# facebookresearch/robust_cvd

Hardware: NVIDIA H100
Metric: flow_residual_constraints_per_sec_per_gn_iteration (higher is better)
Workload: dtype f64

## Files before the change

### include/rcvd_hooks.h

```cpp
#ifndef RCVD_HOOKS_H_
#define RCVD_HOOKS_H_
#include "rcvd.h"
#ifdef __cplusplus
extern "C" {
#endif

int64_t rcvd_launch_count(rcvd_problem* p);
int64_t rcvd_filter_launch_count(void);
int64_t rcvd_builder_launch_count(void);
int64_t rcvd_static_flag_launch_count(void);
int64_t rcvd_tracks_launch_count(void);
int64_t rcvd_builder_last_rounds(void);

int32_t rcvd_structure_info(rcvd_problem* p, int32_t out[8]);

int32_t rcvd_debug_factor_plan(const rcvd_config* cfg, int32_t np, const int32_t* pairs, int32_t nt, const int32_t* trip_centers,
                               int32_t order_slack, int32_t nranks, int32_t rank, int32_t num_sms,
                               int32_t* order, int32_t* level, int32_t* owner, int32_t* perm, int32_t out[13]);
int32_t rcvd_debug_update_passes(const rcvd_config* cfg, int32_t np, const int32_t* pairs, int32_t nt, const int32_t* trip_centers,
                                 int32_t order_slack, int32_t nranks, int32_t rank, int32_t num_sms,
                                 int32_t* passes, int32_t* sources, int32_t* join, int32_t* flags, int32_t counts[5]);

int32_t rcvd_debug_linear_solve(rcvd_problem* p, const double* S, const double* D2, const double* b, double* y);

int32_t rcvd_debug_solve_matrix(rcvd_problem* p, const double* H, const double* D2, const double* b, double* y);
int32_t rcvd_debug_factor_dense(rcvd_problem* p, int32_t* order, double* L, double* Linv);
int32_t rcvd_debug_linear_paths(rcvd_problem* p, int64_t out[13]);

int32_t rcvd_debug_linear_residual(rcvd_problem* p, double radius, double out[6]);

int32_t rcvd_debug_last_iteration(rcvd_problem* p, double* g, double* xc, double out[2]);

int32_t rcvd_debug_profile_linear(rcvd_problem* p, int32_t reps, double out_ms[8]);
int32_t rcvd_debug_level_profile(rcvd_problem* p, double* out, int32_t max_levels);
int32_t rcvd_debug_fp64_tensor_peak(int32_t device, int32_t shape, double* tflops);

int32_t rcvd_debug_set_fast_path(rcvd_problem* p, int32_t on);
int32_t rcvd_debug_set_overlap(rcvd_problem* p, int32_t on);
int32_t rcvd_debug_set_order_slack(rcvd_problem* p, int32_t slack);
int32_t rcvd_debug_set_eval_only(rcvd_problem* p, int32_t on);
int32_t rcvd_debug_set_distributed(rcvd_problem* p, int32_t on);
int32_t rcvd_distribution_info(rcvd_problem* p, int32_t out[4]);
int32_t rcvd_debug_set_update_kernel(rcvd_problem* p, int32_t tma, int32_t side_items_per_cta);

#ifdef __cplusplus
}
#endif
#endif
```

### robust_cvd_b200/csrc/rcvd_api.cu

```cuda
#include <algorithm>
#include <chrono>
#include <cmath>
#include <cstdarg>
#include <cstdio>
#include <cstring>
#include <dlfcn.h>
#include <limits>
#include <string>
#include <vector>

#include <cub/device/device_segmented_sort.cuh>
#include "rcvd_eval.cuh"
#include "rcvd_linalg.cuh"
#include "rcvd_update.cuh"
#include "rcvd_plan.h"
#include "rcvd_host.h"

using namespace rcvd;

static thread_local std::string g_err = "";
int set_err(int code, const char* fmt, ...) {
  char buf[512]; va_list ap; va_start(ap, fmt); vsnprintf(buf, sizeof(buf), fmt, ap); va_end(ap);
  g_err = buf; return code;
}

namespace nccl {
typedef struct { char internal[128]; } UniqueId;
typedef void* Comm;
static void* lib = nullptr;
static int (*GetUniqueId)(UniqueId*) = nullptr;
static int (*CommInitRank)(Comm*, int, UniqueId, int) = nullptr;
static int (*AllReduce)(const void*, void*, size_t, int, int, Comm, cudaStream_t) = nullptr;
static int (*CommDestroy)(Comm) = nullptr;
static const char* (*GetErrorString)(int) = nullptr;
static int (*GroupStart)() = nullptr;
static int (*GroupEnd)() = nullptr;
static int (*Broadcast)(const void*, void*, size_t, int, int, Comm, cudaStream_t) = nullptr;
static int (*Reduce)(const void*, void*, size_t, int, int, int, Comm, cudaStream_t) = nullptr;
static bool load() {
  if (lib) return true;
  const char* names[] = {"libnccl.so.2", "libnccl.so"};
  for (const char* n : names) { lib = dlopen(n, RTLD_NOW | RTLD_GLOBAL); if (lib) break; }
  if (!lib) return false;
  GetUniqueId = (int (*)(UniqueId*))dlsym(lib, "ncclGetUniqueId");
  CommInitRank = (int (*)(Comm*, int, UniqueId, int))dlsym(lib, "ncclCommInitRank");
  AllReduce = (int (*)(const void*, void*, size_t, int, int, Comm, cudaStream_t))dlsym(lib, "ncclAllReduce");
  CommDestroy = (int (*)(Comm))dlsym(lib, "ncclCommDestroy");
  GetErrorString = (const char* (*)(int))dlsym(lib, "ncclGetErrorString");
  GroupStart = (int (*)())dlsym(lib, "ncclGroupStart"); GroupEnd = (int (*)())dlsym(lib, "ncclGroupEnd");
  Broadcast = (int (*)(const void*, void*, size_t, int, int, Comm, cudaStream_t))dlsym(lib, "ncclBroadcast");
  Reduce = (int (*)(const void*, void*, size_t, int, int, int, Comm, cudaStream_t))dlsym(lib, "ncclReduce");
  return GetUniqueId && CommInitRank && AllReduce && CommDestroy && GroupStart && GroupEnd && Broadcast && Reduce;
}
constexpr int kFloat64 = 8, kUint8 = 1, kSum = 0, kMax = 2;
}

enum { SC_COST = 0, SC_CAND = 1, SC_GY = 2, SC_YHY = 3, SC_STEP2 = 4, SC_X2 = 5, SC_GMAX = 6, SC_GDOTD = 7, SC_DMAX = 8, SC_N = 16 };

__global__ void k_extract_diag(const double* __restrict__ H, double* __restrict__ diag, int N, int npad) {
  const int i = blockIdx.x * blockDim.x + threadIdx.x;
  if (i >= N * npad) return;
  const int f = i / npad, l = i % npad;
  diag[i] = H[(size_t)f * npad * npad + (size_t)l * npad + l];
}
__global__ void k_jacobi_scale(const double* __restrict__ diag, double* __restrict__ S, int n, int enable) {
  const int i = blockIdx.x * blockDim.x + threadIdx.x;
  if (i < n) S[i] = enable ? 1.0 / (1.0 + sqrt(diag[i])) : 1.0;
}
__global__ void k_lm_prepare(const double* __restrict__ diagH, const double* __restrict__ S, const double* __restrict__ g, double* __restrict__ lmdiag,
                             double* __restrict__ D2, double* __restrict__ gs, int n, int reuse, double radius, double dmin, double dmax) {
  const int i = blockIdx.x * blockDim.x + threadIdx.x;
  if (i >= n) return;
  const double s = S[i];
  double d = lmdiag[i];
  if (!reuse) { d = fmin(fmax(s * s * diagH[i], dmin), dmax); lmdiag[i] = d; }
  D2[i] = d / radius;
  gs[i] = s * g[i];
}
__global__ void k_mul(const double* __restrict__ a, const double* __restrict__ b, double* __restrict__ o, int n) {
  const int i = blockIdx.x * blockDim.x + threadIdx.x;
  if (i < n) o[i] = a[i] * b[i];
}
__device__ __forceinline__ double project_lb(const rcvd_config& c, const Layout& L, const uint8_t* in_range, int f, int l, double v) {
  if (c.depth_lower_bound && l >= L.offD && l < L.offS && ((l - L.offD) % L.k) == 0 && in_range[f]) return fmax(v, 0.0);
  return v;
}
__global__ void __launch_bounds__(256) k_state_norms(rcvd_config cfg, Layout L, const uint8_t* __restrict__ in_range, const uint8_t* __restrict__ active,
                                                      const double* __restrict__ x, const double* __restrict__ g, double* __restrict__ scal, int N) {
  const int i = blockIdx.x * blockDim.x + threadIdx.x;
  double x2 = 0.0, gm = 0.0;
  if (i < N * L.nf) {
    const int f = i / L.nf, l = i % L.nf;
    const size_t v = (size_t)f * L.npad + l;
    if (active[v]) {
      x2 = x[i] * x[i];
      gm = fabs(x[i] - project_lb(cfg, L, in_range, f, l, x[i] - g[v]));
    }
  }
  x2 = warp_sum(x2);
#pragma unroll
  for (int o = 16; o > 0; o >>= 1) gm = fmax(gm, __shfl_xor_sync(0xffffffffu, gm, o));
  if ((threadIdx.x & 31) == 0) {
    red_add(scal + SC_X2, x2);
    atomicMax((unsigned long long*)(scal + SC_GMAX), (unsigned long long)__double_as_longlong(gm));
  }
}
__global__ void __launch_bounds__(256) k_dot2(const double* __restrict__ a, const double* __restrict__ b, const double* __restrict__ c,
                                               const double* __restrict__ d, int n, double* __restrict__ scal, int s0, int s1) {
  const int i = blockIdx.x * blockDim.x + threadIdx.x;
  double p = 0.0, q = 0.0;
  if (i < n) { p = a[i] * b[i]; q = c[i] * d[i]; }
  p = warp_sum(p); q = warp_sum(q);
  if ((threadIdx.x & 31) == 0) { red_add(scal + s0, p); red_add(scal + s1, q); }
}
__global__ void k_finalize_mask(rcvd_config cfg, Layout L, uint8_t* __restrict__ mask, int N) {
  const int i = blockIdx.x * blockDim.x + threadIdx.x;
  if (i >= N * L.npad) return;
  const int l = i % L.npad;
  if (l >= L.nf || is_const_local(cfg, L, l)) mask[i] = 0;
}
__global__ void k_project_state(rcvd_config cfg, Layout L, const uint8_t* __restrict__ in_range, double* __restrict__ x, int N) {
  const int i = blockIdx.x * blockDim.x + threadIdx.x;
  if (i < N * L.nf) x[i] = project_lb(cfg, L, in_range, i / L.nf, i % L.nf, x[i]);
}
__global__ void k_h_to_dense(const double* __restrict__ H, const HBlock* __restrict__ hb, int nblocks, double* __restrict__ out, int N, int nf, int npad, const int* __restrict__ uperm) {
  const int b = blockIdx.y;
  const int e = blockIdx.x * blockDim.x + threadIdx.x;
  if (e >= nf * nf) return;
  const int i = e / nf, j = e % nf;
  const HBlock hbk = hb[b];
  if (hbk.r == hbk.c && j > i) return;
  const double v = H[(size_t)b * npad * npad + (size_t)i * npad + j];
  const size_t U = (size_t)N * nf;
  const int ur = uperm[hbk.r], uc = uperm[hbk.c];
  out[((size_t)ur * nf + i) * U + (size_t)uc * nf + j] = v;
  out[((size_t)uc * nf + j) * U + (size_t)ur * nf + i] = v;
}

enum { LP_POTRF_SMEM = 0, LP_POTRF_PANEL, LP_TRSM_LL4, LP_TRSM_LL2, LP_TRSM_GEMM, LP_UPD_TMA1, LP_UPD_TMA2, LP_SUB_LEVEL, LP_SUB_FUSED,
       LP_TRINV, LP_OTHER, LP_UPD_TMA1_MULTI, LP_TRSM_STREAMED, LP_N };

struct RecordSet {
  const int width, nframes;
  std::vector<int32_t> frames; std::vector<int64_t> offsets{0}; std::vector<float> records;
  RecordTiles dev = {}; int num_tiles = 0;
  RecordSet(int width_, int nframes_) : width(width_), nframes(nframes_) {}
  int groups() const { return (int)offsets.size() - 1; }
  int64_t count() const { return offsets.back(); }
};

struct rcvd_problem {
  rcvd_config cfg; Layout L; int N = 0; int device = 0;
  cudaStream_t stream = nullptr;
  std::vector<uint8_t> in_range; std::vector<double> median, adaptive;
  RecordSet pairs{6, 2}, trips{10, 1}, dpairs{6, 2};
  std::vector<int32_t> struct_pairs;
  int first_frame = 0, last_frame = -1;
  int32_t* d_blk_of = nullptr; uint8_t *d_in_range = nullptr, *d_active = nullptr;
  double *d_median = nullptr, *d_adaptive = nullptr; float* d_scale_locs = nullptr; int nscale = 0;
  double *d_x = nullptr, *d_xc = nullptr, *d_xsave = nullptr;
  double *d_g = nullptr, *d_S = nullptr, *d_diagH = nullptr, *d_lmdiag = nullptr, *d_D2 = nullptr, *d_gs = nullptr, *d_rhs = nullptr, *d_ytmp = nullptr,
         *d_y = nullptr, *d_Sy = nullptr, *d_Hy = nullptr, *d_partial = nullptr, *d_scal = nullptr;
  double* h_scal = nullptr;
  int part_reg = 0, part_trip = 0, part_dp = 0, npartial = 0;
  double *d_H = nullptr, *d_Lb = nullptr, *d_T = nullptr, *d_invL = nullptr, *d_invT = nullptr;
  HBlock *d_hblocks = nullptr, *d_lblocks = nullptr; int* d_fail = nullptr;
  int* d_potrf_progress = nullptr;
  FactorKernels fk = {};
  FactorPlan plan;
  int *d_lvl_frames = nullptr; TrsmTask* d_trsm_tasks = nullptr; int2* d_upd_pairs = nullptr; SolveTask* d_fwd_tasks = nullptr;
  SubTask* d_sub_tasks = nullptr; int* d_sub_counters = nullptr; int* d_sub_need = nullptr;
  cudaGraphExec_t solve_graph = nullptr;
  bool structure_ready = false, constraints_set = false, frames_set = false;
  int nranks = 1, rank = 0; nccl::Comm comm = nullptr;
  int64_t launches = 0, graph_launches = 0;
  std::vector<double> h_state; bool state_dirty = false; bool overlap = true; int order_slack = 4;
  cudaStream_t side_stream = nullptr; cudaEvent_t ev_fork = nullptr, ev_join = nullptr;
  std::vector<cudaEvent_t> ev_side;
  cudaStream_t inv_stream = nullptr; cudaEvent_t ev_inv_join = nullptr;
  double *d_g2 = nullptr, *d_delta = nullptr; int* h_fail = nullptr;
  cudaEvent_t ev[8] = {nullptr};
  std::vector<void*> allocs;
  std::vector<std::pair<int, cudaEvent_t>>* prof = nullptr;
  bool eval_only = false;
  bool records_sorted = false;
  int fast_path = 1;
  bool dist_enabled = true, graph_warm = false, force_full_H = false;
  int *d_lvl_own = nullptr, *d_load_lblocks = nullptr, *d_own_hblocks = nullptr, *d_uperm = nullptr;
  UpdItem* d_upd_items = nullptr; CUtensorMap tmapT; int num_sms = 0, upd_ipc = 0;
  std::vector<double> level_ms;
  bool factored = false;
  int64_t paths[LP_N] = {0}, graph_paths[LP_N] = {0};
  rcvd_problem() {}
};

template <class... Params, class... Args>
static int launch(rcvd_problem* p, void (*kernel)(Params...), dim3 grid, dim3 block, size_t smem, cudaStream_t s, bool pdl, Args... args) {
  cudaLaunchAttribute attr = {};
  attr.id = cudaLaunchAttributeProgrammaticStreamSerialization; attr.val.programmaticStreamSerializationAllowed = 1;
  cudaLaunchConfig_t lc = {};
  lc.gridDim = grid; lc.blockDim = block; lc.dynamicSmemBytes = smem; lc.stream = s; lc.attrs = &attr; lc.numAttrs = pdl ? 1 : 0;
  CK(cudaLaunchKernelEx(&lc, kernel, args...));
  p->launches += 1;
  return RCVD_OK;
}

template <class T> static int dalloc(rcvd_problem* p, T** ptr, size_t count) {
  *ptr = nullptr;
  if (count == 0) count = 1;
  cudaError_t e = cudaMallocAsync((void**)ptr, count * sizeof(T), p->stream);
  if (e != cudaSuccess) return set_err(RCVD_ERR_CUDA, "cudaMallocAsync(%zu bytes) failed: %s", count * sizeof(T), cudaGetErrorString(e));
  p->allocs.push_back(*ptr);
  return RCVD_OK;
}
template <class T> static int upload(rcvd_problem* p, T** ptr, const std::vector<T>& v) {
  int rc = dalloc(p, ptr, v.size()); if (rc) return rc;
  if (!v.empty()) CK(cudaMemcpyAsync(*ptr, v.data(), v.size() * sizeof(T), cudaMemcpyHostToDevice, p->stream));
  return RCVD_OK;
}
static void free_all(rcvd_problem* p) {
  if (p->solve_graph) { cudaGraphExecDestroy(p->solve_graph); p->solve_graph = nullptr; }
  if (p->side_stream) cudaStreamSynchronize(p->side_stream);
  if (p->inv_stream) cudaStreamSynchronize(p->inv_stream);
  for (void* q : p->allocs) cudaFreeAsync(q, p->stream);
  p->allocs.clear();
  if (p->stream) cudaStreamSynchronize(p->stream);
  if (p->h_scal) { cudaFreeHost(p->h_scal); p->h_scal = nullptr; }
  p->structure_ready = false; p->factored = false;
}

static DevProblem dev_problem(const rcvd_problem* p) {
  DevProblem d; d.cfg = p->cfg; d.L = p->L; d.N = p->N;
  d.pairs = p->pairs.dev; d.trips = p->trips.dev; d.dpairs = p->dpairs.dev;
  d.blk_of = p->d_blk_of; d.in_range = p->d_in_range; d.median = p->d_median;
  d.adaptive = p->adaptive.empty() ? nullptr : p->d_adaptive; d.scale_locs = p->d_scale_locs;
  d.rank = p->rank; d.nranks = p->nranks;
  return d;
}

template <EvalMode MODE>
static int enqueue_residuals(rcvd_problem* p, const double* x, double* g) {
  const DevProblem d = dev_problem(p);
  const RegCounts rcn = reg_counts(p->cfg, p->L, p->N, p->nscale);
  const int regblocks = p->part_trip - p->part_reg, ntiles = p->pairs.num_tiles;
  cudaStream_t st = p->stream; double* part = p->d_partial; int rc;
  if (ntiles > 0) {
    const bool tc = MODE == EvalMode::CostGradH && p->fast_path != 0;
    if (tc && p->fast_path == 1 && p->records_sorted) rc = launch(p, k_accumulate_runs, ntiles, kTile, kRunSmem, st, false, d, x, p->d_H, g, part);
    else if (tc && fast_path_ok(p->cfg, p->L)) rc = launch(p, k_accumulate_fast, ntiles, kTile, kFastSmem, st, false, d, x, p->d_H, g, part);
    else rc = launch(p, k_pairs<MODE>, ntiles, kTile, 0, st, false, d, x, p->d_H, g, part, p->d_active);
    if (rc) return rc;
  }
  if (regblocks > 0 && (rc = launch(p, k_regularisers<MODE>, regblocks, 128, 0, st, false, d, rcn, x, p->d_H, g, part + p->part_reg, p->d_active,
                                    p->first_frame, p->last_frame))) return rc;
  if (p->trips.num_tiles > 0 && (rc = launch(p, k_triplets<MODE>, p->trips.num_tiles, kTile, 0, st, false, d, x, p->d_H, g, part + p->part_trip, p->d_active))) return rc;
  if (p->dpairs.num_tiles > 0 && (rc = launch(p, k_depth_pairs<MODE>, p->dpairs.num_tiles, kTile, 0, st, false, d, x, p->d_H, g, part + p->part_dp, p->d_active))) return rc;
  return RCVD_OK;
}

#define UP(ptr, vec) if ((rc = upload(p, &(ptr), vec))) return rc
#define DA(ptr, n) if ((rc = dalloc(p, &(ptr), (n)))) return rc
static int upload_plan(rcvd_problem* p) {
  const FactorPlan& pl = p->plan; int rc;
  UP(p->d_blk_of, pl.blk_of); UP(p->d_hblocks, pl.hblocks); UP(p->d_lblocks, pl.lblocks); UP(p->d_lvl_frames, pl.lvl_frames); UP(p->d_lvl_own, pl.lvl_own);
  UP(p->d_load_lblocks, pl.load_lblocks); UP(p->d_own_hblocks, pl.own_hblocks); UP(p->d_uperm, pl.uperm);
  UP(p->d_trsm_tasks, pl.trsm_tasks); UP(p->d_upd_pairs, pl.upd_pairs);
  UP(p->d_sub_tasks, pl.sub_tasks); UP(p->d_sub_need, pl.sub_need); DA(p->d_sub_counters, (size_t)4 * p->N + 4);
  UP(p->d_fwd_tasks, pl.fwd_tasks); UP(p->d_upd_items, pl.upd_items);
  return RCVD_OK;
}

static int upload_record_set(rcvd_problem* p, RecordSet& s) {
  std::vector<int32_t> frames(s.frames.size()), tile_group, tile_count; std::vector<int64_t> tile_begin;
  for (size_t i = 0; i < frames.size(); ++i) frames[i] = p->plan.iperm[s.frames[i]];
  for (int i = 0; i < s.groups(); ++i)
    for (int64_t b = s.offsets[i]; b < s.offsets[i + 1]; b += kTile) { tile_group.push_back(i); tile_begin.push_back(b); tile_count.push_back((int32_t)std::min<int64_t>(kTile, s.offsets[i + 1] - b)); }
  s.num_tiles = (int)tile_group.size();
  float* rec; int32_t *fr, *tg, *tn; int64_t* tb; int rc;
  UP(rec, s.records); UP(fr, frames); UP(tg, tile_group); UP(tb, tile_begin); UP(tn, tile_count);
  s.dev = RecordTiles{rec, fr, tg, tb, tn};
  return RCVD_OK;
}

static int set_up_problem_data(rcvd_problem* p) {
  const int N = p->N; const Layout& L = p->L; const std::vector<int>& uperm = p->plan.uperm; int rc;
  for (RecordSet* s : {&p->pairs, &p->trips, &p->dpairs}) if ((rc = upload_record_set(p, *s))) return rc;
  p->records_sorted = false;
  if (run_path_ok(p->cfg, L) && p->pairs.count() > 0 && p->pairs.count() < (int64_t)0x7fffffff) {
    const long long n = p->pairs.count();
    unsigned *d_k0 = nullptr, *d_k1 = nullptr; int *d_i0 = nullptr, *d_i1 = nullptr; float* d_sorted = nullptr; int64_t* d_off = nullptr; void* d_tmp = nullptr;
    if ((rc = dalloc(p, &d_k0, (size_t)n)) || (rc = dalloc(p, &d_k1, (size_t)n)) || (rc = dalloc(p, &d_i0, (size_t)n)) || (rc = dalloc(p, &d_i1, (size_t)n)) || (rc = dalloc(p, &d_sorted, (size_t)n * 6)) ||
        (rc = upload(p, &d_off, p->pairs.offsets))) return rc;
    if ((rc = launch(p, k_record_keys, (unsigned)((n + 255) / 256), 256, 0, p->stream, false, p->cfg, p->pairs.dev.records, n, d_k0, d_i0))) return rc;
    size_t tmp_bytes = 0;
    CK(cub::DeviceSegmentedSort::SortPairs(nullptr, tmp_bytes, d_k0, d_k1, d_i0, d_i1, (int)n, p->pairs.groups(), d_off, d_off + 1, p->stream));
    CK(cudaMallocAsync(&d_tmp, std::max<size_t>(tmp_bytes, 16), p->stream));
    CK(cub::DeviceSegmentedSort::SortPairs(d_tmp, tmp_bytes, d_k0, d_k1, d_i0, d_i1, (int)n, p->pairs.groups(), d_off, d_off + 1, p->stream));
    if ((rc = launch(p, k_gather_records, (unsigned)((n * 6 + 255) / 256), 256, 0, p->stream, false, p->pairs.dev.records, d_i1, n, d_sorted))) return rc;
    CK(cudaFreeAsync(d_tmp, p->stream));
    CK(cudaGetLastError());
    p->pairs.dev.records = d_sorted; p->records_sorted = true;
  }
  {
    std::vector<uint8_t> ir(N); std::vector<double> md(N), ad;
    for (int i = 0; i < N; ++i) { ir[i] = p->in_range[uperm[i]]; md[i] = p->median[uperm[i]]; }
    UP(p->d_in_range, ir); UP(p->d_median, md);
    if (!p->adaptive.empty()) {
      const size_t G = p->adaptive.size() / N; ad.resize(p->adaptive.size());
      for (int i = 0; i < N; ++i) std::copy(p->adaptive.begin() + (size_t)uperm[i] * G, p->adaptive.begin() + (size_t)(uperm[i] + 1) * G, ad.begin() + (size_t)i * G);
      UP(p->d_adaptive, ad);
    }
  }
  {
    std::vector<float> locs; const int gx = p->cfg.scale_grid_x, gy = p->cfg.scale_grid_y;
    for (int y = 0; y < gy; ++y) for (int x = 0; x < gx; ++x) {
      const float fx = -1.f + 2.f * x / (gx - 1);
      const float fy = -1.f + 2.f * y / (gy - 1);
      locs.push_back(fx); locs.push_back(fy);
    }
    p->nscale = (int)(locs.size() / 2);
    UP(p->d_scale_locs, locs);
  }
  p->first_frame = 0; p->last_frame = -1;
  { bool any = false; for (int f = 0; f < N; ++f) if (p->in_range[f]) { if (!any) { p->first_frame = f; any = true; } p->last_frame = f; } }
  p->part_reg = p->pairs.num_tiles;
  p->part_trip = p->part_reg + (reg_counts(p->cfg, L, N, p->nscale).total + 127) / 128;
  p->part_dp = p->part_trip + p->trips.num_tiles;
  p->npartial = p->part_dp + p->dpairs.num_tiles;
  return RCVD_OK;
}
#undef UP

static int allocate_storage(rcvd_problem* p) {
  const int N = p->N; const Layout& L = p->L; const int npad = L.npad, nLoff = p->plan.nLoff; const size_t bs = (size_t)npad * npad; int rc;
  const size_t Upad = (size_t)N * npad, U = (size_t)N * L.nf;
  DA(p->d_x, U); DA(p->d_xc, U); DA(p->d_xsave, U);
  DA(p->d_g, 2 * Upad + 8); p->d_diagH = p->d_g + Upad + 8;
  DA(p->d_S, Upad); DA(p->d_lmdiag, Upad); DA(p->d_D2, Upad); DA(p->d_gs, Upad); DA(p->d_rhs, Upad);
  DA(p->d_g2, Upad + 8); DA(p->d_delta, Upad);
  DA(p->d_ytmp, Upad); DA(p->d_y, Upad); DA(p->d_Sy, Upad); DA(p->d_Hy, Upad); DA(p->d_scal, SC_N); DA(p->d_active, Upad); DA(p->d_fail, 1);
  DA(p->d_potrf_progress, (size_t)N);
  DA(p->d_partial, (size_t)p->npartial);
  if (p->eval_only) { DA(p->d_H, 1); DA(p->d_Lb, 1); DA(p->d_T, 1); DA(p->d_invL, 1); DA(p->d_invT, 1); }
  else {
    DA(p->d_H, p->plan.hblocks.size() * bs); DA(p->d_Lb, (size_t)(N + nLoff) * bs); DA(p->d_T, (size_t)std::max(nLoff, 1) * bs);
    DA(p->d_invL, (size_t)N * bs); DA(p->d_invT, (size_t)N * npad * 16);
  }
#undef DA
  {
    bool encoded = false;
    typedef CUresult (*EncodeFn)(CUtensorMap*, CUtensorMapDataType, cuuint32_t, void*, const cuuint64_t*, const cuuint64_t*, const cuuint32_t*, const cuuint32_t*,
                                 CUtensorMapInterleave, CUtensorMapSwizzle, CUtensorMapL2promotion, CUtensorMapFloatOOBfill);
    void* fn = nullptr; cudaDriverEntryPointQueryResult qres;
    if (cudaGetDriverEntryPoint("cuTensorMapEncodeTiled", &fn, cudaEnableDefault, &qres) == cudaSuccess && fn && qres == cudaDriverEntryPointSuccess) {
      const cuuint64_t gdim[2] = {(cuuint64_t)npad, (cuuint64_t)std::max(nLoff, 1) * npad};
      const cuuint64_t gstr[1] = {(cuuint64_t)npad * sizeof(double)};
      const cuuint32_t box[2] = {16u, (cuuint32_t)p->plan.upd_rb};
      const cuuint32_t estr[2] = {1u, 1u};
      const CUresult r = ((EncodeFn)fn)(&p->tmapT, CU_TENSOR_MAP_DATA_TYPE_FLOAT64, 2, p->d_T, gdim, gstr, box, estr, CU_TENSOR_MAP_INTERLEAVE_NONE,
                                        CU_TENSOR_MAP_SWIZZLE_128B, CU_TENSOR_MAP_L2_PROMOTION_L2_128B, CU_TENSOR_MAP_FLOAT_OOB_FILL_NONE);
      encoded = (r == CUDA_SUCCESS);
    }
    cudaGetLastError();
    if (!encoded) return set_err(RCVD_ERR_CUDA, "cuTensorMapEncodeTiled unavailable or failed: the TMA update kernel cannot run");
    CK(cudaFuncSetAttribute(k_update_tma<1>, cudaFuncAttributeMaxDynamicSharedMemorySize, (int)upd_smem_bytes(p->plan.upd_rb, 1)));
    CK(cudaFuncSetAttribute(k_update_tma<2>, cudaFuncAttributeMaxDynamicSharedMemorySize, (int)upd_smem_bytes(p->plan.upd_rb, 2)));
  }
  CK(cudaMallocHost((void**)&p->h_scal, (SC_N + 2) * sizeof(double)));
  p->h_fail = (int*)(p->h_scal + SC_N);
  CK(cudaMemsetAsync(p->d_x, 0, U * sizeof(double), p->stream));
  CK(cudaMemsetAsync(p->d_lmdiag, 0, Upad * sizeof(double), p->stream));
  CK(cudaMemsetAsync(p->d_S, 0, Upad * sizeof(double), p->stream));
  CK(cudaMemsetAsync(p->d_active, 0, Upad, p->stream));
  if ((rc = enqueue_residuals<EvalMode::MarkActive>(p, p->d_x, nullptr))) return rc;
  if ((rc = launch(p, k_finalize_mask, (int)((Upad + 255) / 256), 256, 0, p->stream, false, p->cfg, L, p->d_active, N))) return rc;
  if (p->nranks > 1) {
    const int r = nccl::AllReduce(p->d_active, p->d_active, Upad, nccl::kUint8, nccl::kMax, p->comm, p->stream);
    if (r != 0) return set_err(RCVD_ERR_NCCL, "ncclAllReduce(active mask) failed");
  }
  FactorKernels& fk = p->fk = factor_kernels(npad);
  if (fk.trinv_bytes > kMaxDynSmem) return set_err(RCVD_ERR_INVALID, "frame block too large for the panel-inverse kernel (npad=%d)", npad);
  CK(cudaFuncSetAttribute(k_trinv, cudaFuncAttributeMaxDynamicSharedMemorySize, (int)fk.trinv_bytes));
  CK(cudaFuncSetAttribute(k_accumulate_fast, cudaFuncAttributeMaxDynamicSharedMemorySize, kFastSmem));
  CK(cudaFuncSetAttribute(k_accumulate_runs, cudaFuncAttributeMaxDynamicSharedMemorySize, kRunSmem));
  if (fk.trsm_ll) {
    CK(cudaFuncSetAttribute(k_trsm_ll<2>, cudaFuncAttributeMaxDynamicSharedMemorySize, (int)fk.trsm_ll2_bytes));
    CK(cudaFuncSetAttribute(k_trsm_ll<2, true>, cudaFuncAttributeMaxDynamicSharedMemorySize, (int)fk.trsm_ll2_bytes));
    CK(cudaOccupancyMaxActiveBlocksPerMultiprocessor(&fk.trsm2_ctas_per_sm, k_trsm_ll<2, true>, 128, fk.trsm_ll2_bytes));
  }
  if (fk.trsm_ll4) {
    CK(cudaFuncSetAttribute(k_trsm_ll<4>, cudaFuncAttributeMaxDynamicSharedMemorySize, (int)fk.trsm_ll4_bytes));
    CK(cudaFuncSetAttribute(k_trsm_ll<4, true>, cudaFuncAttributeMaxDynamicSharedMemorySize, (int)fk.trsm_ll4_bytes));
  }
  if (fk.potrf_smem) CK(cudaFuncSetAttribute(k_potrf_smem, cudaFuncAttributeMaxDynamicSharedMemorySize, (int)fk.potrf_bytes));
  return RCVD_OK;
}

static int build_structure(rcvd_problem* p) {
  if (p->nranks > 1 && !p->dpairs.frames.empty()) return set_err(RCVD_ERR_INVALID, "depth-normalisation pairs are not sharded: they need a single-GPU problem (nranks = 1)");
  free_all(p);
  CK(cudaSetDevice(p->device));
  std::vector<int32_t> graph = p->struct_pairs.empty() ? p->pairs.frames : p->struct_pairs;
  graph.insert(graph.end(), p->dpairs.frames.begin(), p->dpairs.frames.end());
  if (const char* e = make_factor_plan(p->plan, p->cfg, graph, p->trips.frames, p->order_slack, p->nranks, p->rank, p->dist_enabled, p->num_sms))
    return set_err(RCVD_ERR_INVALID, "%s", e);
  while (p->ev_side.size() < 2 * p->plan.levels.size()) { cudaEvent_t e; CK(cudaEventCreateWithFlags(&e, cudaEventDisableTiming)); p->ev_side.push_back(e); }
  int rc;
  if ((rc = upload_plan(p)) || (rc = set_up_problem_data(p)) || (rc = allocate_storage(p))) return rc;
  CK(cudaStreamSynchronize(p->stream));
  p->structure_ready = true;
  return RCVD_OK;
}

static int allreduce(rcvd_problem* p, double* buf, size_t count) {
  if (p->nranks <= 1) return RCVD_OK;
  const int r = nccl::AllReduce(buf, buf, count, nccl::kFloat64, nccl::kSum, p->comm, p->stream);
  if (r != 0) return set_err(RCVD_ERR_NCCL, "ncclAllReduce failed: %s", nccl::GetErrorString ? nccl::GetErrorString(r) : "?");
  return RCVD_OK;
}
struct Seg { size_t first, count; };
static int grouped(rcvd_problem* p, double* base, size_t unit, const std::vector<Seg>& segs, bool bcast) {
  int r = nccl::GroupStart();
  for (size_t i = 0; i < segs.size() && r == 0; ++i) {
    if (segs[i].count == 0) continue;
    const int root = (int)(i % (size_t)p->nranks);
    double* ptr = base + segs[i].first * unit;
    r = bcast ? nccl::Broadcast(ptr, ptr, segs[i].count * unit, nccl::kFloat64, root, p->comm, p->stream)
              : nccl::Reduce(ptr, ptr, segs[i].count * unit, nccl::kFloat64, nccl::kSum, root, p->comm, p->stream);
  }
  const int r2 = nccl::GroupEnd();
  if (r == 0) r = r2;
  if (r != 0) return set_err(RCVD_ERR_NCCL, "grouped NCCL %s failed: %s", bcast ? "broadcast" : "reduce", nccl::GetErrorString ? nccl::GetErrorString(r) : "?");
  return RCVD_OK;
}

struct FactorSolve {
  enum { P_LOAD = 0, P_POTRF, P_TRINV, P_TRSM, P_GEMM, P_SOLVE };
  rcvd_problem* p; const FactorPlan& pl; const FactorKernels& fk; const int N, npad, strips; cudaStream_t st, side, inv;
  int prof_level = 0;
  bool side_used = false, inv_used = false;
  int side_joined = -1;

  explicit FactorSolve(rcvd_problem* p_)
      : p(p_), pl(p_->plan), fk(p_->fk), N(p_->N), npad(p_->L.npad), strips((npad + kTrsmStrip - 1) / kTrsmStrip), st(p_->stream), side(p_->side_stream),
        inv(p_->inv_stream) {}

  void mark(int cls) {
    if (!p->prof) return;
    cudaEvent_t e; cudaEventCreate(&e); cudaEventRecord(e, st); p->prof->push_back({cls < 0 ? cls : (cls | (prof_level << 8)), e});
  }
  template <class... Params, class... Args>
  int launch(int path, void (*kernel)(Params...), dim3 grid, dim3 block, size_t smem, cudaStream_t s, bool pdl, Args... args) {
    if (int rc = ::launch(p, kernel, grid, block, smem, s, pdl, args...)) return rc;
    p->paths[path]++;
    return RCVD_OK;
  }
  int wait(cudaStream_t waiter, cudaStream_t from, cudaEvent_t e) {
    CK(cudaEventRecord(e, from)); CK(cudaStreamWaitEvent(waiter, e, 0));
    return RCVD_OK;
  }
  int join_all(int level) {
    if (side_used) { if (int rc = wait(st, side, p->ev_join)) return rc; side_joined = 2 * level - 1; }
    if (inv_used) { if (int rc = wait(st, inv, p->ev_inv_join)) return rc; inv_used = false; }
    return RCVD_OK;
  }

  bool trsm_deep(const Level& v) const { return strips * v.ntrsm <= p->num_sms && fk.trsm_ll4; }
  bool streamed(const Level& v) const {
    return fk.trsm_ll && v.nown > 0 && v.ntrsm > 0 && fk.potrf_smem && strips * v.ntrsm <= (trsm_deep(v) ? 1 : fk.trsm2_ctas_per_sm) * p->num_sms;
  }

  int factor_diagonal(const int* frames, int nfr, bool pdl) {
    if (fk.potrf_smem)
      return launch(LP_POTRF_SMEM, k_potrf_smem, dim3(nfr), dim3(kPotrfSmemThreads), fk.potrf_bytes, st, pdl, p->d_Lb, p->d_invT, frames, npad,
                    p->d_fail, p->d_potrf_progress);
    for (int jb = 0; jb < npad / 16; ++jb) {
      if (int rc = launch(LP_POTRF_PANEL, k_potrf_panel, dim3(nfr), dim3(kPotrfThreads), 0, st, false, p->d_Lb, p->d_invT, frames, npad, jb, p->d_fail)) return rc;
      const int m = npad - (jb + 1) * 16, n64 = (m + 63) / 64;
      if (m > 0) { if (int rc = launch(LP_OTHER, k_potrf_trail, dim3(n64 * (n64 + 1) / 2, nfr), dim3(128), 0, st, false, p->d_Lb, frames, npad, jb)) return rc; }
    }
    return RCVD_OK;
  }

  int trsm(const Level& lv, const int* frames, int nfr, bool chain) {
    const bool inv_stream = fk.trsm_ll && p->overlap;
    if (inv_stream) { if (int rc = wait(inv, st, p->ev_fork)) return rc; inv_used = true; }
    if (int rc = launch(LP_TRINV, k_trinv, dim3(npad / 16, nfr), dim3(256), fk.trinv_bytes, inv_stream ? inv : st, false,
                        p->d_Lb, p->d_invT, p->d_invL, frames, npad)) return rc;
    mark(P_TRINV);
    if (lv.ntrsm == 0) return RCVD_OK;
    int rc;
    if (fk.trsm_ll) {
      const bool deep = trsm_deep(lv);
      decltype(&k_trsm_ll<2>) kernel = deep ? (chain ? k_trsm_ll<4, true> : k_trsm_ll<4>) : (chain ? k_trsm_ll<2, true> : k_trsm_ll<2>);
      if (chain) p->paths[LP_TRSM_STREAMED]++;
      rc = launch(deep ? LP_TRSM_LL4 : LP_TRSM_LL2, kernel, dim3(strips, lv.ntrsm), dim3(128), deep ? fk.trsm_ll4_bytes : fk.trsm_ll2_bytes, st, chain,
                  p->d_T, p->d_Lb, p->d_invT, p->d_trsm_tasks + lv.trsm_off, npad, chain ? p->d_potrf_progress : nullptr);
    } else {
      const int tiles = (npad + 63) / 64;
      rc = launch(LP_TRSM_GEMM, k_gemm_nt, dim3(tiles, tiles, lv.ntrsm), dim3(128), 0, st, false, p->d_T, p->d_Lb, p->d_invL,
                  p->d_trsm_tasks + lv.trsm_off, npad);
    }
    if (rc) return rc;
    mark(P_TRSM);
    return RCVD_OK;
  }

  int update(cudaStream_t s, int off, int n) {
    if (n <= p->num_sms)
      return launch(LP_UPD_TMA2, k_update_tma<2>, dim3(n), dim3(UpdShape<2>::threads), upd_smem_bytes(pl.upd_rb, 2), s, false,
                    p->tmapT, p->d_Lb, p->d_upd_items + off, n, p->d_upd_pairs, npad, pl.upd_neff, pl.upd_rb, 0);
    int grid = std::min(n, 2 * p->num_sms);
    if (p->upd_ipc > 0) grid = std::max(grid, (n + p->upd_ipc - 1) / p->upd_ipc);
    if (grid < n) p->paths[LP_UPD_TMA1_MULTI]++;
    return launch(LP_UPD_TMA1, k_update_tma<1>, dim3(grid), dim3(UpdShape<1>::threads), upd_smem_bytes(pl.upd_rb, 1), s, false,
                  p->tmapT, p->d_Lb, p->d_upd_items + off, n, p->d_upd_pairs, npad, pl.upd_neff, pl.upd_rb, 0);
  }

  int updates(int li) {
    const Level& lv = pl.levels[li];
    const bool u2 = lv.nit2[0] + lv.nit2[1] > 0;
    const bool fork_late = li + 1 < (int)pl.levels.size() && streamed(pl.levels[li + 1]);
    if (p->overlap && u2 && !fork_late) { if (int rc = wait(side, st, p->ev_fork)) return rc; }
    if (p->overlap) {
      int s = -1;
      for (int q = side_joined + 1; q < 2 * li; ++q) { const Level& v = pl.levels[q / 2]; if (v.nit2[q % 2] > 0 && v.join[q % 2] <= li) s = q; }
      if (s >= 0) { CK(cudaStreamWaitEvent(st, p->ev_side[s], 0)); side_joined = s; }
    }
    if (lv.nit > 0) { if (int rc = update(st, lv.it_off, lv.nit)) return rc; mark(P_GEMM); }
    if (p->overlap && u2 && fork_late) { if (int rc = wait(side, st, p->ev_fork)) return rc; }
    for (int h = 0; h < 2; ++h) if (lv.nit2[h] > 0) {
      if (int rc = update(p->overlap ? side : st, lv.it2_off[h], lv.nit2[h])) return rc;
      mark(P_GEMM);
      if (p->overlap) { CK(cudaEventRecord(p->ev_side[2 * li + h], side)); side_used = true; }
    }
    return RCVD_OK;
  }

  int broadcast_level(int li) {
    std::vector<Seg> segs;
    for (int q = 0; q < p->nranks; ++q) segs.push_back({(size_t)pl.tseg[(li * p->nranks + q) * 2], (size_t)pl.tseg[(li * p->nranks + q) * 2 + 1]});
    return grouped(p, p->d_T, (size_t)npad * npad, segs, true);
  }
  int phase_boundary() {
    if (int rc = join_all(pl.LB)) return rc;
    const size_t bsz = (size_t)npad * npad;
    std::vector<Seg> invs, tr;
    for (int q = 0; q < p->nranks; ++q) invs.push_back({(size_t)pl.fa_off[q], (size_t)pl.fa_cnt[q]});
    for (int q = 0; q < p->nranks; ++q) tr.push_back({(size_t)pl.fb_off[q], (size_t)pl.fb_cnt[q]});
    for (int q = 0; q < p->nranks; ++q) tr.push_back({(size_t)N + (size_t)pl.bseg[2 * q], (size_t)pl.bseg[2 * q + 1]});
    if (int rc = grouped(p, p->d_invL, bsz, invs, true)) return rc;
    return grouped(p, p->d_Lb, bsz, tr, true);
  }

  int substitution() {
    CK(cudaMemcpyAsync(p->d_rhs, p->d_gs, (size_t)N * npad * sizeof(double), cudaMemcpyDeviceToDevice, st));
    const int LS = pl.sub_first_level;
    int rc;
    for (int l = 0; l < LS; ++l) {
      const Level& lv = pl.levels[l];
      if ((rc = launch(LP_SUB_LEVEL, k_fwd_diag, dim3((npad + 7) / 8, lv.nframes), dim3(256), 0, st, false, p->d_invL, p->d_rhs, p->d_ytmp,
                       p->d_lvl_frames + lv.frame_off, npad))) return rc;
      if (lv.nfwd > 0 && (rc = launch(LP_SUB_LEVEL, k_fwd_update, dim3((npad + 7) / 8, lv.nfwd), dim3(256), 0, st, false, p->d_T, p->d_ytmp, p->d_rhs,
                                      p->d_fwd_tasks + lv.fwd_off, npad))) return rc;
    }
    if (LS < (int)pl.levels.size() && !pl.sub_tasks.empty()) {
      CK(cudaMemsetAsync(p->d_sub_counters, 0, ((size_t)4 * N + 4) * sizeof(int), st));
      SubCounters cn; cn.ticket = p->d_sub_counters; cn.fin = p->d_sub_counters + 4; cn.fdone = cn.fin + N; cn.bin = cn.fdone + N; cn.bdone = cn.bin + N;
      cn.fin_need = p->d_sub_need; cn.bin_need = p->d_sub_need + N;
      const int ntasks = (int)pl.sub_tasks.size();
      if ((rc = launch(LP_SUB_FUSED, k_substitution, dim3(std::min(ntasks, p->num_sms)), dim3(kSubThreads), fk.substitution_bytes, st, false,
                       p->d_invL, p->d_T, p->d_rhs, p->d_ytmp, p->d_y, p->d_sub_tasks, ntasks, cn, npad))) return rc;
    }
    for (int l = LS - 1; l >= 0; --l) {
      const Level& lv = pl.levels[l];
      if (lv.nfwd > 0 && (rc = launch(LP_SUB_LEVEL, k_bwd_update, dim3((npad + 31) / 32, lv.nfwd), dim3(256), 0, st, false, p->d_T, p->d_y, p->d_ytmp,
                                      p->d_fwd_tasks + lv.fwd_off, npad))) return rc;
      if ((rc = launch(LP_SUB_LEVEL, k_bwd_diag, dim3((npad + 31) / 32, lv.nframes), dim3(256), 0, st, false, p->d_invL, p->d_ytmp, p->d_y,
                       p->d_lvl_frames + lv.frame_off, npad))) return rc;
    }
    mark(P_SOLVE);
    return RCVD_OK;
  }
};

static int enqueue_factor_solve(rcvd_problem* p) {
  FactorSolve f(p);
  const FactorPlan& pl = p->plan; const int npad = p->L.npad, nlv = (int)pl.levels.size();
  f.mark(-1);
  CK(cudaMemsetAsync(p->d_potrf_progress, 0, (size_t)p->N * sizeof(int), p->stream));
  const int nfill = (int)pl.load_lblocks.size() - pl.nload;
  if (int rc = f.launch(LP_OTHER, k_load_factor, dim3((npad * npad + 255) / 256, pl.nload + load_factor_pad_rows(npad, pl.upd_neff, nfill)), dim3(256), 0,
                        p->stream, false, p->d_H, p->d_Lb, p->d_lblocks, p->d_S, p->d_D2, npad, p->L.nf, pl.upd_neff, p->d_load_lblocks, pl.nload, nfill)) return rc;
  f.mark(FactorSolve::P_LOAD);
  for (int li = 0; li < nlv; ++li) {
    const Level& lv = pl.levels[li]; f.prof_level = li;
    if (pl.dist && li == pl.LB) { if (int rc = f.phase_boundary()) return rc; }
    if (lv.nown > 0) {
      const int* frames = p->d_lvl_own + lv.own_off;
      const bool chain = f.streamed(lv);
      if (int rc = f.factor_diagonal(frames, lv.nown, chain && li > 0)) return rc;
      f.mark(FactorSolve::P_POTRF);
      if (int rc = f.trsm(lv, frames, lv.nown, chain)) return rc;
    }
    if (pl.dist && li < pl.LB) { if (int rc = f.broadcast_level(li)) return rc; }
    if (int rc = f.updates(li)) return rc;
  }
  if (pl.dist && pl.LB >= nlv) { if (int rc = f.phase_boundary()) return rc; }
  if (int rc = f.join_all(nlv)) return rc;
  if (int rc = f.substitution()) return rc;
  CK(cudaGetLastError());
  return RCVD_OK;
}

static int factor_solve(rcvd_problem* p) {
  if (p->nranks > 1 && !p->graph_warm) {
    p->graph_warm = true; p->factored = true;
    return enqueue_factor_solve(p);
  }
  if (!p->solve_graph) {
    cudaGraph_t graph;
    const int64_t l0 = p->launches;
    int64_t paths0[LP_N]; std::copy(p->paths, p->paths + LP_N, paths0);
    CK(cudaStreamBeginCapture(p->stream, cudaStreamCaptureModeThreadLocal));
    int rc = enqueue_factor_solve(p);
    cudaError_t e = cudaStreamEndCapture(p->stream, &graph);
    for (int i = 0; i < LP_N; ++i) { p->graph_paths[i] = p->paths[i] - paths0[i]; p->paths[i] = paths0[i]; }
    if (rc) return rc;
    if (e != cudaSuccess) return set_err(RCVD_ERR_CUDA, "graph capture failed: %s", cudaGetErrorString(e));
    CK(cudaGraphInstantiate(&p->solve_graph, graph, 0));
    cudaGraphDestroy(graph);
    p->graph_launches = p->launches - l0;
    p->launches = l0;
  }
  CK(cudaGraphLaunch(p->solve_graph, p->stream));
  p->launches += p->graph_launches;
  for (int i = 0; i < LP_N; ++i) p->paths[i] += p->graph_paths[i];
  p->factored = true;
  return RCVD_OK;
}


static int enqueue_evaluate(rcvd_problem* p, const double* x, bool wantG, bool wantH, double* gout, int slot) {
  if (wantH && p->eval_only) return set_err(RCVD_ERR_INVALID, "this handle was set to evaluation-only (rcvd_debug_set_eval_only): no normal matrix");
  const Layout& L = p->L; const int N = p->N, npad = L.npad; cudaStream_t st = p->stream;
  const size_t bs = (size_t)npad * npad, Upad = (size_t)N * npad;
  if (wantH) CK(cudaMemsetAsync(p->d_H, 0, p->plan.hblocks.size() * bs * sizeof(double), st));
  if (wantG) CK(cudaMemsetAsync(gout, 0, (Upad + 8) * sizeof(double), st));
  int rc = wantH ? enqueue_residuals<EvalMode::CostGradH>(p, x, gout)
           : wantG ? enqueue_residuals<EvalMode::CostGrad>(p, x, gout) : enqueue_residuals<EvalMode::Cost>(p, x, gout);
  if (rc) return rc;
  if ((rc = launch(p, k_reduce_partials, 1, 1024, 0, st, false, p->d_partial, p->npartial, p->d_scal, slot))) return rc;
  if (p->nranks > 1) {
    if (wantG) {
      CK(cudaMemcpyAsync(gout + Upad, p->d_scal + slot, sizeof(double), cudaMemcpyDeviceToDevice, st));
      size_t cnt = Upad + 8;
      if (wantH && gout == p->d_g) { if ((rc = launch(p, k_extract_diag, (int)((Upad + 255) / 256), 256, 0, st, false, p->d_H, p->d_diagH, N, npad))) return rc; cnt = 2 * Upad + 8; }
      if ((rc = allreduce(p, gout, cnt))) return rc;
      CK(cudaMemcpyAsync(p->d_scal + slot, gout + Upad, sizeof(double), cudaMemcpyDeviceToDevice, st));
    } else if ((rc = allreduce(p, p->d_scal + slot, 1))) return rc;
    if (wantH) {
      if (p->plan.dist && !p->force_full_H) {
        std::vector<Seg> segs;
        for (int q = 0; q < p->nranks; ++q) segs.push_back({(size_t)p->plan.fa_off[q], (size_t)(p->plan.fa_cnt[q] + p->plan.fb_cnt[q])});
        for (int q = 0; q < p->nranks; ++q) segs.push_back({(size_t)p->plan.hseg[2 * q], (size_t)p->plan.hseg[2 * q + 1]});
        if ((rc = grouped(p, p->d_H, bs, segs, false))) return rc;
      } else if ((rc = allreduce(p, p->d_H, p->plan.hblocks.size() * bs))) return rc;
    }
  }
  return RCVD_OK;
}

static int upload_frames(rcvd_problem* p, double* dst, const double* src_user, int stride_dst, int stride_src, int count) {
  std::vector<double> tmp((size_t)p->N * stride_dst, 0.0);
  for (int i = 0; i < p->N; ++i) memcpy(tmp.data() + (size_t)i * stride_dst, src_user + (size_t)p->plan.uperm[i] * stride_src, (size_t)count * sizeof(double));
  CK(cudaMemcpyAsync(dst, tmp.data(), tmp.size() * sizeof(double), cudaMemcpyHostToDevice, p->stream));
  CK(cudaStreamSynchronize(p->stream));
  return RCVD_OK;
}
static int download_frames(rcvd_problem* p, double* dst_user, const double* src, int stride_dst, int stride_src, int count) {
  std::vector<double> tmp((size_t)p->N * stride_src);
  CK(cudaMemcpyAsync(tmp.data(), src, tmp.size() * sizeof(double), cudaMemcpyDeviceToHost, p->stream));
  CK(cudaStreamSynchronize(p->stream));
  for (int i = 0; i < p->N; ++i) memcpy(dst_user + (size_t)p->plan.uperm[i] * stride_dst, tmp.data() + (size_t)i * stride_src, (size_t)count * sizeof(double));
  return RCVD_OK;
}
static int save_state(rcvd_problem* p) {
  DevGuard g(p->device); cudaStreamSynchronize(p->stream);
  if (p->h_state.size() != (size_t)p->N * p->L.nf) p->h_state.assign((size_t)p->N * p->L.nf, 0.0);
  return download_frames(p, p->h_state.data(), p->d_x, p->L.nf, p->L.nf, p->L.nf);
}

static int ensure_ready(rcvd_problem* p) {
  if (!p->structure_ready) {
    if (p->in_range.empty()) p->in_range.assign(p->N, 1);
    if (p->median.empty()) p->median.assign(p->N, 1.0);
    int rc = build_structure(p); if (rc) return rc;
    p->state_dirty = true;
  }
  if (p->state_dirty) {
    if (p->h_state.size() != (size_t)p->N * p->L.nf) p->h_state.assign((size_t)p->N * p->L.nf, 0.0);
    { int rc = upload_frames(p, p->d_x, p->h_state.data(), p->L.nf, p->L.nf, p->L.nf); if (rc) return rc; }
    p->state_dirty = false;
  }
  return RCVD_OK;
}

static int read_scalars(rcvd_problem* p) {
  CK(cudaMemcpyAsync(p->h_scal, p->d_scal, SC_N * sizeof(double), cudaMemcpyDeviceToHost, p->stream));
  CK(cudaMemcpyAsync(p->h_fail, p->d_fail, sizeof(int), cudaMemcpyDeviceToHost, p->stream));
  CK(cudaStreamSynchronize(p->stream));
  return RCVD_OK;
}

namespace ls {
struct Sample { double x, value, gradient; bool valueValid, gradValid; };
static double evalPoly(const std::vector<double>& p, double x) { double v = 0; for (double c : p) v = v * x + c; return v; }
static bool solveDense(std::vector<std::vector<double>> A, std::vector<double> b, std::vector<double>& x) {
  const int n = (int)b.size(); std::vector<int> perm(n); for (int i = 0; i < n; ++i) perm[i] = i;
  for (int k = 0; k < n; ++k) {
    int pr = k, pc = k; double best = 0;
    for (int i = k; i < n; ++i) for (int j = k; j < n; ++j) if (std::fabs(A[i][j]) > best) { best = std::fabs(A[i][j]); pr = i; pc = j; }
    if (best == 0) return false;
    std::swap(A[k], A[pr]); std::swap(b[k], b[pr]);
    for (int i = 0; i < n; ++i) std::swap(A[i][k], A[i][pc]);
    std::swap(perm[k], perm[pc]);
    for (int i = k + 1; i < n; ++i) { const double f = A[i][k] / A[k][k]; for (int j = k; j < n; ++j) A[i][j] -= f * A[k][j]; b[i] -= f * b[k]; }
  }
  std::vector<double> y(n);
  for (int i = n - 1; i >= 0; --i) { double s = b[i]; for (int j = i + 1; j < n; ++j) s -= A[i][j] * y[j]; y[i] = s / A[i][i]; }
  x.assign(n, 0.0); for (int i = 0; i < n; ++i) x[perm[i]] = y[i];
  return true;
}
static std::vector<double> realRoots(std::vector<double> p) {
  while (!p.empty() && p[0] == 0.0) p.erase(p.begin());
  std::vector<double> out; const int d = (int)p.size() - 1; if (d < 1) return out;
  if (d == 1) { out.push_back(-p[1] / p[0]); return out; }
  if (d == 2) { const double a = p[0], b = p[1], c = p[2], D = b * b - 4 * a * c; if (D >= 0) { const double sq = std::sqrt(D); out.push_back((-b + sq) / (2 * a)); out.push_back((-b - sq) / (2 * a)); } else { out.push_back(-b / (2 * a)); out.push_back(-b / (2 * a)); } return out; }
  std::vector<std::pair<double, double>> z(d);
  for (int i = 0; i < d; ++i) { const double ang = 2 * M_PI * i / d + 0.4; z[i] = {0.9 * std::cos(ang), 0.9 * std::sin(ang)}; }
  auto cmul = [](std::pair<double, double> a, std::pair<double, double> b) { return std::make_pair(a.first * b.first - a.second * b.second, a.first * b.second + a.second * b.first); };
  auto cdiv = [](std::pair<double, double> a, std::pair<double, double> b) { const double dd = b.first * b.first + b.second * b.second; return std::make_pair((a.first * b.first + a.second * b.second) / dd, (a.second * b.first - a.first * b.second) / dd); };
  for (int it = 0; it < 500; ++it) {
    double mx = 0;
    for (int i = 0; i < d; ++i) {
      std::pair<double, double> v = {p[0], 0.0};
      for (int j = 1; j <= d; ++j) { v = cmul(v, z[i]); v.first += p[j]; }
      std::pair<double, double> den = {p[0], 0.0};
      for (int j = 0; j < d; ++j) if (j != i) den = cmul(den, {z[i].first - z[j].first, z[i].second - z[j].second});
      auto dl = cdiv(v, den); z[i].first -= dl.first; z[i].second -= dl.second;
      mx = std::max(mx, std::fabs(dl.first) + std::fabs(dl.second));
    }
    if (mx < 1e-14) break;
  }
  for (auto& r : z) out.push_back(r.first);
  return out;
// ... 280 lines not shown
  return RCVD_OK;
}
RCVD_API int32_t rcvd_problem_set_constraints(rcvd_problem* p, int32_t np, const int32_t* pf, const int64_t* off, const float* rec) {
  return set_records(p, &rcvd_problem::pairs, "constraint", np, pf, off, rec);
}
RCVD_API int32_t rcvd_problem_set_triplets(rcvd_problem* p, int32_t nt, const int32_t* centers, const int64_t* off, const float* rec) {
  return set_records(p, &rcvd_problem::trips, "triplet", nt, centers, off, rec);
}
RCVD_API int32_t rcvd_problem_set_depth_pairs(rcvd_problem* p, int32_t np, const int32_t* pf, const int64_t* off, const float* rec) {
  if (p && p->nranks > 1 && np > 0) return set_err(RCVD_ERR_INVALID, "depth-normalisation pairs are not sharded: they need a single-GPU problem (nranks = 1)");
  return set_records(p, &rcvd_problem::dpairs, "depth-pair", np, pf, off, rec);
}
RCVD_API int32_t rcvd_problem_set_structure(rcvd_problem* p, int32_t np, const int32_t* pf) {
  if (!p || np < 0 || (np > 0 && !pf)) return set_err(RCVD_ERR_INVALID, "bad structure arrays");
  p->struct_pairs.assign(pf, pf + 2 * (size_t)np);
  p->structure_ready = false;
  return RCVD_OK;
}
RCVD_API int32_t rcvd_nccl_unique_id(uint8_t out[128]) {
  if (!nccl::load()) return set_err(RCVD_ERR_NCCL, "libnccl.so.2 not found");
  nccl::UniqueId id; const int r = nccl::GetUniqueId(&id);
  if (r != 0) return set_err(RCVD_ERR_NCCL, "ncclGetUniqueId failed (%d)", r);
  memcpy(out, id.internal, 128); return RCVD_OK;
}
RCVD_API int32_t rcvd_problem_init_comm(rcvd_problem* p, int32_t nranks, int32_t rank, const uint8_t uid[128]) {
  if (!p || nranks < 1 || rank < 0 || rank >= nranks) return set_err(RCVD_ERR_INVALID, "bad rank/nranks");
  if (nranks == 1) { p->nranks = 1; p->rank = 0; return RCVD_OK; }
  if (!nccl::load()) return set_err(RCVD_ERR_NCCL, "libnccl.so.2 not found");
  SET_DEVICE(p->device);
  nccl::UniqueId id; memcpy(id.internal, uid, 128);
  const int r = nccl::CommInitRank(&p->comm, nranks, id, rank);
  if (r != 0) return set_err(RCVD_ERR_NCCL, "ncclCommInitRank failed: %s", nccl::GetErrorString ? nccl::GetErrorString(r) : "?");
  p->nranks = nranks; p->rank = rank; p->structure_ready = false;
  return RCVD_OK;
}
RCVD_API int32_t rcvd_problem_set_state(rcvd_problem* p, const double* x) {
  if (!p || !x) return set_err(RCVD_ERR_INVALID, "null argument");
  p->h_state.assign(x, x + (size_t)p->N * p->L.nf); p->state_dirty = true;
  return RCVD_OK;
}
RCVD_API int32_t rcvd_problem_get_state(rcvd_problem* p, double* x) {
  if (!p || !x) return set_err(RCVD_ERR_INVALID, "null argument");
  const size_t U = (size_t)p->N * p->L.nf;
  if (!p->structure_ready || p->state_dirty) { if (p->h_state.size() != U) p->h_state.assign(U, 0.0); memcpy(x, p->h_state.data(), U * sizeof(double)); return RCVD_OK; }
  SET_DEVICE(p->device);
  return download_frames(p, x, p->d_x, p->L.nf, p->L.nf, p->L.nf);
}
RCVD_API int32_t rcvd_evaluate(rcvd_problem* p, double* cost, double* gradient) {
  if (!p || !cost) return set_err(RCVD_ERR_INVALID, "null argument");
  SET_DEVICE(p->device);
  int rc = ensure_ready(p); if (rc) return rc;
  CK(cudaMemsetAsync(p->d_scal, 0, SC_N * sizeof(double), p->stream));
  rc = enqueue_evaluate(p, p->d_x, gradient != nullptr, false, p->d_g, SC_COST); if (rc) return rc;
  rc = read_scalars(p); if (rc) return rc;
  *cost = p->h_scal[SC_COST];
  if (gradient) {
    if ((rc = download_frames(p, gradient, p->d_g, p->L.nf, p->L.npad, p->L.nf))) return rc;
  }
  return RCVD_OK;
}
RCVD_API int32_t rcvd_normal_matrix_dense(rcvd_problem* p, double* Hout) {
  if (!p || !Hout) return set_err(RCVD_ERR_INVALID, "null argument");
  SET_DEVICE(p->device);
  int rc = ensure_ready(p); if (rc) return rc;
  p->force_full_H = true;
  rc = enqueue_evaluate(p, p->d_x, true, true, p->d_g, SC_COST);
  p->force_full_H = false;
  if (rc) return rc;
  const size_t U = (size_t)p->N * p->L.nf;
  double* d_out = nullptr;
  CK(cudaMalloc((void**)&d_out, U * U * sizeof(double)));
  CK(cudaMemsetAsync(d_out, 0, U * U * sizeof(double), p->stream));
  rc = launch(p, k_h_to_dense, dim3(nblk((size_t)p->L.nf * p->L.nf), (int)p->plan.hblocks.size()), 256, 0, p->stream, false, p->d_H, p->d_hblocks, (int)p->plan.hblocks.size(), d_out, p->N, p->L.nf, p->L.npad, p->d_uperm);
  cudaError_t e = rc ? cudaSuccess : cudaMemcpyAsync(Hout, d_out, U * U * sizeof(double), cudaMemcpyDeviceToHost, p->stream);
  cudaStreamSynchronize(p->stream); cudaFree(d_out);
  if (rc) return rc;
  if (e != cudaSuccess) return set_err(RCVD_ERR_CUDA, "copy failed: %s", cudaGetErrorString(e));
  return RCVD_OK;
}
static int solve_loaded(rcvd_problem* p, const double* S, const double* D2, const double* b, double* y) {
  const int N = p->N, nf = p->L.nf, npad = p->L.npad; const size_t Upad = (size_t)N * npad;
  std::vector<double> hs(Upad, 1.0), hd(Upad, 1.0), hb(Upad, 0.0);
  for (int f = 0; f < N; ++f) for (int l = 0; l < nf; ++l) { const size_t u = (size_t)p->plan.uperm[f] * nf + l; hs[(size_t)f * npad + l] = S ? S[u] : 1.0; hd[(size_t)f * npad + l] = D2[u]; hb[(size_t)f * npad + l] = b[u]; }
  CK(cudaMemcpyAsync(p->d_S, hs.data(), Upad * 8, cudaMemcpyHostToDevice, p->stream));
  CK(cudaMemcpyAsync(p->d_D2, hd.data(), Upad * 8, cudaMemcpyHostToDevice, p->stream));
  CK(cudaMemcpyAsync(p->d_gs, hb.data(), Upad * 8, cudaMemcpyHostToDevice, p->stream));
  CK(cudaMemsetAsync(p->d_fail, 0, sizeof(int), p->stream));
  int rc = factor_solve(p); if (rc) return rc;
  std::vector<double> hy(Upad);
  CK(cudaMemcpyAsync(hy.data(), p->d_y, Upad * 8, cudaMemcpyDeviceToHost, p->stream));
  rc = read_scalars(p); if (rc) return rc;
  for (int f = 0; f < N; ++f) for (int l = 0; l < nf; ++l) y[(size_t)p->plan.uperm[f] * nf + l] = hy[(size_t)f * npad + l];
  if (*p->h_fail) return set_err(RCVD_ERR_NUMERIC, "factorisation hit a non-positive pivot");
  return RCVD_OK;
}
RCVD_API int32_t rcvd_debug_linear_solve(rcvd_problem* p, const double* S, const double* D2, const double* b, double* y) {
  if (!p) return set_err(RCVD_ERR_INVALID, "null argument");
  SET_DEVICE(p->device);
  int rc = ensure_ready(p); if (rc) return rc;
  rc = enqueue_evaluate(p, p->d_x, true, true, p->d_g, SC_COST); if (rc) return rc;
  return solve_loaded(p, S, D2, b, y);
}
RCVD_API int32_t rcvd_debug_solve_matrix(rcvd_problem* p, const double* H, const double* D2, const double* b, double* y) {
  if (!p || !H || !D2 || !b || !y) return set_err(RCVD_ERR_INVALID, "null argument");
  if (p->nranks > 1) return set_err(RCVD_ERR_INVALID, "rcvd_debug_solve_matrix works on single-GPU handles only");
  if (p->eval_only) return set_err(RCVD_ERR_INVALID, "this handle was set to evaluation-only (rcvd_debug_set_eval_only): no factor storage");
  SET_DEVICE(p->device);
  int rc = ensure_ready(p); if (rc) return rc;
  const int N = p->N, nf = p->L.nf, npad = p->L.npad; const size_t U = (size_t)N * nf, bs = (size_t)npad * npad;
  std::vector<uint8_t> coupled((size_t)N * N, 0);
  for (const HBlock& hb : p->plan.hblocks) { const int a = p->plan.uperm[hb.r], c = p->plan.uperm[hb.c]; coupled[(size_t)a * N + c] = coupled[(size_t)c * N + a] = 1; }
  for (int a = 0; a < N; ++a) for (int c = 0; c < N; ++c) {
    if (coupled[(size_t)a * N + c]) continue;
    for (int i = 0; i < nf; ++i) for (int j = 0; j < nf; ++j)
      if (H[((size_t)a * nf + i) * U + (size_t)c * nf + j] != 0.0)
        return set_err(RCVD_ERR_INVALID, "H couples frames %d and %d, which the problem's frame graph does not couple", a, c);
  }
  std::vector<double> hH(p->plan.hblocks.size() * bs, 0.0);
  for (int h = 0; h < (int)p->plan.hblocks.size(); ++h) {
    const int a = p->plan.uperm[p->plan.hblocks[h].r], c = p->plan.uperm[p->plan.hblocks[h].c];
    for (int i = 0; i < nf; ++i) for (int j = 0; j < nf; ++j) hH[h * bs + (size_t)i * npad + j] = H[((size_t)a * nf + i) * U + (size_t)c * nf + j];
  }
  CK(cudaMemcpyAsync(p->d_H, hH.data(), hH.size() * sizeof(double), cudaMemcpyHostToDevice, p->stream));
  return solve_loaded(p, nullptr, D2, b, y);
}
RCVD_API int32_t rcvd_debug_factor_dense(rcvd_problem* p, int32_t* order, double* L, double* Linv) {
  if (!p || !order || !L) return set_err(RCVD_ERR_INVALID, "null argument");
  if (!p->structure_ready || !p->factored) return set_err(RCVD_ERR_INVALID, "no factorisation has run on this handle");
  if (p->plan.dist) return set_err(RCVD_ERR_INVALID, "the distributed factorisation keeps its blocks on their owners");
  SET_DEVICE(p->device);
  CK(cudaStreamSynchronize(p->side_stream)); CK(cudaStreamSynchronize(p->inv_stream)); CK(cudaStreamSynchronize(p->stream));
  const int N = p->N, nf = p->L.nf, npad = p->L.npad, nT = p->plan.nLoff; const size_t U = (size_t)N * nf, bs = (size_t)npad * npad;
  std::vector<double> hL((size_t)N * bs), hT((size_t)nT * bs);
  CK(cudaMemcpy(hL.data(), p->d_Lb, hL.size() * sizeof(double), cudaMemcpyDeviceToHost));
  if (nT > 0) CK(cudaMemcpy(hT.data(), p->d_T, hT.size() * sizeof(double), cudaMemcpyDeviceToHost));
  std::vector<size_t> off(N);
  for (int q = 0; q < N; ++q) { off[p->plan.elim_order[q]] = (size_t)q * nf; order[q] = p->plan.uperm[p->plan.elim_order[q]]; }
  std::fill(L, L + U * U, 0.0);
  for (int f = 0; f < N; ++f)
    for (int i = 0; i < nf; ++i) for (int j = 0; j <= i; ++j) L[(off[f] + i) * U + off[f] + j] = hL[f * bs + (size_t)i * npad + j];
  for (int t = 0; t < nT; ++t) {
    const HBlock& b = p->plan.lblocks[N + t];
    for (int i = 0; i < nf; ++i) for (int j = 0; j < nf; ++j) L[(off[b.r] + i) * U + off[b.c] + j] = hT[t * bs + (size_t)i * npad + j];
  }
  if (Linv) {
    CK(cudaMemcpy(hL.data(), p->d_invL, hL.size() * sizeof(double), cudaMemcpyDeviceToHost));
    for (int f = 0; f < N; ++f) {
      double* out = Linv + off[f] * nf;
      for (int i = 0; i < nf; ++i) for (int j = 0; j < nf; ++j) out[(size_t)i * nf + j] = j <= i ? hL[f * bs + (size_t)i * npad + j] : 0.0;
    }
  }
  return RCVD_OK;
}
RCVD_API int32_t rcvd_debug_linear_paths(rcvd_problem* p, int64_t out[13]) {
  if (!p || !out) return set_err(RCVD_ERR_INVALID, "null argument");
  static_assert(LP_N == 13, "include/rcvd_hooks.h documents thirteen counters");
  std::copy(p->paths, p->paths + LP_N, out);
  return RCVD_OK;
}
RCVD_API int32_t rcvd_time_accumulate(rcvd_problem* p, int32_t iters, double* ms) {
  if (!p || iters <= 0) return set_err(RCVD_ERR_INVALID, "bad argument");
  SET_DEVICE(p->device);
  int rc = ensure_ready(p); if (rc) return rc;
  if ((rc = enqueue_evaluate(p, p->d_x, true, true, p->d_g, SC_COST))) return rc;
  CK(cudaEventRecord(p->ev[0], p->stream));
  for (int i = 0; i < iters; ++i) if ((rc = enqueue_evaluate(p, p->d_x, true, true, p->d_g, SC_COST))) return rc;
  CK(cudaEventRecord(p->ev[1], p->stream));
  CK(cudaStreamSynchronize(p->stream));
  *ms = ev_ms(p->ev[0], p->ev[1]) / iters;
  return RCVD_OK;
}
RCVD_API int32_t rcvd_time_iteration(rcvd_problem* p, int32_t iters, double radius, double* ms_iter, double* ms_acc, double* ms_lin, double* ms_cost) {
  if (!p || iters <= 0) return set_err(RCVD_ERR_INVALID, "bad argument");
  SET_DEVICE(p->device);
  int rc = ensure_ready(p); if (rc) return rc;
  const size_t Upad = (size_t)p->N * p->L.npad; cudaStream_t st = p->stream;
  rcvd_solve_options o; rcvd_default_solve_options(&o);
  double ta = 0, tl = 0, tc = 0, tt = 0;
  for (int it = -1; it < iters; ++it) {
    CK(cudaMemsetAsync(p->d_scal, 0, SC_N * sizeof(double), st));
    CK(cudaMemsetAsync(p->d_fail, 0, sizeof(int), st));
    CK(cudaEventRecord(p->ev[0], st));
    if ((rc = enqueue_assemble(p))) return rc;
    if ((rc = launch(p, k_jacobi_scale, nblk(Upad), 256, 0, st, false, p->d_diagH, p->d_S, (int)Upad, o.jacobi_scaling))) return rc;
    CK(cudaEventRecord(p->ev[1], st));
    if ((rc = enqueue_damped_step(p, o, radius, false))) return rc;
    CK(cudaEventRecord(p->ev[2], st));
    if ((rc = enqueue_candidate_cost(p, 1.0, false))) return rc;
    CK(cudaEventRecord(p->ev[3], st));
    if ((rc = read_scalars(p))) return rc;
    if (it >= 0) { ta += ev_ms(p->ev[0], p->ev[1]); tl += ev_ms(p->ev[1], p->ev[2]); tc += ev_ms(p->ev[2], p->ev[3]); tt += ev_ms(p->ev[0], p->ev[3]); }
  }
  *ms_iter = tt / iters; if (ms_acc) *ms_acc = ta / iters; if (ms_lin) *ms_lin = tl / iters; if (ms_cost) *ms_cost = tc / iters;
  return RCVD_OK;
}
RCVD_API int32_t rcvd_debug_last_iteration(rcvd_problem* p, double* g, double* xc, double out[2]) {
  if (!p || !g || !xc || !out) return set_err(RCVD_ERR_INVALID, "null argument");
  if (!p->structure_ready) return set_err(RCVD_ERR_INVALID, "no iteration has run on this handle");
  SET_DEVICE(p->device);
  int rc = read_scalars(p); if (rc) return rc;
  out[0] = p->h_scal[SC_COST]; out[1] = p->h_scal[SC_CAND];
  if ((rc = download_frames(p, g, p->d_g, p->L.nf, p->L.npad, p->L.nf))) return rc;
  return download_frames(p, xc, p->d_xc, p->L.nf, p->L.nf, p->L.nf);
}
RCVD_API int32_t rcvd_debug_profile_linear(rcvd_problem* p, int32_t reps, double out_ms[8]) {
  const bool keep_overlap = reps < 0; if (reps < 0) reps = -reps;
  if (!p || !out_ms || reps == 0) return set_err(RCVD_ERR_INVALID, "bad argument");
  SET_DEVICE(p->device);
  int rc = ensure_ready(p); if (rc) return rc;
  const bool ov = p->overlap; if (!keep_overlap) p->overlap = false;
  for (int i = 0; i < 8; ++i) out_ms[i] = 0.0;
  std::vector<std::pair<int, cudaEvent_t>> evs;
  p->level_ms.assign(p->plan.levels.size() * 6, 0.0);
  for (int r = -1; r < reps; ++r) {
    CK(cudaMemsetAsync(p->d_fail, 0, sizeof(int), p->stream));
    evs.clear(); p->prof = &evs;
    rc = enqueue_factor_solve(p);
    p->prof = nullptr; p->factored = true;
    cudaStreamSynchronize(p->stream); cudaStreamSynchronize(p->side_stream); cudaStreamSynchronize(p->inv_stream);
    double ngemm = 0;
    for (size_t i = 1; i < evs.size(); ++i) {
      float ms = 0; cudaEventElapsedTime(&ms, evs[i - 1].second, evs[i].second);
      const int cls = evs[i].first < 0 ? -1 : (evs[i].first & 0xff), lvl = evs[i].first < 0 ? 0 : (evs[i].first >> 8);
      if (r >= 0 && cls >= 0 && cls < 6) out_ms[cls] += ms;
      if (cls == 4) ngemm += 1;
      if (r == reps - 1 && cls >= 0 && cls < 6 && p->level_ms.size() >= (size_t)(lvl + 1) * 6) p->level_ms[(size_t)lvl * 6 + cls] += ms;
    }
    for (auto& e : evs) cudaEventDestroy(e.second);
    out_ms[6] = ngemm;
    if (rc) break;
  }
  p->overlap = ov;
  for (int i = 0; i < 6; ++i) out_ms[i] /= reps;
  out_ms[7] = p->plan.upd_flops;
  return rc;
}
template <int SHAPE>
__global__ void k_dmma_peak(double* out, int iters) {
  double c[8][4];
#pragma unroll
  for (int i = 0; i < 8; ++i) { c[i][0] = 0; c[i][1] = 0; c[i][2] = 0; c[i][3] = 0; }
  const double a = threadIdx.x * 1e-3, b = 1.0 + threadIdx.x * 1e-6;
  for (int it = 0; it < iters; ++it) {
#pragma unroll
    for (int i = 0; i < 8; ++i) {
      if (SHAPE == 0) dmma_8x8x4(c[i][0], c[i][1], a, b);
      if (SHAPE == 1) dmma_16x8x4(c[i][0], c[i][1], c[i][2], c[i][3], a, a, b);
      if (SHAPE == 2)
        asm volatile("mma.sync.aligned.m16n8k8.row.col.f64.f64.f64.f64 {%0,%1,%2,%3}, {%4,%4,%4,%4}, {%5,%5}, {%0,%1,%2,%3};"
                     : "+d"(c[i][0]), "+d"(c[i][1]), "+d"(c[i][2]), "+d"(c[i][3]) : "d"(a), "d"(b));
      if (SHAPE == 3)
        asm volatile("mma.sync.aligned.m16n8k16.row.col.f64.f64.f64.f64 {%0,%1,%2,%3}, {%4,%4,%4,%4,%4,%4,%4,%4}, {%5,%5,%5,%5}, {%0,%1,%2,%3};"
                     : "+d"(c[i][0]), "+d"(c[i][1]), "+d"(c[i][2]), "+d"(c[i][3]) : "d"(a), "d"(b));
    }
  }
  double s = 0;
#pragma unroll
  for (int i = 0; i < 8; ++i) s += c[i][0] + c[i][1] + c[i][2] + c[i][3];
  out[(size_t)blockIdx.x * blockDim.x + threadIdx.x] = s;
}
RCVD_API int32_t rcvd_debug_fp64_tensor_peak(int32_t device, int32_t shape, double* tflops) {
  if (!tflops || shape < 0 || shape > 3) return set_err(RCVD_ERR_INVALID, "bad argument");
  if (int rc = check_device(device)) return rc;
  SET_DEVICE(device);
  cudaDeviceProp prop; CK(cudaGetDeviceProperties(&prop, device));
  const int threads = 512, blocks = prop.multiProcessorCount * 4, iters = 20000 >> shape;
  const double flops_per_mma = 512.0 * (1 << shape);
  double* out = nullptr; CK(cudaMalloc((void**)&out, (size_t)blocks * threads * sizeof(double)));
  cudaEvent_t e0, e1; cudaEventCreate(&e0); cudaEventCreate(&e1);
  double best = 0;
  for (int rep = 0; rep < 4; ++rep) {
    cudaEventRecord(e0);
    switch (shape) {
      case 0: k_dmma_peak<0><<<blocks, threads>>>(out, iters); break;
      case 1: k_dmma_peak<1><<<blocks, threads>>>(out, iters); break;
      case 2: k_dmma_peak<2><<<blocks, threads>>>(out, iters); break;
      default: k_dmma_peak<3><<<blocks, threads>>>(out, iters); break;
    }
    cudaEventRecord(e1); cudaEventSynchronize(e1);
    float ms = 0; cudaEventElapsedTime(&ms, e0, e1);
    const double tf = flops_per_mma * 8 * iters * (double)blocks * (threads / 32) / (ms * 1e-3) / 1e12;
    if (rep > 0 && tf > best) best = tf;
  }
  cudaEventDestroy(e0); cudaEventDestroy(e1); cudaFree(out);
  CK(cudaGetLastError());
  *tflops = best; return RCVD_OK;
}
__global__ void __launch_bounds__(256) k_lin_residual(const double* __restrict__ S, const double* __restrict__ HSy, const double* __restrict__ D2,
                                                       const double* __restrict__ y, const double* __restrict__ gs, const double* __restrict__ g,
                                                       int n, double* __restrict__ out) {
  const int i = blockIdx.x * blockDim.x + threadIdx.x;
  double r2 = 0.0, b2 = 0.0, g2 = 0.0, y2 = 0.0;
  if (i < n) { const double r = S[i] * HSy[i] + D2[i] * y[i] - gs[i]; r2 = r * r; b2 = gs[i] * gs[i]; g2 = g[i] * g[i]; y2 = y[i] * y[i]; }
  r2 = warp_sum(r2); b2 = warp_sum(b2); g2 = warp_sum(g2); y2 = warp_sum(y2);
  if ((threadIdx.x & 31) == 0) { red_add(out + 0, r2); red_add(out + 1, b2); red_add(out + 2, g2); red_add(out + 3, y2); }
}
RCVD_API int32_t rcvd_debug_linear_residual(rcvd_problem* p, double radius, double out[6]) {
  if (!p || !out || !(radius > 0.0)) return set_err(RCVD_ERR_INVALID, "bad argument");
  SET_DEVICE(p->device);
  int rc = ensure_ready(p); if (rc) return rc;
  const size_t Upad = (size_t)p->N * p->L.npad; cudaStream_t st = p->stream;
  rcvd_solve_options o; rcvd_default_solve_options(&o);
  CK(cudaMemsetAsync(p->d_scal, 0, SC_N * sizeof(double), st));
  CK(cudaMemsetAsync(p->d_fail, 0, sizeof(int), st));
  if ((rc = enqueue_assemble(p))) return rc;
  if ((rc = launch(p, k_jacobi_scale, nblk(Upad), 256, 0, st, false, p->d_diagH, p->d_S, (int)Upad, o.jacobi_scaling))) return rc;
  if ((rc = enqueue_damped_step(p, o, radius, false))) return rc;
  if (p->plan.dist && (rc = allreduce(p, p->d_Hy, Upad))) return rc;
  double* d_out = p->d_scal + 9;
  if ((rc = launch(p, k_lin_residual, nblk(Upad), 256, 0, st, false, p->d_S, p->d_Hy, p->d_D2, p->d_y, p->d_gs, p->d_g, (int)Upad, d_out))) return rc;
  if ((rc = read_scalars(p))) return rc;
  const double r2 = p->h_scal[9], b2 = p->h_scal[10];
  out[0] = b2 > 0.0 ? std::sqrt(r2 / b2) : std::sqrt(r2); out[1] = std::sqrt(b2); out[2] = p->h_scal[SC_COST];
  out[3] = std::sqrt(p->h_scal[11]); out[4] = std::sqrt(p->h_scal[12]); out[5] = (double)*p->h_fail;
  return RCVD_OK;
}
RCVD_API int32_t rcvd_debug_level_profile(rcvd_problem* p, double* out, int32_t max_levels) {
  if (!p || !out) return -1;
  const int n = std::min<int>(max_levels, (int)(p->level_ms.size() / 6));
  for (int i = 0; i < n * 6; ++i) out[i] = p->level_ms[i];
  return n;
}
RCVD_API int64_t rcvd_launch_count(rcvd_problem* p) { return p ? p->launches : 0; }
RCVD_API int32_t rcvd_debug_set_order_slack(rcvd_problem* p, int32_t slack) { if (!p) return RCVD_ERR_INVALID; p->order_slack = slack; p->structure_ready = false; return RCVD_OK; }
RCVD_API int32_t rcvd_debug_set_overlap(rcvd_problem* p, int32_t on) { if (!p) return RCVD_ERR_INVALID; p->overlap = on != 0; if (p->solve_graph) { cudaGraphExecDestroy(p->solve_graph); p->solve_graph = nullptr; } return RCVD_OK; }
RCVD_API int32_t rcvd_debug_set_update_kernel(rcvd_problem* p, int32_t tma, int32_t side_items_per_cta) {
  if (!p) return RCVD_ERR_INVALID;
  if (!tma) return set_err(RCVD_ERR_INVALID, "the cp.async update path was removed: k_update_tma is the only update kernel");
  p->upd_ipc = side_items_per_cta;
  if (p->solve_graph) { cudaGraphExecDestroy(p->solve_graph); p->solve_graph = nullptr; }
  return RCVD_OK;
}
RCVD_API int32_t rcvd_debug_set_eval_only(rcvd_problem* p, int32_t on) { if (!p) return RCVD_ERR_INVALID; p->eval_only = on != 0; p->structure_ready = false; return RCVD_OK; }
RCVD_API int32_t rcvd_debug_set_distributed(rcvd_problem* p, int32_t on) { if (!p) return RCVD_ERR_INVALID; p->dist_enabled = on != 0; if (p->structure_ready) { int rc_ = save_state(p); if (rc_) return rc_; p->state_dirty = true; } p->structure_ready = false; return RCVD_OK; }
RCVD_API int32_t rcvd_distribution_info(rcvd_problem* p, int32_t out[4]) {
  if (!p || !out) return set_err(RCVD_ERR_INVALID, "null argument");
  SET_DEVICE(p->device);
  int rc = ensure_ready(p); if (rc) return rc;
  out[0] = p->plan.dist ? 1 : 0; out[1] = p->plan.LB; out[2] = (int)p->plan.levels.size(); out[3] = p->plan.dist ? p->plan.fa_cnt[p->rank] + p->plan.fb_cnt[p->rank] : p->N;
  return RCVD_OK;
}
RCVD_API int32_t rcvd_debug_set_fast_path(rcvd_problem* p, int32_t on) {
  if (!p) return RCVD_ERR_INVALID;
  if (on < 0 || on > 2) return set_err(RCVD_ERR_INVALID, "fast path switch must be 0, 1 or 2 (got %d)", on);
  p->fast_path = on; return RCVD_OK;
}
RCVD_API int32_t rcvd_solve(rcvd_problem* p, const rcvd_solve_options* opt, rcvd_solve_summary* summary) {
  if (!p || !summary) return set_err(RCVD_ERR_INVALID, "null argument");
  SET_DEVICE(p->device);
  rcvd_solve_options o; if (opt) o = *opt; else rcvd_default_solve_options(&o);
  return lm_solve(p, o, *summary);
}
static int32_t debug_plan(FactorPlan& pl, const rcvd_config* cfg, int32_t np, const int32_t* pairs, int32_t nt, const int32_t* trip_centers,
                          int32_t order_slack, int32_t nranks, int32_t rank, int32_t num_sms) {
  if (!cfg || np < 0 || nt < 0 || (np > 0 && !pairs) || (nt > 0 && !trip_centers)) return set_err(RCVD_ERR_INVALID, "null or negative argument");
  if (nranks < 1 || rank < 0 || rank >= nranks || num_sms < 1) return set_err(RCVD_ERR_INVALID, "bad rank/nranks/num_sms");
  if (const char* e = make_factor_plan(pl, *cfg, std::vector<int32_t>(pairs, pairs + 2 * (size_t)np), std::vector<int32_t>(trip_centers, trip_centers + nt),
                                       order_slack, nranks, rank, true, num_sms))
    return set_err(RCVD_ERR_INVALID, "%s", e);
  return RCVD_OK;
}
RCVD_API int32_t rcvd_debug_factor_plan(const rcvd_config* cfg, int32_t np, const int32_t* pairs, int32_t nt, const int32_t* trip_centers,
                                        int32_t order_slack, int32_t nranks, int32_t rank, int32_t num_sms,
                                        int32_t* order, int32_t* level, int32_t* owner, int32_t* perm, int32_t out[13]) {
  if (!order || !level || !owner || !perm || !out) return set_err(RCVD_ERR_INVALID, "null or negative argument");
  FactorPlan pl;
  if (int32_t rc = debug_plan(pl, cfg, np, pairs, nt, trip_centers, order_slack, nranks, rank, num_sms)) return rc;
  const int N = cfg->num_frames;
  for (int i = 0; i < N; ++i) {
    const int f = pl.uperm[i];
    order[i] = pl.uperm[pl.elim_order[i]]; level[f] = pl.level[i]; owner[f] = pl.owner[i]; perm[i] = f;
  }
  const int32_t v[13] = {(int32_t)pl.levels.size(), pl.nLoff, (int32_t)pl.hblocks.size(), pl.upd_targets, (int32_t)pl.upd_items.size(), (int32_t)pl.sub_tasks.size(),
                         pl.dist ? 1 : 0, pl.LB, pl.sub_first_level, (int32_t)pl.own_lblocks.size(), (int32_t)pl.own_hblocks.size(),
                         pl.dist ? pl.fa_cnt[rank] + pl.fb_cnt[rank] : N, (int32_t)pl.upd_tasks.size()};
  std::copy(v, v + 13, out);
  return RCVD_OK;
}
RCVD_API int32_t rcvd_debug_update_passes(const rcvd_config* cfg, int32_t np, const int32_t* pairs, int32_t nt, const int32_t* trip_centers,
                                          int32_t order_slack, int32_t nranks, int32_t rank, int32_t num_sms,
                                          int32_t* passes, int32_t* sources, int32_t* join, int32_t* flags, int32_t counts[5]) {
  if (!counts) return set_err(RCVD_ERR_INVALID, "null argument");
  FactorPlan pl;
  if (int32_t rc = debug_plan(pl, cfg, np, pairs, nt, trip_centers, order_slack, nranks, rank, num_sms)) return rc;
  const int32_t need[3] = {(int32_t)pl.upd_tasks.size(), (int32_t)pl.upd_pairs.size(), 2 * (int32_t)pl.levels.size()};
  if (passes) {
    if (!sources || !join || !flags || counts[0] < need[0] || counts[1] < need[1] || counts[2] < need[2]) return set_err(RCVD_ERR_INVALID, "null or short output array");
    const int N = cfg->num_frames;
    for (size_t l = 0; l < pl.levels.size(); ++l) {
      const Level& lv = pl.levels[l];
      join[2 * l] = lv.join[0]; join[2 * l + 1] = lv.join[1];
      for (int q = lv.upd_off; q < lv.upd2_off[1] + lv.nupd2[1]; ++q) {
        const UpdPass& t = pl.upd_tasks[q];
        const HBlock& b = pl.lblocks[t.dst];
        int32_t* o = passes + 5 * (size_t)q;
        o[0] = pl.uperm[b.r]; o[1] = pl.uperm[b.c]; o[2] = (int32_t)l; o[3] = q >= lv.upd2_off[1] ? 2 : q >= lv.upd2_off[0] ? 1 : 0; o[4] = t.count;
        flags[q] = t.flags;
        for (int i = 0; i < t.count; ++i) sources[t.first + i] = pl.uperm[pl.lblocks[N + pl.upd_pairs[t.first + i].x].c];
      }
    }
  }
  std::copy(need, need + 3, counts); counts[3] = pl.TB; counts[4] = pl.upd_window;
  return RCVD_OK;
}
RCVD_API int32_t rcvd_structure_info(rcvd_problem* p, int32_t out[8]) {
  if (!p) return set_err(RCVD_ERR_INVALID, "null argument");
  SET_DEVICE(p->device);
  int rc = ensure_ready(p); if (rc) return rc;
  out[0] = p->N; out[1] = p->plan.nLoff; out[2] = (int)p->plan.levels.size(); out[3] = (int)p->plan.hblocks.size(); out[4] = p->L.npad; out[5] = p->L.nf; out[6] = p->pairs.num_tiles;
  out[7] = p->plan.upd_targets;
  return RCVD_OK;
}
```

### robust_cvd_b200/csrc/rcvd_linalg.cuh

```cuda
#pragma once
#include "rcvd_device.cuh"
#include "rcvd_ptx.cuh"

namespace rcvd {

constexpr int kPotrfThreads = 256;

__global__ void __launch_bounds__(kPotrfThreads) k_potrf_panel(double* __restrict__ Lb, double* __restrict__ invT,
                                                                const int* __restrict__ frames, int npad, int jb, int* __restrict__ fail) {
  __shared__ double D[16][17];
  __shared__ double Di[16][17];
  const int frame = frames[blockIdx.x];
  double* A = Lb + (size_t)frame * npad * npad;
  double* iT = invT + (size_t)frame * npad * 16;
  const int tid = threadIdx.x;
  const int j0 = jb * 16;
  {
    const int r = tid >> 4, cc = tid & 15;
    D[r][cc] = (cc <= r) ? A[(size_t)(j0 + r) * npad + j0 + cc] : 0.0;
  }
  __syncthreads();
  if (tid < 32) {
    const int i = tid;
    for (int j = 0; j < 16; ++j) {
// ... 284 lines not shown
  for (int i = 0; i < j; ++i) out[(size_t)(i * 16 + r) * npad + j * 16 + c] = 0.0;
  Z[(size_t)j * 256 + tid] = iT[(size_t)j * 256 + tid];
  out[(size_t)(j * 16 + r) * npad + j * 16 + c] = Z[(size_t)j * 256 + tid];
  __syncthreads();
  for (int i = j + 1; i < nt; ++i) {
    const int kw = (i - j) * 16;
    for (int e = tid; e < 16 * kw; e += 256) { const int rr = e / kw, kk = e % kw; Lrow_s[rr * ldp + kk] = A[(size_t)(i * 16 + rr) * npad + j * 16 + kk]; }
    __syncthreads();
    double s0 = 0.0, s1 = 0.0, s2 = 0.0, s3 = 0.0;
    const double* lr = Lrow_s + r * ldp;
    const double* zp = Z + (size_t)j * 256 + c;
    for (int kk = 0; kk < kw; kk += 4) {
      s0 += lr[kk] * zp[(size_t)kk * 16]; s1 += lr[kk + 1] * zp[(size_t)(kk + 1) * 16];
      s2 += lr[kk + 2] * zp[(size_t)(kk + 2) * 16]; s3 += lr[kk + 3] * zp[(size_t)(kk + 3) * 16];
    }
    W[r][c] = (s0 + s1) + (s2 + s3);
    __syncthreads();
    double zv = 0.0;
    const double* ti = iT + (size_t)i * 256;
#pragma unroll
    for (int q = 0; q < 16; ++q) zv -= ti[r * 16 + q] * W[q][c];
    Z[(size_t)i * 256 + tid] = zv;
    out[(size_t)(i * 16 + r) * npad + j * 16 + c] = zv;
    __syncthreads();
  }
}

struct TrsmTask { int dst; int src; int kframe; };

constexpr int kGemmLd = 20;

template <int NI, int NJ>
__device__ __forceinline__ void gemm_stage(const double* __restrict__ as, const double* __restrict__ bsm, double (&acc)[4][4][2], int wm, int wn, int g, int t) {
#pragma unroll
  for (int k4 = 0; k4 < 4; ++k4) {
    double af[NI > 0 ? NI : 1], bf[NJ > 0 ? NJ : 1];
#pragma unroll
    for (int i = 0; i < NI; ++i) af[i] = as[(wm + i * 8 + g) * kGemmLd + k4 * 4 + t];
#pragma unroll
    for (int j = 0; j < NJ; ++j) bf[j] = bsm[(wn + j * 8 + g) * kGemmLd + k4 * 4 + t];
#pragma unroll
    for (int i = 0; i < NI; ++i)
#pragma unroll
      for (int j = 0; j < NJ; ++j) dmma_8x8x4(acc[i][j][0], acc[i][j][1], af[i], bf[j]);
  }
}

__global__ void __launch_bounds__(128, 4) k_gemm_nt(double* __restrict__ T, const double* __restrict__ Lb, const double* __restrict__ invL,
                                                  const TrsmTask* __restrict__ tasks, int npad) {
  __shared__ __align__(16) double As[2][64 * kGemmLd];
  __shared__ __align__(16) double Bs[2][64 * kGemmLd];
  const TrsmTask task = tasks[blockIdx.z];
  const int m0 = blockIdx.y * 64, n0 = blockIdx.x * 64;
  const size_t bs = (size_t)npad * npad;
  const int tid = threadIdx.x, warp = tid >> 5, lane = tid & 31;
  const int wm = (warp >> 1) * 32, wn = (warp & 1) * 32;
  const int g = lane >> 2, t = lane & 3;
  const int kchunks = min(npad, n0 + 64) / 16;
  const int ni = min(4, max(0, (npad - (m0 + wm)) / 8)), nj = min(4, max(0, (npad - (n0 + wn)) / 8));
  double acc[4][4][2];
#pragma unroll
  for (int i = 0; i < 4; ++i)
#pragma unroll
    for (int j = 0; j < 4; ++j) { acc[i][j][0] = 0.0; acc[i][j][1] = 0.0; }

  auto load_stage = [&](int st, int kk) {
    const double* Ag = Lb + (size_t)task.src * bs + kk * 16;
    const double* Bg = invL + (size_t)task.kframe * bs + kk * 16;
#pragma unroll
    for (int q = 0; q < 4; ++q) {
      const int cidx = tid + q * 128;
      const int row = cidx >> 3, kc = (cidx & 7) * 2;
      const bool va = (m0 + row) < npad, vb = (n0 + row) < npad;
      cp_async16(&As[st][row * kGemmLd + kc], Ag + (size_t)(va ? m0 + row : 0) * npad + kc, va);
      cp_async16(&Bs[st][row * kGemmLd + kc], Bg + (size_t)(vb ? n0 + row : 0) * npad + kc, vb);
    }
    cp_async_commit();
  };

  load_stage(0, 0);
  for (int kk = 0; kk < kchunks; ++kk) {
    const int st = kk & 1;
    if (kk + 1 < kchunks) { load_stage(st ^ 1, kk + 1); cp_async_wait<1>(); } else { cp_async_wait<0>(); }
    __syncthreads();
    const double* as = As[st]; const double* bsm = Bs[st];
    if (ni == 4 && nj == 4) gemm_stage<4, 4>(as, bsm, acc, wm, wn, g, t);
    else if (ni == 4 && nj == 2) gemm_stage<4, 2>(as, bsm, acc, wm, wn, g, t);
    else if (ni == 2 && nj == 4) gemm_stage<2, 4>(as, bsm, acc, wm, wn, g, t);
    else if (ni == 2 && nj == 2) gemm_stage<2, 2>(as, bsm, acc, wm, wn, g, t);
    __syncthreads();
  }
  double* C = T + (size_t)task.dst * bs;
#pragma unroll
  for (int i = 0; i < 4; ++i) {
    const int row = m0 + wm + i * 8 + g;
    if (row >= npad) continue;
#pragma unroll
    for (int j = 0; j < 4; ++j) {
      const int col = n0 + wn + j * 8 + 2 * t;
      if (col >= npad) continue;
      *reinterpret_cast<double2*>(C + (size_t)row * npad + col) = make_double2(acc[i][j][0], acc[i][j][1]);
    }
  }
}

__global__ void __launch_bounds__(128, 4) k_potrf_trail(double* __restrict__ Lb, const int* __restrict__ frames, int npad, int jb) {
  __shared__ __align__(16) double Ps[2][64 * kGemmLd];
  const int frame = frames[blockIdx.y];
  double* A = Lb + (size_t)frame * npad * npad;
  const int j0 = jb * 16, j1 = j0 + 16;
  const int2 tij = tri_index(blockIdx.x);
  const int m0 = j1 + tij.x * 64, n0 = j1 + tij.y * 64;
  const int tid = threadIdx.x, warp = tid >> 5, lane = tid & 31, g = lane >> 2, t = lane & 3;
  const int wm = (warp >> 1) * 32, wn = (warp & 1) * 32;
  for (int e = tid; e < 64 * 8; e += 128) {
    const int row = e >> 3, kc = (e & 7) * 2;
    const bool va = (m0 + row) < npad, vb = (n0 + row) < npad;
    cp_async16(&Ps[0][row * kGemmLd + kc], A + (size_t)(va ? m0 + row : 0) * npad + j0 + kc, va);
    cp_async16(&Ps[1][row * kGemmLd + kc], A + (size_t)(vb ? n0 + row : 0) * npad + j0 + kc, vb);
  }
  cp_async_commit(); cp_async_wait<0>();
  __syncthreads();
  const int ni = min(4, max(0, (npad - (m0 + wm)) / 8)), nj = min(4, max(0, (npad - (n0 + wn)) / 8));
  double acc[4][4][2];
#pragma unroll
  for (int i = 0; i < 4; ++i)
#pragma unroll
    for (int j = 0; j < 4; ++j) { acc[i][j][0] = 0.0; acc[i][j][1] = 0.0; }
  if (ni == 4 && nj == 4) gemm_stage<4, 4>(Ps[0], Ps[1], acc, wm, wn, g, t);
  else if (ni == 4 && nj == 2) gemm_stage<4, 2>(Ps[0], Ps[1], acc, wm, wn, g, t);
  else if (ni == 2 && nj == 4) gemm_stage<2, 4>(Ps[0], Ps[1], acc, wm, wn, g, t);
  else if (ni == 2 && nj == 2) gemm_stage<2, 2>(Ps[0], Ps[1], acc, wm, wn, g, t);
#pragma unroll
  for (int i = 0; i < 4; ++i) {
    const int row = m0 + wm + i * 8 + g;
    if (i >= ni) continue;
#pragma unroll
    for (int j = 0; j < 4; ++j) {
      const int col = n0 + wn + j * 8 + 2 * t;
      if (j >= nj || col > row) continue;
      double* ptr = A + (size_t)row * npad + col;
      if (col + 1 <= row) { double2 o = *reinterpret_cast<double2*>(ptr); o.x -= acc[i][j][0]; o.y -= acc[i][j][1]; *reinterpret_cast<double2*>(ptr) = o; }
      else ptr[0] -= acc[i][j][0];
    }
  }
}

constexpr int kTrsmRW = 8;
constexpr int kTrsmStrip = 4 * kTrsmRW;
__host__ __device__ inline size_t trsm_ll_smem_bytes(int npad, int ahead) { return ((size_t)kTrsmStrip * (npad + 4) + ahead * 16 * (size_t)(npad + 4) + ahead * 16 * 20) * sizeof(double); }

template <int kTrsmAhead, bool kStreamed = false>
__global__ void __launch_bounds__(128) k_trsm_ll(double* __restrict__ T, const double* __restrict__ Lb, const double* __restrict__ invT,
                                                  const TrsmTask* __restrict__ tasks, int npad, const int* progress) {
  static_assert(!kStreamed || kTrsmAhead <= 4, "cp_async_wait_upto3 leaves at most three groups in flight");
  extern __shared__ __align__(16) double smx[];
  __shared__ int s_ready;
  const int ld = npad + 4;
  double* Xs = smx;
  double* Ls = smx + (size_t)kTrsmStrip * ld;
  double* Ds = Ls + (size_t)kTrsmAhead * 16 * ld;
  const TrsmTask task = tasks[blockIdx.y];
  const int m0 = blockIdx.x * kTrsmStrip;
  const size_t bs = (size_t)npad * npad;
  const double* A = Lb + (size_t)task.src * bs;
  const double* Lk = Lb + (size_t)task.kframe * bs;
  const double* iT = invT + (size_t)task.kframe * npad * 16;
  double* X = T + (size_t)task.dst * bs;
  const int tid = threadIdx.x, warp = tid >> 5, lane = tid & 31, g = lane >> 2, t = lane & 3;
  const int nt = npad / 16;
  const int rows = min(kTrsmStrip, npad - m0);
  for (int r = tid >> 3; r < kTrsmStrip; r += 16) {
    const bool v = r < rows;
    const double* src = A + (size_t)(v ? m0 + r : 0) * npad;
    for (int c = (tid & 7) * 2; c < npad; c += 16) cp_async16(&Xs[(size_t)r * ld + c], src + c, v);
  }
  auto stage = [&](int jt) {
    if (jt < nt) {
      double* ls = Ls + (size_t)(jt % kTrsmAhead) * 16 * ld; double* dsm = Ds + (jt % kTrsmAhead) * 320;
      const int kw = jt * 16;
      { const int r = tid >> 3; const double* src = Lk + (size_t)(jt * 16 + r) * npad; for (int c = (tid & 7) * 2; c < kw; c += 16) cp_async16(&ls[(size_t)r * ld + c], src + c, true); }
      { const int r = tid >> 3, c = (tid & 7) * 2; cp_async16(&dsm[r * 20 + c], iT + (size_t)jt * 256 + r * 16 + c, true); }
    }
    cp_async_commit();
  };
  if constexpr (kStreamed) {
    cp_async_commit();
  } else {
#pragma unroll
    for (int q = 0; q < kTrsmAhead; ++q) stage(q);
  }
  constexpr int NI = kTrsmRW / 8;
  const int wr = warp * kTrsmRW;
  int staged = 0, ready = 0;
  for (int jt = 0; jt < nt; ++jt) {
    if constexpr (kStreamed) {
      if (ready < min(nt, jt + kTrsmAhead)) {
        if (tid == 0) {
          int v = ld_acquire_gpu(progress + task.kframe);
          while (v <= jt) { __nanosleep(32); v = ld_acquire_gpu(progress + task.kframe); }
          s_ready = v;
        }
        __syncthreads();
        ready = s_ready;
      }
      for (; staged < min(ready, jt + kTrsmAhead); ++staged) stage(staged);
      cp_async_wait_upto3(staged - 1 - jt);
    } else {
      cp_async_wait<kTrsmAhead - 1>();
    }
    __syncthreads();
    const double* ls = Ls + (size_t)(jt % kTrsmAhead) * 16 * ld; const double* dsm = Ds + (jt % kTrsmAhead) * 320;
    double acc[NI][2][2];
#pragma unroll
    for (int i = 0; i < NI; ++i) { acc[i][0][0] = acc[i][0][1] = acc[i][1][0] = acc[i][1][1] = 0.0; }
    {
      double af[2][4][NI], bf[2][4][2];
      auto frag = [&](int kt, int buf) {
#pragma unroll
        for (int q = 0; q < 4; ++q) {
#pragma unroll
          for (int i = 0; i < NI; ++i) af[buf][q][i] = Xs[(size_t)(wr + i * 8 + g) * ld + kt * 16 + q * 4 + t];
#pragma unroll
          for (int j = 0; j < 2; ++j) bf[buf][q][j] = ls[(size_t)(j * 8 + g) * ld + kt * 16 + q * 4 + t];
        }
      };
      if (jt > 0) frag(0, 0);
      for (int kt = 0; kt < jt; kt += 2) {
        if (kt + 1 < jt) frag(kt + 1, 1);
#pragma unroll
        for (int q = 0; q < 4; ++q)
#pragma unroll
          for (int i = 0; i < NI; ++i)
#pragma unroll
            for (int j = 0; j < 2; ++j) dmma_8x8x4(acc[i][j][0], acc[i][j][1], af[0][q][i], bf[0][q][j]);
        if (kt + 1 < jt) {
          if (kt + 2 < jt) frag(kt + 2, 0);
#pragma unroll
          for (int q = 0; q < 4; ++q)
#pragma unroll
            for (int i = 0; i < NI; ++i)
#pragma unroll
              for (int j = 0; j < 2; ++j) dmma_8x8x4(acc[i][j][0], acc[i][j][1], af[1][q][i], bf[1][q][j]);
        }
      }
    }
#pragma unroll
    for (int i = 0; i < NI; ++i)
#pragma unroll
      for (int j = 0; j < 2; ++j) {
        double2* ptr = reinterpret_cast<double2*>(&Xs[(size_t)(wr + i * 8 + g) * ld + jt * 16 + j * 8 + 2 * t]);
        double2 v = *ptr; v.x -= acc[i][j][0]; v.y -= acc[i][j][1]; *ptr = v;
      }
    __syncwarp();
    double out[NI][2][2];
#pragma unroll
    for (int i = 0; i < NI; ++i) { out[i][0][0] = out[i][0][1] = out[i][1][0] = out[i][1][1] = 0.0; }
#pragma unroll
    for (int k4 = 0; k4 < 4; ++k4) {
      double af[NI], bf[2];
#pragma unroll
      for (int i = 0; i < NI; ++i) af[i] = Xs[(size_t)(wr + i * 8 + g) * ld + jt * 16 + k4 * 4 + t];
#pragma unroll
      for (int j = 0; j < 2; ++j) bf[j] = dsm[(j * 8 + g) * 20 + k4 * 4 + t];
#pragma unroll
      for (int i = 0; i < NI; ++i)
#pragma unroll
        for (int j = 0; j < 2; ++j) dmma_8x8x4(out[i][j][0], out[i][j][1], af[i], bf[j]);
    }
    __syncwarp();
#pragma unroll
    for (int i = 0; i < NI; ++i)
#pragma unroll
      for (int j = 0; j < 2; ++j) {
        const int r = wr + i * 8 + g, cidx = jt * 16 + j * 8 + 2 * t;
        const double2 v = make_double2(out[i][j][0], out[i][j][1]);
        *reinterpret_cast<double2*>(&Xs[(size_t)r * ld + cidx]) = v;
        if (r < rows) *reinterpret_cast<double2*>(&X[(size_t)(m0 + r) * npad + cidx]) = v;
      }
    __syncthreads();
    if constexpr (!kStreamed) stage(jt + kTrsmAhead);
  }
  if constexpr (kStreamed) griddep_wait();
}


__global__ void __launch_bounds__(256) k_fwd_diag(const double* __restrict__ invL, const double* __restrict__ rhs, double* __restrict__ y,
                                                   const int* __restrict__ frames, int npad) {
  const int frame = frames[blockIdx.y];
  const int row = blockIdx.x * 8 + (threadIdx.x >> 5);
  const int lane = threadIdx.x & 31;
  if (row >= npad) return;
  const double* M = invL + (size_t)frame * npad * npad + (size_t)row * npad;
  const double* b = rhs + (size_t)frame * npad;
  double s = 0.0;
  for (int q = lane; q <= row; q += 32) s += M[q] * b[q];
  s = warp_sum(s);
  if (lane == 0) y[(size_t)frame * npad + row] = s;
}
struct SolveTask { int blk; int r; int k; };
__global__ void __launch_bounds__(256) k_fwd_update(const double* __restrict__ T, const double* __restrict__ y, double* __restrict__ rhs,
                                                     const SolveTask* __restrict__ tasks, int npad) {
  const SolveTask tk = tasks[blockIdx.y];
  const int row = blockIdx.x * 8 + (threadIdx.x >> 5);
  const int lane = threadIdx.x & 31;
  if (row >= npad) return;
  const double* M = T + (size_t)tk.blk * npad * npad + (size_t)row * npad;
  const double* v = y + (size_t)tk.k * npad;
  double s = 0.0;
  for (int q = lane; q < npad; q += 32) s += M[q] * v[q];
  s = warp_sum(s);
  if (lane == 0) red_add(rhs + (size_t)tk.r * npad + row, -s);
}
__global__ void __launch_bounds__(256) k_bwd_update(const double* __restrict__ T, const double* __restrict__ x, double* __restrict__ y,
                                                     const SolveTask* __restrict__ tasks, int npad) {
  __shared__ double red[8][33];
  const SolveTask tk = tasks[blockIdx.y];
  const int cl = threadIdx.x & 31, rg = threadIdx.x >> 5;
  const int j = blockIdx.x * 32 + cl;
  double acc = 0.0;
  if (j < npad) {
    const double* M = T + (size_t)tk.blk * npad * npad + j;
    const double* xr = x + (size_t)tk.r * npad;
    for (int i = rg; i < npad; i += 8) acc += M[(size_t)i * npad] * xr[i];
  }
  red[rg][cl] = acc;
  __syncthreads();
  if (rg == 0 && j < npad) {
    double s = 0.0;
#pragma unroll
    for (int q = 0; q < 8; ++q) s += red[q][cl];
    if (s != 0.0) red_add(y + (size_t)tk.k * npad + j, -s);
  }
}
__global__ void __launch_bounds__(256) k_bwd_diag(const double* __restrict__ invL, const double* __restrict__ y, double* __restrict__ x,
                                                   const int* __restrict__ frames, int npad) {
  __shared__ double red[8][33];
  const int frame = frames[blockIdx.y];
  const int cl = threadIdx.x & 31, rg = threadIdx.x >> 5;
  const int j = blockIdx.x * 32 + cl;
  double acc = 0.0;
  if (j < npad) {
    const double* M = invL + (size_t)frame * npad * npad + j;
    const double* v = y + (size_t)frame * npad;
    const int i0 = j - (j % 8) + rg;
    for (int i = (i0 < j ? i0 + 8 : i0); i < npad; i += 8) acc += M[(size_t)i * npad] * v[i];
  }
  red[rg][cl] = acc;
  __syncthreads();
  if (rg == 0 && j < npad) {
    double s = 0.0;
#pragma unroll
    for (int q = 0; q < 8; ++q) s += red[q][cl];
    x[(size_t)frame * npad + j] = s;
  }
}

constexpr int kSubChunk = 64;
constexpr int kSubThreads = 256;
struct SubTask { int type; int blk; int r; int k; int chunk; };
struct SubCounters { int* ticket; int* fin; int* fdone; int* bin; int* bdone; const int* fin_need; const int* bin_need; };

__device__ __forceinline__ void sub_wait(const int* c, int need) { while (ld_acquire_gpu(c) < need) __nanosleep(20); }

__device__ __forceinline__ double2 ldcg2(const double* p) { return __ldcg(reinterpret_cast<const double2*>(p)); }

__global__ void __launch_bounds__(kSubThreads) k_substitution(const double* __restrict__ invL, const double* __restrict__ T, double* rhs, double* y, double* x,
                                                              const SubTask* __restrict__ tasks, int ntasks, SubCounters cn, int npad) {
  extern __shared__ __align__(16) double red[];
  __shared__ int s_task;
  const int tid = threadIdx.x, warp = tid >> 5, lane = tid & 31;
  const int nchunks = (npad + kSubChunk - 1) / kSubChunk;
  const size_t bs = (size_t)npad * npad;
  for (;;) {
    if (tid == 0) s_task = atomicAdd(cn.ticket, 1);
    __syncthreads();
    const int ti = s_task;
    if (ti >= ntasks) break;
    const SubTask tk = tasks[ti];
    const int c0 = tk.chunk * kSubChunk, c1 = min(npad, c0 + kSubChunk);
    const double* vin = tk.type == 0 ? rhs + (size_t)tk.k * npad : (tk.type == 2 ? x + (size_t)tk.r * npad : y + (size_t)tk.k * npad);
    const double* M = (tk.type == 0 || tk.type == 3) ? invL + (size_t)tk.k * bs : T + (size_t)tk.blk * bs;
    auto dep_wait = [&]() {
      if (tid == 0) {
        if (tk.type == 0) sub_wait(cn.fin + tk.k, cn.fin_need[tk.k]);
        else if (tk.type == 1) sub_wait(cn.fdone + tk.k, nchunks);
        else if (tk.type == 2) sub_wait(cn.bdone + tk.r, nchunks);
        else { sub_wait(cn.fdone + tk.k, nchunks); sub_wait(cn.bin + tk.k, cn.bin_need[tk.k]); }
      }
      __syncthreads();
    };
    if (tk.type <= 1) {
      constexpr int RW = kSubChunk / (kSubThreads / 32);
      const int r0 = c0 + warp * RW;
      double acc[RW];
#pragma unroll
      for (int i = 0; i < RW; ++i) acc[i] = 0.0;
      for (int qb = 0; qb < npad; qb += 256) {
        double2 m[4][RW];
#pragma unroll
        for (int qi = 0; qi < 4; ++qi) {
          const int q = qb + qi * 64 + 2 * lane;
#pragma unroll
          for (int i = 0; i < RW; ++i) {
            const int row = r0 + i;
            const int len = tk.type == 0 ? row + 1 : npad;
            m[qi][i] = (row < c1 && q < len) ? *reinterpret_cast<const double2*>(M + (size_t)row * npad + q) : make_double2(0.0, 0.0);
            if (q + 1 >= len) m[qi][i].y = 0.0;
          }
        }
        if (qb == 0) dep_wait();
        double2 v[4];
#pragma unroll
        for (int qi = 0; qi < 4; ++qi) { const int q = qb + qi * 64 + 2 * lane; v[qi] = q < npad ? ldcg2(vin + q) : make_double2(0.0, 0.0); }
#pragma unroll
        for (int qi = 0; qi < 4; ++qi)
#pragma unroll
          for (int i = 0; i < RW; ++i) acc[i] += m[qi][i].x * v[qi].x + m[qi][i].y * v[qi].y;
      }
#pragma unroll
      for (int i = 0; i < RW; ++i) {
        const double sum = warp_sum(acc[i]);
        const int row = r0 + i;
        if (lane == 0 && row < c1) { if (tk.type == 0) y[(size_t)tk.k * npad + row] = sum; else red_add(rhs + (size_t)tk.r * npad + row, -sum); }
      }
    } else {
      const int cl = tid & 31, rg = tid >> 5, j = c0 + 2 * cl;
      double ax = 0.0, ay = 0.0;
      const int ifirst = tk.type == 3 ? j + ((rg - j) & 7) : rg;
      for (int ib = ifirst; ib < npad || ib == ifirst; ib += 256) {
        double2 m[32];
#pragma unroll
        for (int u = 0; u < 32; ++u) { const int i = ib + 8 * u; m[u] = (i < npad && j < c1) ? *reinterpret_cast<const double2*>(M + (size_t)i * npad + j) : make_double2(0.0, 0.0); }
        if (ib == ifirst) dep_wait();
// ... 99 lines not shown
```

### robust_cvd_b200/csrc/rcvd_plan.h

```cpp
#pragma once
#include <algorithm>
#include <map>
#include <set>
#include <vector>

#include "rcvd_linalg.cuh"
#include "rcvd_update.cuh"

namespace rcvd {

struct UpdPass { int dst; int first; int count; int flags; };

struct Level { int frame_off, nframes; int trsm_off, ntrsm; int upd_off, nupd; int upd2_off[2], nupd2[2]; int fwd_off, nfwd; int it_off, nit, it2_off[2], nit2[2]; int own_off, nown; int join[2]; };

constexpr int kUpdWindow = 2, kUpdWindowMaxNf = 256;

struct FactorPlan {
  std::vector<int> elim_order;
  std::vector<int> level, owner;
  std::vector<Level> levels;
  bool dist = false; int LB = 0;
  std::vector<int> uperm, iperm;
  std::vector<int> fa_off, fa_cnt, fb_off, fb_cnt, tseg, bseg, hseg;
  int nLoff = 0;
// ... 55 lines not shown
      }
    }
    for (int f = 0; f < N; ++f) std::sort(cs[f].begin(), cs[f].end(), [&](int a, int b) { return pos[a] < pos[b]; });
  }
  std::vector<int> lvl(N, 0); int nl = 0;
  for (int k : order) { for (int a : cs[k]) lvl[a] = std::max(lvl[a], lvl[k] + 1); nl = std::max(nl, lvl[k] + 1); }
  std::vector<std::vector<int>> lf(nl);
  for (int k : order) lf[lvl[k]].push_back(k);

  const int R = nranks;
  bool dist = R > 1 && dist_enabled && cfg.intr_opt != RCVD_INTR_SHARED && !(cfg.position_reg > 0.0) && trip_centers.empty();
  int TB = nl; while (TB > 0 && (int)lf[TB - 1].size() < 3) --TB;
  int LB = 0;
  if (dist) { LB = TB; if (LB == 0) dist = false; }
  P.dist = dist; P.LB = LB; P.TB = TB;
  std::vector<int> own(N, 0);
  if (dist) {
    std::vector<double> tot_in(N, 0.0);
    for (int l = 0; l < LB; ++l) for (int k : lf[l]) { const auto& m = cs[k]; for (size_t a = 0; a < m.size(); ++a) for (size_t b = 0; b <= a; ++b) tot_in[m[b]] += (a == b) ? 0.5 : 1.0; }
    std::vector<double> load(R, 0.0);
    for (int l = 0; l < nl; ++l) {
      std::vector<int> fr = lf[l];
      auto w = [&](int k) { return tot_in[k] + (l < LB ? 0.6 * cs[k].size() + 0.3 : 0.0); };
      std::stable_sort(fr.begin(), fr.end(), [&](int a, int b) { return w(a) > w(b); });
      for (int k : fr) { int q = 0; for (int t = 1; t < R; ++t) if (load[t] < load[q]) q = t; own[k] = q; load[q] += w(k); }
    }
  }
  std::vector<int>& uperm = P.uperm; std::vector<int>& iperm = P.iperm;
  iperm.assign(N, -1);
  P.fa_off.assign(R, 0); P.fa_cnt.assign(R, 0); P.fb_off.assign(R, 0); P.fb_cnt.assign(R, 0);
  for (int q = 0; q < R; ++q) for (int ph = 0; ph < 2; ++ph) {
    (ph ? P.fb_off : P.fa_off)[q] = (int)uperm.size();
    for (int f = 0; f < N; ++f) if (own[f] == q && ((lvl[f] >= LB) == (ph == 1))) uperm.push_back(f);
    (ph ? P.fb_cnt : P.fa_cnt)[q] = (int)uperm.size() - (ph ? P.fb_off : P.fa_off)[q];
  }
  for (int i = 0; i < N; ++i) iperm[uperm[i]] = i;
  bool identity_perm = true; for (int i = 0; i < N; ++i) if (uperm[i] != i) identity_perm = false;
  if (!identity_perm) {
    auto I = [&](int f) { return iperm[f]; };
    std::vector<int> order2(N), pos2(N), lvl2(N), own2(N); std::vector<std::vector<int>> cs2(N); std::vector<std::set<int>> orig2(N);
    for (int i = 0; i < N; ++i) order2[i] = I(order[i]);
    for (int f = 0; f < N; ++f) { pos2[I(f)] = pos[f]; lvl2[I(f)] = lvl[f]; own2[I(f)] = own[f]; for (int a : cs[f]) cs2[I(f)].push_back(I(a)); for (int a : orig[f]) orig2[I(f)].insert(I(a)); }
    for (auto& v : lf) for (int& k : v) k = I(k);
    order.swap(order2); pos.swap(pos2); lvl.swap(lvl2); own.swap(own2); cs.swap(cs2); orig.swap(orig2);
  }
  std::map<std::pair<int, int>, int> lid; int nLoff = 0;
  std::vector<int> lcol;
  auto number_col = [&](int k) { for (int r : cs[k]) { lid[{r, k}] = N + nLoff++; lcol.push_back(k); } };
  P.tseg.assign((size_t)std::max(LB, 0) * R * 2, 0); P.bseg.assign((size_t)R * 2, 0);
  for (int l = 0; l < LB; ++l) for (int q = 0; q < R; ++q) {
    const int first = nLoff;
    for (int k : lf[l]) if (own[k] == q) number_col(k);
    P.tseg[((size_t)l * R + q) * 2] = first; P.tseg[((size_t)l * R + q) * 2 + 1] = nLoff - first;
  }
  for (int q = 0; q < R; ++q) {
    const int first = nLoff;
    for (int l = LB; l < nl; ++l) for (int k : lf[l]) if (own[k] == q) number_col(k);
    P.bseg[(size_t)q * 2] = first; P.bseg[(size_t)q * 2 + 1] = nLoff - first;
  }
  P.nLoff = nLoff;
  std::vector<HBlock>& hblocks = P.hblocks;
  P.blk_of.assign((size_t)N * N, -1);
  for (int f = 0; f < N; ++f) hblocks.push_back({f, f, f});
  P.hseg.assign((size_t)R * 2, 0);
  for (int q = 0; q < R; ++q) {
    P.hseg[(size_t)q * 2] = (int)hblocks.size();
    for (int a = 0; a < N; ++a) for (int b : orig[a]) if (a < b) {
      const int r = pos[a] > pos[b] ? a : b, c = pos[a] > pos[b] ? b : a;
      if (own[c] != q) continue;
      const int hid = (int)hblocks.size();
      hblocks.push_back({lid[{r, c}], r, c});
      P.blk_of[(size_t)r * N + c] = hid * 2 + 1;
      P.blk_of[(size_t)c * N + r] = hid * 2 + 0;
    }
    P.hseg[(size_t)q * 2 + 1] = (int)hblocks.size() - P.hseg[(size_t)q * 2];
  }
  const int nHblocks = (int)hblocks.size();
  P.lblocks.resize(N + nLoff);
  for (int f = 0; f < N; ++f) P.lblocks[f] = {f, f, f};
  for (auto& kv : lid) P.lblocks[kv.second] = {-1, kv.first.first, kv.first.second};
  for (int h = N; h < nHblocks; ++h) P.lblocks[hblocks[h].lblk].lblk = h;
  P.elim_order = order; P.level = lvl; P.owner = own;
  for (int b = 0; b < N + nLoff; ++b) { const int c = b < N ? b : lcol[b - N]; if (!dist || own[c] == rank) P.own_lblocks.push_back(b); }
  for (int h = 0; h < nHblocks; ++h) if (!dist || own[hblocks[h].c] == rank) P.own_hblocks.push_back(h);
  for (int b : P.own_lblocks) if (P.lblocks[b].lblk >= 0) P.load_lblocks.push_back(b);
  P.nload = (int)P.load_lblocks.size();
  for (int b : P.own_lblocks) if (P.lblocks[b].lblk < 0) P.load_lblocks.push_back(b);
  const int upd_neff = std::min(npad, (L.nf + 7) / 8 * 8);
  const int upd_nt = (upd_neff + kUpdMaxTile - 1) / kUpdMaxTile;
  const int upd_tile = std::min(kUpdMaxTile, upd_neff);
  P.upd_rb = upd_tile; P.upd_neff = upd_neff;
  auto col_of = [&](int target) { return target < N ? target : lcol[target - N]; };
  std::map<int, std::vector<std::pair<int, int2>>> prod;
  std::map<int, int> first_level;
  for (int l = 0; l < nl; ++l) {
    const bool shared_level = !dist || l >= LB;
    std::set<int> targets;
    for (int k : lf[l]) for (size_t a = 0; a < cs[k].size(); ++a) for (size_t b = 0; b <= a; ++b) {
      const int r = cs[k][a], c = cs[k][b];
      const int target = (r == c) ? r : lid[{r, c}];
      first_level.emplace(target, l);
      if (!shared_level && own[c] != rank) continue;
      prod[target].push_back({l, make_int2(lid[{r, k}] - N, lid[{c, k}] - N)});
      targets.insert(target);
    }
    P.upd_targets += (int)targets.size();
  }
  const int W = P.upd_window = L.nf <= kUpdWindowMaxNf ? kUpdWindow : 1;
  auto window = [&](int l) { return l < TB ? l / W : nl + l; };
  std::vector<std::vector<std::pair<int, std::vector<int2>>>> late(nl), deferred(nl);
  for (auto& kv : prod) {
    const int Lc = lvl[col_of(kv.first)];
    const auto& v = kv.second;
    for (size_t i = 0, j; i < v.size(); i = j) {
      const bool is_late = v[i].first == Lc - 1;
      for (j = i + 1; j < v.size() && (v[j].first == Lc - 1) == is_late && (is_late || window(v[j].first) == window(v[i].first)); ++j) {}
      auto& pass = (is_late ? late : deferred)[v[j - 1].first];
      pass.push_back({kv.first, {}});
      for (size_t q = i; q < j; ++q) pass.back().second.push_back(v[q].second);
    }
  }
  std::vector<uint8_t> updated(N + nLoff, 0);
  for (int l = 0; l < nl; ++l) {
    Level lv; lv.frame_off = (int)P.lvl_frames.size(); lv.nframes = (int)lf[l].size(); lv.own_off = (int)P.lvl_own.size();
    lv.trsm_off = (int)P.trsm_tasks.size(); lv.upd_off = (int)P.upd_tasks.size(); lv.fwd_off = (int)P.fwd_tasks.size();
    const bool shared_level = !dist || l >= LB;
    for (int k : lf[l]) {
      P.lvl_frames.push_back(k);
      const bool mine = shared_level || own[k] == rank;
      if (mine) P.lvl_own.push_back(k);
      for (int r : cs[k]) {
        const int id = lid[{r, k}];
        if (mine) P.trsm_tasks.push_back({id - N, id, k});
        P.fwd_tasks.push_back({id - N, r, k});
      }
    }
    lv.nown = (int)P.lvl_own.size() - lv.own_off;
    lv.join[0] = lv.join[1] = nl;
    const bool split = W > 1 && l < TB;
    for (int pass = 0; pass < 3; ++pass) {
      if (pass > 0) lv.upd2_off[pass - 1] = (int)P.upd_tasks.size();
      for (auto& tp : (pass ? deferred : late)[l]) {
        const int Lc = lvl[col_of(tp.first)];
        if (pass > 0 && (!split || Lc == l + 2) != (pass == 1)) continue;
        if (pass > 0) lv.join[pass - 1] = std::min(lv.join[pass - 1], Lc - 1);
        const bool first_fill = P.lblocks[tp.first].lblk < 0 && !updated[tp.first] && prod[tp.first][0].first == first_level[tp.first];
        updated[tp.first] = 1;
        P.upd_tasks.push_back({tp.first, (int)P.upd_pairs.size(), (int)tp.second.size(), (tp.first < N ? 1 : 0) | (first_fill ? 2 : 0)});
        { const double n = (double)L.nf; P.upd_flops += (double)tp.second.size() * (tp.first < N ? n * n * (n + 1.0) : 2.0 * n * n * n); }
        P.upd_pairs.insert(P.upd_pairs.end(), tp.second.begin(), tp.second.end());
      }
    }
    lv.ntrsm = (int)P.trsm_tasks.size() - lv.trsm_off; lv.nupd = lv.upd2_off[0] - lv.upd_off; lv.nfwd = (int)P.fwd_tasks.size() - lv.fwd_off;
    lv.nupd2[0] = lv.upd2_off[1] - lv.upd2_off[0]; lv.nupd2[1] = (int)P.upd_tasks.size() - lv.upd2_off[1];
    std::vector<UpdItem>& items = P.upd_items;
    for (int pass = 0; pass < 3; ++pass) {
      const int t0 = pass ? lv.upd2_off[pass - 1] : lv.upd_off, tn = pass ? lv.nupd2[pass - 1] : lv.nupd;
      const size_t i0 = items.size();
      for (int q = t0; q < t0 + tn; ++q) {
        const UpdPass& tk = P.upd_tasks[q];
        for (int ti = 0; ti < upd_nt; ++ti) for (int tj = 0; tj < ((tk.flags & 1) ? ti + 1 : upd_nt); ++tj) {
          UpdItem it; it.dst = tk.dst; it.first = tk.first; it.count = tk.count; it.m0 = (short)(ti * upd_tile); it.n0 = (short)(tj * upd_tile);
          it.mrows = (short)std::min(upd_tile, upd_neff - ti * upd_tile); it.ncols = (short)std::min(upd_tile, upd_neff - tj * upd_tile);
          it.flags = (((tk.flags & 1) && ti == tj) ? kUpdSymDiag : 0) | ((tk.flags & 2) ? kUpdFirstFill : 0);
          items.push_back(it);
        }
      }
      auto cost = [](const UpdItem& a) { return (long)a.count * (a.mrows / 8) * (a.ncols / 8) * ((a.flags & kUpdSymDiag) ? 3 : 4); };
      std::stable_sort(items.begin() + i0, items.end(), [&](const UpdItem& a, const UpdItem& b) { return cost(a) > cost(b); });
      if (pass) { lv.it2_off[pass - 1] = (int)i0; lv.nit2[pass - 1] = (int)(items.size() - i0); } else { lv.it_off = (int)i0; lv.nit = (int)(items.size() - i0); }
    }
    P.levels.push_back(lv);
  }
  P.sub_need.assign(2 * (size_t)N, 0);
  {
    const int nch = (npad + kSubChunk - 1) / kSubChunk;
    const int limit = 4 * num_sms;
    int LS = (int)P.levels.size();
    while (LS > 0 && (P.levels[LS - 1].nframes + P.levels[LS - 1].nfwd) * nch <= limit) --LS;
    P.sub_first_level = LS;
    for (size_t l = LS; l < P.levels.size(); ++l) {
      const Level& lv = P.levels[l];
      for (int i = 0; i < lv.nframes; ++i) for (int c = 0; c < nch; ++c) P.sub_tasks.push_back({0, -1, -1, P.lvl_frames[lv.frame_off + i], c});
      for (int q = 0; q < lv.nfwd; ++q) { const SolveTask& t = P.fwd_tasks[lv.fwd_off + q]; for (int c = 0; c < nch; ++c) P.sub_tasks.push_back({1, t.blk, t.r, t.k, c}); P.sub_need[t.r] += nch; P.sub_need[N + t.k] += nch; }
    }
    for (int l = (int)P.levels.size() - 1; l >= LS; --l) {
      const Level& lv = P.levels[l];
      for (int q = 0; q < lv.nfwd; ++q) { const SolveTask& t = P.fwd_tasks[lv.fwd_off + q]; for (int c = 0; c < nch; ++c) P.sub_tasks.push_back({2, t.blk, t.r, t.k, c}); }
      for (int i = 0; i < lv.nframes; ++i) for (int c = 0; c < nch; ++c) P.sub_tasks.push_back({3, -1, -1, P.lvl_frames[lv.frame_off + i], c});
    }
  }
  return nullptr;
}

}
```

### robust_cvd_b200/csrc/rcvd_ptx.cuh

```cuda
#pragma once
#include <cuda.h>
#include <cuda_runtime.h>
#include <stdint.h>

namespace rcvd {

__device__ __forceinline__ uint32_t smem_u32(const void* p) { return (uint32_t)__cvta_generic_to_shared(p); }

__device__ __forceinline__ void dmma_8x8x4(double& c0, double& c1, double a, double b) {
  asm volatile("mma.sync.aligned.m8n8k4.row.col.f64.f64.f64.f64 {%0,%1}, {%2}, {%3}, {%0,%1};"
               : "+d"(c0), "+d"(c1) : "d"(a), "d"(b));
}
__device__ __forceinline__ void dmma_16x8x4(double& c0, double& c1, double& c2, double& c3, double a0, double a1, double b) {
  asm volatile("mma.sync.aligned.m16n8k4.row.col.f64.f64.f64.f64 {%0,%1,%2,%3}, {%4,%5}, {%6}, {%0,%1,%2,%3};"
               : "+d"(c0), "+d"(c1), "+d"(c2), "+d"(c3) : "d"(a0), "d"(a1), "d"(b));
}

__device__ __forceinline__ void cp_async16(void* smem, const void* gmem) {
  asm volatile("cp.async.cg.shared.global [%0], [%1], 16;" ::"r"(smem_u32(smem)), "l"(gmem) : "memory");
}
__device__ __forceinline__ void cp_async16(void* smem, const void* gmem, bool valid) {
  const int sz = valid ? 16 : 0;
  asm volatile("cp.async.cg.shared.global [%0], [%1], 16, %2;" ::"r"(smem_u32(smem)), "l"(gmem), "r"(sz) : "memory");
}
__device__ __forceinline__ void cp_async4_ca(void* smem, const void* gmem) {
  asm volatile("cp.async.ca.shared.global [%0], [%1], 4;" ::"r"(smem_u32(smem)), "l"(gmem) : "memory");
}
__device__ __forceinline__ void cp_async_commit() { asm volatile("cp.async.commit_group;" ::: "memory"); }
template <int N> __device__ __forceinline__ void cp_async_wait() { asm volatile("cp.async.wait_group %0;" ::"n"(N) : "memory"); }
__device__ __forceinline__ void cp_async_wait_upto3(int n) {
  if (n >= 3) cp_async_wait<3>(); else if (n == 2) cp_async_wait<2>(); else if (n == 1) cp_async_wait<1>(); else cp_async_wait<0>();
}

__device__ __forceinline__ void mbar_init(uint64_t* bar, int count) { asm volatile("mbarrier.init.shared::cta.b64 [%0], %1;" ::"r"(smem_u32(bar)), "r"(count) : "memory"); }
__device__ __forceinline__ void mbar_expect_tx(uint64_t* bar, uint32_t bytes) {
  asm volatile("mbarrier.arrive.expect_tx.shared::cta.b64 _, [%0], %1;" ::"r"(smem_u32(bar)), "r"(bytes) : "memory");
}
__device__ __forceinline__ void mbar_arrive(uint64_t* bar) { asm volatile("mbarrier.arrive.shared::cta.b64 _, [%0];" ::"r"(smem_u32(bar)) : "memory"); }
__device__ __forceinline__ void mbar_wait(uint64_t* bar, uint32_t parity) {
  asm volatile(
      "{\n"
      ".reg .pred P1;\n"
      "LAB_WAIT:\n"
      "mbarrier.try_wait.parity.shared::cta.b64 P1, [%0], %1;\n"
      "@P1 bra DONE;\n"
      "bra LAB_WAIT;\n"
      "DONE:\n"
      "}" ::"r"(smem_u32(bar)), "r"(parity) : "memory");
}
__device__ __forceinline__ void tma_load_2d(void* dst, const CUtensorMap* map, uint64_t* bar, int c0, int c1) {
  asm volatile("cp.async.bulk.tensor.2d.shared::cluster.global.mbarrier::complete_tx::bytes [%0], [%1, {%3, %4}], [%2];"
               ::"r"(smem_u32(dst)), "l"(reinterpret_cast<uint64_t>(map)), "r"(smem_u32(bar)), "r"(c0), "r"(c1) : "memory");
}
__device__ __forceinline__ void prefetch_l2_bulk(const void* gmem, int bytes) { asm volatile("cp.async.bulk.prefetch.L2.global [%0], %1;" ::"l"(gmem), "r"(bytes) : "memory"); }

__device__ __forceinline__ int ld_acquire_gpu(const int* p) { int v; asm volatile("ld.acquire.gpu.global.s32 %0, [%1];" : "=r"(v) : "l"(p) : "memory"); return v; }
__device__ __forceinline__ void st_release_gpu(int* p, int v) { asm volatile("st.release.gpu.global.s32 [%0], %1;" ::"l"(p), "r"(v) : "memory"); }
__device__ __forceinline__ void red_release_add(int* p, int v) { asm volatile("red.release.gpu.global.add.s32 [%0], %1;" ::"l"(p), "r"(v) : "memory"); }
__device__ __forceinline__ void griddep_wait() { asm volatile("griddepcontrol.wait;" ::: "memory"); }
__device__ __forceinline__ void griddep_launch_dependents() { asm volatile("griddepcontrol.launch_dependents;" ::: "memory"); }
template <int ID, int N> __device__ __forceinline__ void named_bar_sync() { asm volatile("bar.sync %0, %1;" ::"n"(ID), "n"(N) : "memory"); }
template <int ID, int N> __device__ __forceinline__ void named_bar_arrive() { asm volatile("bar.arrive %0, %1;" ::"n"(ID), "n"(N) : "memory"); }

template <class Index> __device__ __forceinline__ int2 tri_index(Index t) {
  int i = (int)((sqrtf(8.f * t + 1.f) - 1.f) * 0.5f);
  while ((i + 1) * (i + 2) / 2 <= (int)t) ++i;
  while (i * (i + 1) / 2 > (int)t) --i;
  return make_int2(i, (int)t - i * (i + 1) / 2);
}

}
```

### robust_cvd_b200/csrc/rcvd_update.cuh

```cuda
#pragma once
#include "rcvd_linalg.cuh"
#include "rcvd_ptx.cuh"

namespace rcvd {

struct UpdItem {
  int dst;
  int first, count;
  short m0, n0;
  short mrows, ncols;
  int flags;
};
constexpr int kUpdSymDiag = 1;
constexpr int kUpdFirstFill = 2;

constexpr int kUpdMaxTile = 80;
constexpr int kUpdPartial = 4 * 25 * 32 * 2;
template <int TEAMS> struct UpdShape { static constexpr int stages = TEAMS == 2 ? 8 : 5, threads = TEAMS * 128 + 32, ctas = TEAMS == 2 ? 1 : 2; };
__host__ __device__ inline size_t upd_smem_bytes(int rb, int teams) {
  const int stages = teams == 2 ? 8 : 5;
  return (size_t)stages * 2 * rb * 16 * sizeof(double) + (teams == 2 ? (size_t)kUpdPartial * sizeof(double) : 0) + 2 * stages * sizeof(uint64_t) + 1024;
}

template <int NI, int NJ>
__device__ __forceinline__ void upd_mma(const double (&af)[NI], const double (&bf)[NJ], double (&acc)[5][5][2]) {
#pragma unroll
  for (int i = 0; i + 1 < NI; i += 2)
#pragma unroll
    for (int j = 0; j < NJ; ++j) dmma_16x8x4(acc[i][j][0], acc[i][j][1], acc[i + 1][j][0], acc[i + 1][j][1], af[i], af[i + 1], bf[j]);
  if (NI & 1) {
#pragma unroll
    for (int j = 0; j < NJ; ++j) dmma_8x8x4(acc[NI - 1][j][0], acc[NI - 1][j][1], af[NI - 1], bf[j]);
  }
}

template <int NI, int NJ>
__device__ __forceinline__ void upd_stage(const unsigned char* __restrict__ As, const unsigned char* __restrict__ Bs, const int (&kc)[4], int k4n, double (&acc)[5][5][2]) {
  if (k4n == 4) {
#pragma unroll
    for (int k4 = 0; k4 < 4; ++k4) {
      double af[NI], bf[NJ];
#pragma unroll
      for (int i = 0; i < NI; ++i) af[i] = *reinterpret_cast<const double*>(As + kc[k4] + i * 1024);
#pragma unroll
      for (int j = 0; j < NJ; ++j) bf[j] = *reinterpret_cast<const double*>(Bs + kc[k4] + j * 1024);
      upd_mma<NI, NJ>(af, bf, acc);
    }
  } else {
#pragma unroll
    for (int k4 = 0; k4 < 4; ++k4) {
      if (k4 < k4n) {
        double af[NI], bf[NJ];
#pragma unroll
        for (int i = 0; i < NI; ++i) af[i] = *reinterpret_cast<const double*>(As + kc[k4] + i * 1024);
#pragma unroll
        for (int j = 0; j < NJ; ++j) bf[j] = *reinterpret_cast<const double*>(Bs + kc[k4] + j * 1024);
        upd_mma<NI, NJ>(af, bf, acc);
      }
    }
  }
}

template <int NI, int NJ>
__device__ __forceinline__ void upd_epilogue(double* __restrict__ C, int npad, const double (&acc)[5][5][2], int t, const double* __restrict__ part, bool fresh) {
  const bool hi = (t & 2) != 0;
#pragma unroll
  for (int i = 0; i < NI; ++i) {
    double2 v[NJ];
#pragma unroll
    for (int j = 0; j < NJ; ++j) v[j] = fresh ? make_double2(0.0, 0.0) : *reinterpret_cast<const double2*>(C + (size_t)i * 8 * npad + j * 8);
#pragma unroll
    for (int j = 0; j < NJ; ++j) {
      double a0 = acc[i][j][0], a1 = acc[i][j][1];
      if (part) { const double2 q = *reinterpret_cast<const double2*>(part + (size_t)(i * 5 + j) * 64); a0 += q.x; a1 += q.y; }
      const double give = hi ? a0 : a1;
      const double got = __shfl_xor_sync(0xffffffffu, give, 2);
      const double lo = hi ? got : a0, up = hi ? a1 : got;
      v[j].x -= lo; v[j].y -= up;
      *reinterpret_cast<double2*>(C + (size_t)i * 8 * npad + j * 8) = v[j];
    }
  }
}
template <int NI, int NJ>
__device__ __forceinline__ void upd_store_partial(double* __restrict__ part, const double (&acc)[5][5][2]) {
#pragma unroll
  for (int i = 0; i < NI; ++i)
#pragma unroll
    for (int j = 0; j < NJ; ++j) *reinterpret_cast<double2*>(part + (size_t)(i * 5 + j) * 64) = make_double2(acc[i][j][0], acc[i][j][1]);
}

#define RCVD_UPD_CASES(M) \
  M(1, 1) M(1, 2) M(1, 3) M(1, 4) M(1, 5) M(2, 1) M(2, 2) M(2, 3) M(2, 4) M(2, 5) M(3, 1) M(3, 2) M(3, 3) M(3, 4) M(3, 5) \
  M(4, 1) M(4, 2) M(4, 3) M(4, 4) M(4, 5) M(5, 1) M(5, 2) M(5, 3) M(5, 4) M(5, 5)

template <int TEAMS>
__global__ void __launch_bounds__(UpdShape<TEAMS>::threads, UpdShape<TEAMS>::ctas) k_update_tma(const __grid_constant__ CUtensorMap tmap, double* __restrict__ dst,
                                                               const UpdItem* __restrict__ items, int nitems, const int2* __restrict__ pairs,
                                                               int npad, int neff, int rb, int dbg) {
  extern __shared__ __align__(1024) unsigned char ring[];
  griddep_launch_dependents();
  if (smem_u32(ring) & 1023u) __trap();
  constexpr int kUpdStages = UpdShape<TEAMS>::stages;
  const int tile_bytes = rb * 128, stage_bytes = 2 * tile_bytes;
  double* partial = reinterpret_cast<double*>(ring + (size_t)kUpdStages * stage_bytes);
  uint64_t* full = reinterpret_cast<uint64_t*>(partial + (TEAMS == 2 ? kUpdPartial : 0));
  uint64_t* empty = full + kUpdStages;
  const int tid = threadIdx.x, warp = tid >> 5, lane = tid & 31;
  if (tid == 0) {
    for (int s = 0; s < kUpdStages; ++s) { mbar_init(&full[s], 1); mbar_init(&empty[s], 4); }
    asm volatile("fence.mbarrier_init.release.cluster;" ::: "memory");
    asm volatile("fence.proxy.async.shared::cta;" ::: "memory");
  }
  __syncthreads();
  const int nk = (neff + 15) >> 4;
  const size_t bs = (size_t)npad * npad;
  if (warp == 4 * TEAMS) {
    if (lane != 0 || (dbg & 1)) return;
    int stage = 0; uint32_t phase = 0;
    for (int w = blockIdx.x; w < nitems; w += gridDim.x) {
      const UpdItem it = items[w];
      for (int p = 0; p < it.count; ++p) {
        const int2 pr = pairs[it.first + p];
        const int rowA = pr.x * npad + it.m0, rowB = pr.y * npad + it.n0;
        for (int kk = 0; kk < nk; ++kk) {
          mbar_wait(&empty[stage], phase ^ 1);
          unsigned char* sa = ring + (size_t)stage * stage_bytes;
          mbar_expect_tx(&full[stage], (uint32_t)stage_bytes);
          tma_load_2d(sa, &tmap, &full[stage], kk * 16, rowA);
          tma_load_2d(sa + tile_bytes, &tmap, &full[stage], kk * 16, rowB);
          if (++stage == kUpdStages) { stage = 0; phase ^= 1; }
        }
      }
      if (TEAMS == 1 && !(it.flags & kUpdFirstFill)) {
        const int hm = ((it.mrows >> 3) + 1) >> 1 << 3, hn = ((it.ncols >> 3) + 1) >> 1 << 3;
        const double* row = dst + (size_t)it.dst * bs + (size_t)it.m0 * npad + it.n0;
        for (int r = 0; r < it.mrows; ++r, row += npad) {
          const int bytes = ((it.flags & kUpdSymDiag) && r < hm ? hn : it.ncols) * 8;
          prefetch_l2_bulk(row, bytes);
        }
      }
    }
    return;
  }
  const int team = warp >> 2, tw = warp & 3;
  const int g = lane >> 2, t = lane & 3;
  const int pg = ((g & 3) << 1) | (g >> 2);
  int kc[4];
#pragma unroll
  for (int k4 = 0; k4 < 4; ++k4) kc[k4] = (((2 * k4 + (t >> 1)) ^ pg) << 4) + ((t & 1) << 3);
  const int wr = tw >> 1, wc = tw & 1;
  double* mypart = partial + (size_t)tw * (25 * 64) + lane * 2;
  if (TEAMS == 2 && team == 0) named_bar_arrive<2, 256>();
  int stage = 0; uint32_t phase = 0; unsigned sidx = 0;
  for (int w = blockIdx.x; w < nitems; w += gridDim.x) {
    const UpdItem it = items[w];
    const int hm = ((it.mrows >> 3) + 1) >> 1 << 3, hn = ((it.ncols >> 3) + 1) >> 1 << 3;
    const int wm = wr * hm, wn = wc * hn;
    int ni = wr ? (it.mrows - hm) >> 3 : hm >> 3, nj = wc ? (it.ncols - hn) >> 3 : hn >> 3;
    if ((it.flags & kUpdSymDiag) && wr == 0 && wc == 1) ni = 0;
    if (ni == 0 || nj == 0) { ni = 0; nj = 0; }
    double acc[5][5][2];
#pragma unroll
    for (int i = 0; i < 5; ++i)
#pragma unroll
      for (int j = 0; j < 5; ++j) { acc[i][j][0] = 0.0; acc[i][j][1] = 0.0; }
    const int code = ni * 8 + nj;
    const int steps = it.count * nk;
    int kk = 0;
    for (int s = 0; s < steps; ++s, ++sidx) {
      if (TEAMS == 1 || (int)(sidx & 1u) == team) {
        if (!(dbg & 1)) mbar_wait(&full[stage], phase);
        const int k4n = min(4, (neff - kk * 16 + 3) >> 2);
        const unsigned char* sa = ring + (size_t)stage * stage_bytes + (size_t)(wm + pg) * 128;
        const unsigned char* sb = ring + (size_t)stage * stage_bytes + tile_bytes + (size_t)(wn + pg) * 128;
        switch (code) {
#define RCVD_UPD_STAGE(NI_, NJ_) case NI_ * 8 + NJ_: upd_stage<NI_, NJ_>(sa, sb, kc, k4n, acc); break;
          RCVD_UPD_CASES(RCVD_UPD_STAGE)
#undef RCVD_UPD_STAGE
          default: break;
        }
        __syncwarp();
        if (lane == 0 && !(dbg & 1)) mbar_arrive(&empty[stage]);
      }
      if (++stage == kUpdStages) { stage = 0; phase ^= 1; }
      if (++kk == nk) kk = 0;
    }
    if (TEAMS == 2 && team == 1) {
      named_bar_sync<2, 256>();
      switch (code) {
#define RCVD_UPD_PART(NI_, NJ_) case NI_ * 8 + NJ_: upd_store_partial<NI_, NJ_>(mypart, acc); break;
        RCVD_UPD_CASES(RCVD_UPD_PART)
#undef RCVD_UPD_PART
        default: break;
      }
      named_bar_arrive<1, 256>();
      continue;
    }
    if (TEAMS == 2) named_bar_sync<1, 256>();
    if (dbg & 2) { if (acc[0][0][0] == 1.2345e300) dst[0] = acc[4][4][1] + acc[2][3][0]; if (TEAMS == 2) named_bar_arrive<2, 256>(); continue; }
    double* C = dst + (size_t)it.dst * bs + (size_t)(it.m0 + wm + pg) * npad + it.n0 + wn + ((t & 1) << 2) + (t & 2);
    const bool fresh = (it.flags & kUpdFirstFill) != 0;
    switch (code) {
#define RCVD_UPD_EPI(NI_, NJ_) case NI_ * 8 + NJ_: upd_epilogue<NI_, NJ_>(C, npad, acc, t, TEAMS == 2 ? mypart : nullptr, fresh); break;
      RCVD_UPD_CASES(RCVD_UPD_EPI)
#undef RCVD_UPD_EPI
      default: break;
    }
    if (TEAMS == 2) named_bar_arrive<2, 256>();
  }
}

}
```

### robust_cvd_b200/solver.py

```python
import ctypes as C
import os
import numpy as np

from . import abi

_HERE = os.path.dirname(os.path.abspath(__file__))
_LIB = None


def lib():
    global _LIB
    if _LIB is None:
        path = os.path.join(_HERE, "librcvd_b200.so")
        if not os.path.exists(path):
            raise RuntimeError(f"{path} is missing: run `python -c 'import __graft_entry__ as g; g.build()'` "
                               "(the CUDA extension is mandatory, there is no CPU fallback)")
        L = C.CDLL(path)
        L.rcvd_last_error.restype = C.c_char_p
        L.rcvd_launch_count.restype = C.c_int64
        L.rcvd_problem_create.argtypes = [C.POINTER(abi.Config), C.c_int32, C.POINTER(C.c_void_p)]
        L.rcvd_problem_destroy.argtypes = [C.c_void_p]
        for name in ("rcvd_frame_stride", "rcvd_depth_param_offset", "rcvd_spatial_param_offset"):
            getattr(L, name).argtypes = [C.POINTER(abi.Config)]
        _LIB = L
    return _LIB


def _p(a, t):
    return a.ctypes.data_as(C.POINTER(t)) if a is not None else None


def _check(rc):
    if rc != 0:
        raise RuntimeError(f"rcvd error {rc}: {lib().rcvd_last_error().decode()}")


def frame_stride(cfg):
    return lib().rcvd_frame_stride(C.byref(cfg))


def depth_param_offset(cfg):
    return lib().rcvd_depth_param_offset(C.byref(cfg))


def spatial_param_offset(cfg):
    return lib().rcvd_spatial_param_offset(C.byref(cfg))


FACTOR_PLAN_COUNTS = ("levels", "offdiag_factor_blocks", "h_blocks", "update_targets", "update_items", "substitution_tasks",
                      "distributed", "first_replicated_level", "first_substitution_level", "rank_l_blocks", "rank_h_blocks", "rank_frames",
                      "update_passes")


def factor_plan(cfg, pairs, trip_centers=(), order_slack=4, nranks=1, rank=0, num_sms=132):
    n = cfg.num_frames
    pf = np.ascontiguousarray(np.asarray(pairs, np.int32).reshape(-1, 2))
    tc = np.ascontiguousarray(np.asarray(trip_centers, np.int32).reshape(-1))
    arrays = {k: np.zeros(n, np.int32) for k in ("order", "level", "owner", "perm")}
    out = (C.c_int32 * len(FACTOR_PLAN_COUNTS))()
    _check(lib().rcvd_debug_factor_plan(C.byref(cfg), C.c_int32(pf.shape[0]), _p(pf, C.c_int32), C.c_int32(tc.size), _p(tc, C.c_int32),
                                        C.c_int32(order_slack), C.c_int32(nranks), C.c_int32(rank), C.c_int32(num_sms),
                                        *(_p(a, C.c_int32) for a in arrays.values()), out))
    return {**arrays, **dict(zip(FACTOR_PLAN_COUNTS, list(out)))}


def update_passes(cfg, pairs, trip_centers=(), order_slack=4, nranks=1, rank=0, num_sms=132):
    pf = np.ascontiguousarray(np.asarray(pairs, np.int32).reshape(-1, 2))
    tc = np.ascontiguousarray(np.asarray(trip_centers, np.int32).reshape(-1))
    args = (C.byref(cfg), C.c_int32(pf.shape[0]), _p(pf, C.c_int32), C.c_int32(tc.size), _p(tc, C.c_int32),
            C.c_int32(order_slack), C.c_int32(nranks), C.c_int32(rank), C.c_int32(num_sms))
    counts = (C.c_int32 * 5)()
    _check(lib().rcvd_debug_update_passes(*args, None, None, None, None, counts))
    passes, sources, join = np.zeros((counts[0], 5), np.int32), np.zeros(counts[1], np.int32), np.zeros(counts[2], np.int32)
    flags = np.zeros(counts[0], np.int32)
    _check(lib().rcvd_debug_update_passes(*args, _p(passes, C.c_int32), _p(sources, C.c_int32), _p(join, C.c_int32), _p(flags, C.c_int32), counts))
    return {"passes": passes, "sources": sources, "join": join.reshape(-1, 2), "flags": flags, "tail": counts[3], "window": counts[4]}


class Problem:
    def __init__(self, cfg, device=0):
        self.cfg = cfg
        self.L = lib()
        self.h = C.c_void_p()
        _check(self.L.rcvd_problem_create(C.byref(cfg), C.c_int32(device), C.byref(self.h)))
        self.N = cfg.num_frames
        self.stride = frame_stride(cfg)
        self.U = self.N * self.stride
        self.num_constraints = 0

    def close(self):
        if getattr(self, "h", None):
            self.L.rcvd_problem_destroy(self.h)
            self.h = None

    def __del__(self):
        try:
            self.close()
        except Exception:
            pass

    def set_frames(self, in_range=None, median_depth=None, adaptive_weights=None):
        ir = None if in_range is None else np.ascontiguousarray(in_range, np.uint8)
        md = None if median_depth is None else np.ascontiguousarray(median_depth, np.float64)
        aw = None if adaptive_weights is None else np.ascontiguousarray(adaptive_weights, np.float64)
        _check(self.L.rcvd_problem_set_frames(self.h, _p(ir, C.c_uint8), _p(md, C.c_double), _p(aw, C.c_double)))

    def _set_records(self, setter, frames, frames_per_group, offsets, records, width):
        fr = np.ascontiguousarray(frames, np.int32).reshape(-1, frames_per_group)
        off = np.ascontiguousarray(offsets, np.int64)
        rec = np.ascontiguousarray(records, np.float32).reshape(-1, width)
        assert off.shape[0] == fr.shape[0] + 1 and off[-1] == rec.shape[0]
        _check(setter(self.h, C.c_int32(fr.shape[0]), _p(fr, C.c_int32), _p(off, C.c_int64), _p(rec, C.c_float)))
        return int(rec.shape[0])

    def set_constraints(self, pair_frames, offsets, records):
        self.num_constraints = self._set_records(self.L.rcvd_problem_set_constraints, pair_frames, 2, offsets, records, 6)

    def set_triplets(self, centers, offsets, records):
        self._set_records(self.L.rcvd_problem_set_triplets, centers, 1, offsets, records, 10)

    def set_depth_pairs(self, pair_frames, offsets, records):
        self._set_records(self.L.rcvd_problem_set_depth_pairs, pair_frames, 2, offsets, records, 6)

    def set_structure(self, pair_frames):
        pf = np.ascontiguousarray(pair_frames, np.int32).reshape(-1, 2)
        _check(self.L.rcvd_problem_set_structure(self.h, C.c_int32(pf.shape[0]), _p(pf, C.c_int32)))

    def init_comm(self, nranks, rank, unique_id):
        uid = np.ascontiguousarray(unique_id, np.uint8)
        assert uid.size == 128
        _check(self.L.rcvd_problem_init_comm(self.h, C.c_int32(nranks), C.c_int32(rank), _p(uid, C.c_uint8)))

    def set_state(self, x):
        x = np.ascontiguousarray(x, np.float64).reshape(-1)
        assert x.size == self.U
        _check(self.L.rcvd_problem_set_state(self.h, _p(x, C.c_double)))

    def get_state(self):
        x = np.empty(self.U, np.float64)
        _check(self.L.rcvd_problem_get_state(self.h, _p(x, C.c_double)))
        return x.reshape(self.N, self.stride)

    def evaluate(self, gradient=False):
        cost = C.c_double()
        g = np.zeros(self.U, np.float64) if gradient else None
        _check(self.L.rcvd_evaluate(self.h, C.byref(cost), _p(g, C.c_double)))
        return (cost.value, g) if gradient else cost.value

    def normal_matrix_dense(self):
        H = np.zeros((self.U, self.U), np.float64)
        _check(self.L.rcvd_normal_matrix_dense(self.h, _p(H, C.c_double)))
        return H

    def debug_linear_solve(self, S, D2, b):
        S = np.ascontiguousarray(S, np.float64); D2 = np.ascontiguousarray(D2, np.float64)
        b = np.ascontiguousarray(b, np.float64); y = np.zeros_like(b)
        _check(self.L.rcvd_debug_linear_solve(self.h, _p(S, C.c_double), _p(D2, C.c_double), _p(b, C.c_double), _p(y, C.c_double)))
        return y

    def solve_matrix(self, H, D2, b):
        H = np.ascontiguousarray(H, np.float64); D2 = np.ascontiguousarray(D2, np.float64); b = np.ascontiguousarray(b, np.float64)
        assert H.shape == (self.U, self.U) and D2.size == self.U and b.size == self.U
        y = np.zeros(self.U, np.float64)
        _check(self.L.rcvd_debug_solve_matrix(self.h, _p(H, C.c_double), _p(D2, C.c_double), _p(b, C.c_double), _p(y, C.c_double)))
        return y

    def factor_dense(self, inverses=False):
        order = np.zeros(self.N, np.int32); Lf = np.zeros((self.U, self.U), np.float64)
        Li = np.zeros((self.N, self.stride, self.stride), np.float64) if inverses else None
        _check(self.L.rcvd_debug_factor_dense(self.h, _p(order, C.c_int32), _p(Lf, C.c_double), _p(Li, C.c_double)))
        return order, Lf, Li

    LINEAR_PATHS = ("potrf_smem", "potrf_panel", "trsm_ll4", "trsm_ll2", "trsm_gemm", "update_tma1", "update_tma2", "substitution_levels", "substitution_fused", "trinv", "other", "update_tma1_multi_item", "trsm_ll_streamed")

    def linear_paths(self):
        out = (C.c_int64 * len(self.LINEAR_PATHS))()
        _check(self.L.rcvd_debug_linear_paths(self.h, out))
        return dict(zip(self.LINEAR_PATHS, list(out)))

    def solve(self, options=None):
        opt = options or abi.default_solve_options()
        s = abi.SolveSummary()
        _check(self.L.rcvd_solve(self.h, C.byref(opt), C.byref(s)))
        return s

    def time_accumulate(self, iters=10):
        ms = C.c_double()
        _check(self.L.rcvd_time_accumulate(self.h, C.c_int32(iters), C.byref(ms)))
        return ms.value

    def time_iteration(self, iters=5, radius=1e4):
        a, b, c, d = C.c_double(), C.c_double(), C.c_double(), C.c_double()
        _check(self.L.rcvd_time_iteration(self.h, C.c_int32(iters), C.c_double(radius), C.byref(a), C.byref(b), C.byref(c), C.byref(d)))
        return {"iter_ms": a.value, "accumulate_ms": b.value, "linear_ms": c.value, "cost_ms": d.value}

    def last_iteration(self):
        g, xc, out = np.empty(self.U, np.float64), np.empty(self.U, np.float64), (C.c_double * 2)()
        _check(self.L.rcvd_debug_last_iteration(self.h, _p(g, C.c_double), _p(xc, C.c_double), out))
        return {"gradient": g.reshape(self.N, self.stride), "candidate_state": xc.reshape(self.N, self.stride), "cost": out[0], "candidate_cost": out[1]}

    def structure_info(self):
        out = (C.c_int32 * 8)()
        _check(self.L.rcvd_structure_info(self.h, out))
        keys = ["frames", "offdiag_factor_blocks", "levels", "h_blocks", "npad", "stride", "tiles", "update_tasks"]
        return dict(zip(keys, list(out)))

    def linear_residual(self, radius=1e4):
        out = (C.c_double * 6)()
        _check(self.L.rcvd_debug_linear_residual(self.h, C.c_double(radius), out))
        keys = ["rel_residual", "rhs_norm", "cost", "grad_norm", "step_norm", "pivot_fail"]
        return dict(zip(keys, list(out)))

    def profile_linear(self, reps=3):
        out = (C.c_double * 8)()
        _check(self.L.rcvd_debug_profile_linear(self.h, C.c_int32(reps), out))
        keys = ["load_ms", "potrf_ms", "trinv_ms", "trsm_ms", "gemm_ms", "solve_ms", "gemm_launches", "gemm_flops"]
        return dict(zip(keys, list(out)))

    def set_fast_path(self, on=True):
        _check(self.L.rcvd_debug_set_fast_path(self.h, C.c_int32(int(on))))

    def set_update_kernel(self, tma=True, side_items_per_cta=0):
        _check(self.L.rcvd_debug_set_update_kernel(self.h, C.c_int32(1 if tma else 0), C.c_int32(side_items_per_cta)))

    def set_eval_only(self, on=True):
        _check(self.L.rcvd_debug_set_eval_only(self.h, C.c_int32(1 if on else 0)))

    def set_distributed(self, on=True):
        _check(self.L.rcvd_debug_set_distributed(self.h, C.c_int32(1 if on else 0)))

    def distribution_info(self):
        out = (C.c_int32 * 4)()
        _check(self.L.rcvd_distribution_info(self.h, out))
        return dict(zip(["distributed", "first_replicated_level", "levels", "frames_owned"], list(out)))

    def set_order_slack(self, slack):
        _check(self.L.rcvd_debug_set_order_slack(self.h, C.c_int32(slack)))

    def set_overlap(self, on=True):
        _check(self.L.rcvd_debug_set_overlap(self.h, C.c_int32(1 if on else 0)))

    def launch_count(self):
        return int(self.L.rcvd_launch_count(self.h))


def nccl_unique_id():
    out = np.zeros(128, np.uint8)
    _check(lib().rcvd_nccl_unique_id(_p(out, C.c_uint8)))
    return out


def depth_apply(cfg, depth_params, src, device=0):
    src = np.ascontiguousarray(src, np.float32); h, w = src.shape
    dp = np.ascontiguousarray(depth_params, np.float64); dst = np.empty_like(src)
    _check(lib().rcvd_depth_apply(C.byref(cfg), C.c_int32(device), _p(dp, C.c_double), _p(src, C.c_float), _p(dst, C.c_float), C.c_int32(h), C.c_int32(w)))
    return dst


def depth_param_map(cfg, depth_params, h, w, device=0):
    k = 2 if cfg.value_xform == abi.VALUE_SCALESHIFT else 1
    dp = np.ascontiguousarray(depth_params, np.float64); out = np.empty((h, w, k), np.float64)
    _check(lib().rcvd_depth_param_map(C.byref(cfg), C.c_int32(device), _p(dp, C.c_double), _p(out, C.c_double), C.c_int32(h), C.c_int32(w)))
    return out[:, :, 0] if k == 1 else out


def spatial_warp(cfg, spatial_params, h, w, device=0):
    sp = np.ascontiguousarray(spatial_params, np.float64); out = np.empty((h, w, 2), np.float32)
    _check(lib().rcvd_spatial_warp(C.byref(cfg), C.c_int32(device), _p(sp, C.c_double), _p(out, C.c_float), C.c_int32(h), C.c_int32(w)))
    return out


def flow_guided_filter(depth, cams, fwd_flow, fwd_mask, bwd_flow, bwd_mask, first_out, num_out, frame_radius, spatial_radius=0, median=False,
                       inv_aspect=1.0, far_pairs=None, far_flow=None, far_mask=None, device=0):
    depth = np.ascontiguousarray(depth, np.float32); cams = np.ascontiguousarray(cams, np.float32)
    F, hd, wd = depth.shape
    arrs = []
    for a, dt in ((fwd_flow, np.float32), (fwd_mask, np.uint8), (bwd_flow, np.float32), (bwd_mask, np.uint8), (far_flow, np.float32), (far_mask, np.uint8)):
        arrs.append(None if a is None else np.ascontiguousarray(a, dt))
    ff, fm, bf, bm, rf, rm = arrs
    ref_mask = fm if fm is not None else rm
    if ref_mask is None:
        raise ValueError("flow masks are needed to define the output resolution")
    h, w = ref_mask.shape[1:3]
    nfar = 0 if far_pairs is None else len(far_pairs)
    fp = None if nfar == 0 else np.ascontiguousarray(far_pairs, np.int32).reshape(-1, 2)
    prm = abi.FilterParams(num_frames=F, first_out=first_out, num_out=num_out, width=w, height=h, depth_width=wd, depth_height=hd,
                           frame_radius=frame_radius, spatial_radius=spatial_radius, median=1 if median else 0, num_far=nfar, inv_aspect=inv_aspect)
    out = np.zeros((num_out, h, w), np.float32)
    _check(lib().rcvd_flow_guided_filter(C.byref(prm), C.c_int32(device), _p(depth, C.c_float), _p(cams, C.c_float),
                                         _p(ff, C.c_float), _p(fm, C.c_uint8), _p(bf, C.c_float), _p(bm, C.c_uint8),
                                         _p(fp, C.c_int32), _p(rf, C.c_float), _p(rm, C.c_uint8), _p(out, C.c_float)))
    return out


def bilateral_filter(depth, out_frames, color_bgr=None, frame_radius=2, spatial_radius=0, depth_sigma=0.3, color_sigma=0.0, median=False,
                     in_place=False, xform_cfg=None, xform_params=None, device=0):
    depth = np.ascontiguousarray(depth, np.float32)
    F, h, w = depth.shape
    of = np.ascontiguousarray(out_frames, np.int32).reshape(-1)
    col = None if color_bgr is None else np.ascontiguousarray(color_bgr, np.float32)
    if col is not None and col.shape != (F, h, w, 3):
        raise ValueError(f"colour stack has shape {col.shape}, expected {(F, h, w, 3)}")
    xp = None if xform_params is None else np.ascontiguousarray(xform_params, np.float64)
    prm = abi.BilateralParams(num_frames=F, width=w, height=h, num_out=len(of), frame_radius=frame_radius, spatial_radius=spatial_radius,
                              median=1 if median else 0, depth_sigma=depth_sigma, color_sigma=color_sigma, in_place=1 if in_place else 0)
    out = np.zeros((len(of), h, w), np.float32)
    _check(lib().rcvd_bilateral_filter(C.byref(prm), C.c_int32(device), _p(depth, C.c_float), _p(col, C.c_float), _p(of, C.c_int32),
                                       None if xform_cfg is None else C.byref(xform_cfg), _p(xp, C.c_double), _p(out, C.c_float)))
    return out


def build_constraints(color_bgr, pair_frames,pair_flow, pair_mask, match_separation, inv_aspect, dyn_dist=None, min_dynamic_distance=-1.0,
                      trip_frames=None, trip_flow=None, trip_mask=None, device=0):
    color = np.ascontiguousarray(color_bgr, np.float32)
    F, h, w = color.shape[:3]
    pf = np.ascontiguousarray(pair_frames, np.int32).reshape(-1, 2); P = len(pf)
    pfl = np.ascontiguousarray(pair_flow, np.float32) if P else None; pm = np.ascontiguousarray(pair_mask, np.uint8) if P else None
    T = 0 if trip_frames is None else len(trip_frames)
    tf = np.ascontiguousarray(trip_frames, np.int32) if T else None
    tfl = np.ascontiguousarray(trip_flow, np.float32) if T else None; tm = np.ascontiguousarray(trip_mask, np.uint8) if T else None
    dd = None if dyn_dist is None else np.ascontiguousarray(dyn_dist, np.float32)
    prm = abi.BuilderParams(num_frames=F, width=w, height=h, dyn_width=0 if dd is None else dd.shape[2], dyn_height=0 if dd is None else dd.shape[1],
                            match_separation=match_separation, num_pairs=P, num_triplets=T, min_dynamic_distance=min_dynamic_distance, inv_aspect=inv_aspect)
    poff = np.zeros(P + 1, np.int64); toff = np.zeros(T + 1, np.int64)
    pcap, tcap = 0, 0
    for attempt in range(2):
        pout = np.zeros((max(pcap, 1), 4), np.float32); tout = np.zeros((max(tcap, 1), 6), np.float32)
        rc = lib().rcvd_build_constraints(C.byref(prm), C.c_int32(device), _p(color, C.c_float), _p(dd, C.c_float), _p(pf if P else None, C.c_int32), _p(pfl, C.c_float), _p(pm, C.c_uint8),
                                          _p(tf, C.c_int32), _p(tfl, C.c_float), _p(tm, C.c_uint8), _p(poff, C.c_int64), _p(pout, C.c_float), C.c_int64(pcap),
                                          _p(toff, C.c_int64), _p(tout, C.c_float), C.c_int64(tcap))
        if rc == 0:
            break
        if attempt == 0 and (poff[P] > pcap or toff[T] > tcap):
            pcap, tcap = int(poff[P]), int(toff[T])
            continue
        _check(rc)
    return poff, pout[:poff[P]], toff, tout[:toff[T]]


def compute_tracks(color_bgr, frame_flags, flow=None, flow_mask=None, dyn_masks=None, spawn_distance=20, prune_distance=5, min_dynamic_distance=3.0,
                   inv_aspect=1.0, device=0):
    color = np.ascontiguousarray(color_bgr, np.float32)
    F, h, w = color.shape[:3]
    fl = np.ascontiguousarray(frame_flags, np.uint8).reshape(-1)
    if fl.size != F:
        raise ValueError(f"{fl.size} frame flags for {F} frames")
    fw = None if flow is None else np.ascontiguousarray(flow, np.float32)
    fm = None if flow_mask is None else np.ascontiguousarray(flow_mask, np.uint8)
    dm = None if dyn_masks is None else np.ascontiguousarray(dyn_masks, np.uint8)
    prm = abi.TrackParams(num_frames=F, width=w, height=h, dyn_width=0 if dm is None else dm.shape[2], dyn_height=0 if dm is None else dm.shape[1],
                          spawn_distance=spawn_distance, prune_distance=prune_distance, min_dynamic_distance=min_dynamic_distance, inv_aspect=inv_aspect)
    off = np.zeros(F + 1, np.int64)
    n = C.c_int64(0)
    cap = F * h * w // 128 + 1024
    for attempt in range(2):
        ids = np.zeros(max(cap, 1), np.int32); locs = np.zeros((max(cap, 1), 2), np.float32)
        rc = lib().rcvd_compute_tracks(C.byref(prm), C.c_int32(device), _p(color, C.c_float), _p(dm, C.c_uint8), _p(fw, C.c_float), _p(fm, C.c_uint8),
                                       _p(fl, C.c_uint8), _p(off, C.c_int64), _p(ids, C.c_int32), _p(locs, C.c_float), C.c_int64(cap), C.byref(n))
        if rc == 0:
            break
        if attempt == 0 and off[F] > cap:
            cap = int(off[F])
            continue
        _check(rc)
    return off, ids[:off[F]], locs[:off[F]], int(n.value)


def static_flags(masks, distance, pair_frames=None, pair_offsets=None, pair_locs=None, trip_frames=None, trip_offsets=None, trip_locs=None, want_distance=False, device=0):
    m = np.ascontiguousarray(masks, np.uint8); F, h, w = m.shape
    P = 0 if pair_frames is None else len(pair_frames); T = 0 if trip_frames is None else len(trip_frames)
    pf = np.ascontiguousarray(pair_frames, np.int32).reshape(-1, 2) if P else None
    po = np.ascontiguousarray(pair_offsets, np.int64) if P else None
    pl = np.ascontiguousarray(pair_locs, np.float32).reshape(-1, 4) if P else None
    tf = np.ascontiguousarray(trip_frames, np.int32) if T else None
    to = np.ascontiguousarray(trip_offsets, np.int64) if T else None
    tl = np.ascontiguousarray(trip_locs, np.float32).reshape(-1, 6) if T else None
    ps = np.zeros(int(po[-1]) if P else 0, np.uint8); ts = np.zeros(int(to[-1]) if T else 0, np.uint8)
    dist = np.zeros((F, h, w), np.float32) if want_distance else None
    _check(lib().rcvd_static_flags(C.c_int32(device), _p(m, C.c_uint8), C.c_int32(F), C.c_int32(h), C.c_int32(w), C.c_float(distance),
                                   C.c_int32(P), _p(pf, C.c_int32), _p(po, C.c_int64), _p(pl, C.c_float), _p(ps if P else None, C.c_uint8),
                                   C.c_int32(T), _p(tf, C.c_int32), _p(to, C.c_int64), _p(tl, C.c_float), _p(ts if T else None, C.c_uint8), _p(dist, C.c_float)))
    return ps, ts, dist


def prune_static_flags(num_frames, height, width, distance, pair_frames, pair_offsets, pair_locs, pair_static,
                       trip_centres=None, trip_offsets=None, trip_locs=None, trip_static=None, device=0):
    P = len(pair_frames); T = 0 if trip_centres is None else len(trip_centres)
    pf = np.ascontiguousarray(pair_frames, np.int32).reshape(-1, 2) if P else None
    po = np.ascontiguousarray(pair_offsets, np.int64) if P else None
    pl = np.ascontiguousarray(pair_locs, np.float32).reshape(-1, 4) if P else None
    ps = np.array(pair_static, np.uint8).reshape(-1) if P else np.zeros(0, np.uint8)
    tc = np.ascontiguousarray(trip_centres, np.int32) if T else None
    to = np.ascontiguousarray(trip_offsets, np.int64) if T else None
# ... 19 lines not shown
```

Measured before the change: 85.11 million.

## Stream TRSM output into the level update kernel via per-strip progress flags

```diff
diff --git a/include/rcvd_hooks.h b/include/rcvd_hooks.h
--- a/include/rcvd_hooks.h
+++ b/include/rcvd_hooks.h
@@ -25,7 +25,7 @@
 
 int32_t rcvd_debug_solve_matrix(rcvd_problem* p, const double* H, const double* D2, const double* b, double* y);
 int32_t rcvd_debug_factor_dense(rcvd_problem* p, int32_t* order, double* L, double* Linv);
-int32_t rcvd_debug_linear_paths(rcvd_problem* p, int64_t out[13]);
+int32_t rcvd_debug_linear_paths(rcvd_problem* p, int64_t out[14]);
 
 int32_t rcvd_debug_linear_residual(rcvd_problem* p, double radius, double out[6]);
 
@@ -37,6 +37,7 @@
 
 int32_t rcvd_debug_set_fast_path(rcvd_problem* p, int32_t on);
 int32_t rcvd_debug_set_overlap(rcvd_problem* p, int32_t on);
+int32_t rcvd_debug_set_update_stream(rcvd_problem* p, int32_t on);
 int32_t rcvd_debug_set_order_slack(rcvd_problem* p, int32_t slack);
 int32_t rcvd_debug_set_eval_only(rcvd_problem* p, int32_t on);
 int32_t rcvd_debug_set_distributed(rcvd_problem* p, int32_t on);
diff --git a/robust_cvd_b200/csrc/rcvd_api.cu b/robust_cvd_b200/csrc/rcvd_api.cu
--- a/robust_cvd_b200/csrc/rcvd_api.cu
+++ b/robust_cvd_b200/csrc/rcvd_api.cu
@@ -138,7 +138,7 @@
 }
 
 enum { LP_POTRF_SMEM = 0, LP_POTRF_PANEL, LP_TRSM_LL4, LP_TRSM_LL2, LP_TRSM_GEMM, LP_UPD_TMA1, LP_UPD_TMA2, LP_SUB_LEVEL, LP_SUB_FUSED,
-       LP_TRINV, LP_OTHER, LP_UPD_TMA1_MULTI, LP_TRSM_STREAMED, LP_N };
+       LP_TRINV, LP_OTHER, LP_UPD_TMA1_MULTI, LP_TRSM_STREAMED, LP_UPD_STREAMED, LP_N };
 
 struct RecordSet {
   const int width, nframes;
@@ -166,6 +166,7 @@
   double *d_H = nullptr, *d_Lb = nullptr, *d_T = nullptr, *d_invL = nullptr, *d_invT = nullptr;
   HBlock *d_hblocks = nullptr, *d_lblocks = nullptr; int* d_fail = nullptr;
   int* d_potrf_progress = nullptr;
+  int* d_xprog = nullptr;
   FactorKernels fk = {};
   FactorPlan plan;
   int *d_lvl_frames = nullptr; TrsmTask* d_trsm_tasks = nullptr; int2* d_upd_pairs = nullptr; SolveTask* d_fwd_tasks = nullptr;
@@ -186,8 +187,9 @@
   bool records_sorted = false;
   int fast_path = 1;
   bool dist_enabled = true, graph_warm = false, force_full_H = false;
+  bool stream_u1 = true;
   int *d_lvl_own = nullptr, *d_load_lblocks = nullptr, *d_own_hblocks = nullptr, *d_uperm = nullptr;
-  UpdItem* d_upd_items = nullptr; CUtensorMap tmapT; int num_sms = 0, upd_ipc = 0;
+  UpdItem* d_upd_items = nullptr; CUtensorMap tmapT; int num_sms = 0, upd_ipc = 2;
   std::vector<double> level_ms;
   bool factored = false;
   int64_t paths[LP_N] = {0}, graph_paths[LP_N] = {0};
@@ -340,6 +342,7 @@
   DA(p->d_g2, Upad + 8); DA(p->d_delta, Upad);
   DA(p->d_ytmp, Upad); DA(p->d_y, Upad); DA(p->d_Sy, Upad); DA(p->d_Hy, Upad); DA(p->d_scal, SC_N); DA(p->d_active, Upad); DA(p->d_fail, 1);
   DA(p->d_potrf_progress, (size_t)N);
+  DA(p->d_xprog, (size_t)std::max(nLoff, 1) * ((npad + kTrsmStrip - 1) / kTrsmStrip));
   DA(p->d_partial, (size_t)p->npartial);
   if (p->eval_only) { DA(p->d_H, 1); DA(p->d_Lb, 1); DA(p->d_T, 1); DA(p->d_invL, 1); DA(p->d_invT, 1); }
   else {
@@ -365,6 +368,7 @@
     if (!encoded) return set_err(RCVD_ERR_CUDA, "cuTensorMapEncodeTiled unavailable or failed: the TMA update kernel cannot run");
     CK(cudaFuncSetAttribute(k_update_tma<1>, cudaFuncAttributeMaxDynamicSharedMemorySize, (int)upd_smem_bytes(p->plan.upd_rb, 1)));
     CK(cudaFuncSetAttribute(k_update_tma<2>, cudaFuncAttributeMaxDynamicSharedMemorySize, (int)upd_smem_bytes(p->plan.upd_rb, 2)));
+    CK(cudaFuncSetAttribute(k_update_tma<2, true>, cudaFuncAttributeMaxDynamicSharedMemorySize, (int)upd_smem_bytes(p->plan.upd_rb, 2)));
   }
   CK(cudaMallocHost((void**)&p->h_scal, (SC_N + 2) * sizeof(double)));
   p->h_fail = (int*)(p->h_scal + SC_N);
@@ -469,6 +473,10 @@
   bool streamed(const Level& v) const {
     return fk.trsm_ll && v.nown > 0 && v.ntrsm > 0 && fk.potrf_smem && strips * v.ntrsm <= (trsm_deep(v) ? 1 : fk.trsm2_ctas_per_sm) * p->num_sms;
   }
+  bool u1_streamed(int li) const {
+    const Level& v = pl.levels[li];
+    return p->stream_u1 && v.nit > 0 && v.nit <= p->num_sms && streamed(v) && !(pl.dist && li < pl.LB);
+  }
 
   int factor_diagonal(const int* frames, int nfr, bool pdl) {
     if (fk.potrf_smem)
@@ -482,7 +490,7 @@
     return RCVD_OK;
   }
 
-  int trsm(const Level& lv, const int* frames, int nfr, bool chain) {
+  int trsm(const Level& lv, const int* frames, int nfr, bool chain, bool publish) {
     const bool inv_stream = fk.trsm_ll && p->overlap;
     if (inv_stream) { if (int rc = wait(inv, st, p->ev_fork)) return rc; inv_used = true; }
     if (int rc = launch(LP_TRINV, k_trinv, dim3(npad / 16, nfr), dim3(256), fk.trinv_bytes, inv_stream ? inv : st, false,
@@ -495,7 +503,7 @@
       decltype(&k_trsm_ll<2>) kernel = deep ? (chain ? k_trsm_ll<4, true> : k_trsm_ll<4>) : (chain ? k_trsm_ll<2, true> : k_trsm_ll<2>);
       if (chain) p->paths[LP_TRSM_STREAMED]++;
       rc = launch(deep ? LP_TRSM_LL4 : LP_TRSM_LL2, kernel, dim3(strips, lv.ntrsm), dim3(128), deep ? fk.trsm_ll4_bytes : fk.trsm_ll2_bytes, st, chain,
-                  p->d_T, p->d_Lb, p->d_invT, p->d_trsm_tasks + lv.trsm_off, npad, chain ? p->d_potrf_progress : nullptr);
+                  p->d_T, p->d_Lb, p->d_invT, p->d_trsm_tasks + lv.trsm_off, npad, chain ? p->d_potrf_progress : nullptr, publish ? p->d_xprog : nullptr);
     } else {
       const int tiles = (npad + 63) / 64;
       rc = launch(LP_TRSM_GEMM, k_gemm_nt, dim3(tiles, tiles, lv.ntrsm), dim3(128), 0, st, false, p->d_T, p->d_Lb, p->d_invL,
@@ -506,28 +514,57 @@
     return RCVD_OK;
   }
 
-  int update(cudaStream_t s, int off, int n) {
+  int update(cudaStream_t s, int off, int n, bool streamed = false) {
+    if (streamed) p->paths[LP_UPD_STREAMED]++;
     if (n <= p->num_sms)
-      return launch(LP_UPD_TMA2, k_update_tma<2>, dim3(n), dim3(UpdShape<2>::threads), upd_smem_bytes(pl.upd_rb, 2), s, false,
-                    p->tmapT, p->d_Lb, p->d_upd_items + off, n, p->d_upd_pairs, npad, pl.upd_neff, pl.upd_rb, 0);
+      return launch(LP_UPD_TMA2, streamed ? k_update_tma<2, true> : k_update_tma<2>, dim3(n), dim3(UpdShape<2>::threads), upd_smem_bytes(pl.upd_rb, 2), s,
+                    false, p->tmapT, p->d_Lb, p->d_upd_items + off, n, p->d_upd_pairs, npad, pl.upd_neff, pl.upd_rb, 0, p->d_xprog, strips);
     int grid = std::min(n, 2 * p->num_sms);
     if (p->upd_ipc > 0) grid = std::max(grid, (n + p->upd_ipc - 1) / p->upd_ipc);
     if (grid < n) p->paths[LP_UPD_TMA1_MULTI]++;
     return launch(LP_UPD_TMA1, k_update_tma<1>, dim3(grid), dim3(UpdShape<1>::threads), upd_smem_bytes(pl.upd_rb, 1), s, false,
-                  p->tmapT, p->d_Lb, p->d_upd_items + off, n, p->d_upd_pairs, npad, pl.upd_neff, pl.upd_rb, 0);
+                  p->tmapT, p->d_Lb, p->d_upd_items + off, n, p->d_upd_pairs, npad, pl.upd_neff, pl.upd_rb, 0, nullptr, 0);
+  }
+
+  int capture_tail(cudaGraphNode_t* node) {
+    cudaStreamCaptureStatus cs; const cudaGraphNode_t* deps = nullptr; const cudaGraphEdgeData* ed = nullptr; size_t n = 0;
+    CK(cudaStreamGetCaptureInfo_v3(st, &cs, nullptr, nullptr, &deps, &ed, &n));
+    *node = nullptr;
+    if (cs != cudaStreamCaptureStatusActive) return RCVD_OK;
+    if (n != 1) return set_err(RCVD_ERR_CUDA, "internal: the TRSM is not the main stream's only capture dependency (%zu)", n);
+    *node = deps[0];
+    return RCVD_OK;
+  }
+  int programmatic_edge_from(cudaGraphNode_t from) {
+    cudaStreamCaptureStatus cs; const cudaGraphNode_t* deps = nullptr; const cudaGraphEdgeData* ed = nullptr; size_t n = 0;
+    CK(cudaStreamGetCaptureInfo_v3(st, &cs, nullptr, nullptr, &deps, &ed, &n));
+    std::vector<cudaGraphNode_t> d(deps, deps + n);
+    std::vector<cudaGraphEdgeData> e(n);
+    bool found = false;
+    for (size_t i = 0; i < n; ++i) {
+      if (ed) e[i] = ed[i];
+      if (d[i] == from) { e[i].from_port = cudaGraphKernelNodePortProgrammatic; e[i].type = cudaGraphDependencyTypeProgrammatic; found = true; }
+    }
+    if (!found) return set_err(RCVD_ERR_CUDA, "internal: the TRSM is no longer a capture dependency of the main stream");
+    CK(cudaStreamUpdateCaptureDependencies_v2(st, d.data(), e.data(), n, cudaStreamSetCaptureDependencies));
+    return RCVD_OK;
   }
 
   int updates(int li) {
     const Level& lv = pl.levels[li];
     const bool u2 = lv.nit2[0] + lv.nit2[1] > 0;
     const bool fork_late = li + 1 < (int)pl.levels.size() && streamed(pl.levels[li + 1]);
+    const bool su = u1_streamed(li);
+    cudaGraphNode_t trsm_node = nullptr;
+    if (su) { if (int rc = capture_tail(&trsm_node)) return rc; }
     if (p->overlap && u2 && !fork_late) { if (int rc = wait(side, st, p->ev_fork)) return rc; }
     if (p->overlap) {
       int s = -1;
       for (int q = side_joined + 1; q < 2 * li; ++q) { const Level& v = pl.levels[q / 2]; if (v.nit2[q % 2] > 0 && v.join[q % 2] <= li) s = q; }
       if (s >= 0) { CK(cudaStreamWaitEvent(st, p->ev_side[s], 0)); side_joined = s; }
     }
-    if (lv.nit > 0) { if (int rc = update(st, lv.it_off, lv.nit)) return rc; mark(P_GEMM); }
+    if (trsm_node) { if (int rc = programmatic_edge_from(trsm_node)) return rc; }
+    if (lv.nit > 0) { if (int rc = update(st, lv.it_off, lv.nit, su)) return rc; mark(P_GEMM); }
     if (p->overlap && u2 && fork_late) { if (int rc = wait(side, st, p->ev_fork)) return rc; }
     for (int h = 0; h < 2; ++h) if (lv.nit2[h] > 0) {
       if (int rc = update(p->overlap ? side : st, lv.it2_off[h], lv.nit2[h])) return rc;
@@ -589,6 +626,7 @@
   const FactorPlan& pl = p->plan; const int npad = p->L.npad, nlv = (int)pl.levels.size();
   f.mark(-1);
   CK(cudaMemsetAsync(p->d_potrf_progress, 0, (size_t)p->N * sizeof(int), p->stream));
+  CK(cudaMemsetAsync(p->d_xprog, 0, (size_t)std::max(pl.nLoff, 1) * f.strips * sizeof(int), p->stream));
   const int nfill = (int)pl.load_lblocks.size() - pl.nload;
   if (int rc = f.launch(LP_OTHER, k_load_factor, dim3((npad * npad + 255) / 256, pl.nload + load_factor_pad_rows(npad, pl.upd_neff, nfill)), dim3(256), 0,
                         p->stream, false, p->d_H, p->d_Lb, p->d_lblocks, p->d_S, p->d_D2, npad, p->L.nf, pl.upd_neff, p->d_load_lblocks, pl.nload, nfill)) return rc;
@@ -601,7 +639,7 @@
       const bool chain = f.streamed(lv);
       if (int rc = f.factor_diagonal(frames, lv.nown, chain && li > 0)) return rc;
       f.mark(FactorSolve::P_POTRF);
-      if (int rc = f.trsm(lv, frames, lv.nown, chain)) return rc;
+      if (int rc = f.trsm(lv, frames, lv.nown, chain, f.u1_streamed(li))) return rc;
     }
     if (pl.dist && li < pl.LB) { if (int rc = f.broadcast_level(li)) return rc; }
     if (int rc = f.updates(li)) return rc;
@@ -1188,9 +1226,9 @@
   }
   return RCVD_OK;
 }
-RCVD_API int32_t rcvd_debug_linear_paths(rcvd_problem* p, int64_t out[13]) {
+RCVD_API int32_t rcvd_debug_linear_paths(rcvd_problem* p, int64_t out[14]) {
   if (!p || !out) return set_err(RCVD_ERR_INVALID, "null argument");
-  static_assert(LP_N == 13, "include/rcvd_hooks.h documents thirteen counters");
+  static_assert(LP_N == 14, "include/rcvd_hooks.h documents fourteen counters");
   std::copy(p->paths, p->paths + LP_N, out);
   return RCVD_OK;
 }
@@ -1360,6 +1398,7 @@
 RCVD_API int64_t rcvd_launch_count(rcvd_problem* p) { return p ? p->launches : 0; }
 RCVD_API int32_t rcvd_debug_set_order_slack(rcvd_problem* p, int32_t slack) { if (!p) return RCVD_ERR_INVALID; p->order_slack = slack; p->structure_ready = false; return RCVD_OK; }
 RCVD_API int32_t rcvd_debug_set_overlap(rcvd_problem* p, int32_t on) { if (!p) return RCVD_ERR_INVALID; p->overlap = on != 0; if (p->solve_graph) { cudaGraphExecDestroy(p->solve_graph); p->solve_graph = nullptr; } return RCVD_OK; }
+RCVD_API int32_t rcvd_debug_set_update_stream(rcvd_problem* p, int32_t on) { if (!p) return RCVD_ERR_INVALID; p->stream_u1 = on != 0; if (p->solve_graph) { cudaGraphExecDestroy(p->solve_graph); p->solve_graph = nullptr; } return RCVD_OK; }
 RCVD_API int32_t rcvd_debug_set_update_kernel(rcvd_problem* p, int32_t tma, int32_t side_items_per_cta) {
   if (!p) return RCVD_ERR_INVALID;
   if (!tma) return set_err(RCVD_ERR_INVALID, "the cp.async update path was removed: k_update_tma is the only update kernel");
diff --git a/robust_cvd_b200/csrc/rcvd_linalg.cuh b/robust_cvd_b200/csrc/rcvd_linalg.cuh
--- a/robust_cvd_b200/csrc/rcvd_linalg.cuh
+++ b/robust_cvd_b200/csrc/rcvd_linalg.cuh
@@ -460,8 +460,9 @@
 
 template <int kTrsmAhead, bool kStreamed = false>
 __global__ void __launch_bounds__(128) k_trsm_ll(double* __restrict__ T, const double* __restrict__ Lb, const double* __restrict__ invT,
-                                                  const TrsmTask* __restrict__ tasks, int npad, const int* progress) {
+                                                  const TrsmTask* __restrict__ tasks, int npad, const int* progress, int* xprog) {
   static_assert(!kStreamed || kTrsmAhead <= 4, "cp_async_wait_upto3 leaves at most three groups in flight");
+  if constexpr (kStreamed) griddep_launch_dependents();
   extern __shared__ __align__(16) double smx[];
   __shared__ int s_ready;
   const int ld = npad + 4;
@@ -588,6 +589,7 @@
       }
     __syncthreads();
     if constexpr (!kStreamed) stage(jt + kTrsmAhead);
+    else if (xprog && tid == 0) st_release_gpu(xprog + (size_t)task.dst * gridDim.x + blockIdx.x, jt + 1);
   }
   if constexpr (kStreamed) griddep_wait();
 }
diff --git a/robust_cvd_b200/csrc/rcvd_plan.h b/robust_cvd_b200/csrc/rcvd_plan.h
--- a/robust_cvd_b200/csrc/rcvd_plan.h
+++ b/robust_cvd_b200/csrc/rcvd_plan.h
@@ -231,6 +231,13 @@
       }
     }
     lv.ntrsm = (int)P.trsm_tasks.size() - lv.trsm_off; lv.nupd = lv.upd2_off[0] - lv.upd_off; lv.nfwd = (int)P.fwd_tasks.size() - lv.fwd_off;
+    if (shared_level) {
+      std::set<int> own_x;
+      for (int q = lv.trsm_off; q < lv.trsm_off + lv.ntrsm; ++q) own_x.insert(P.trsm_tasks[q].dst);
+      for (int q = lv.upd_off; q < lv.upd_off + lv.nupd; ++q)
+        for (int s = P.upd_tasks[q].first; s < P.upd_tasks[q].first + P.upd_tasks[q].count; ++s)
+          if (!own_x.count(P.upd_pairs[s].x) || !own_x.count(P.upd_pairs[s].y)) return "internal: a late update pass reads a block its level's TRSM does not produce";
+    }
     lv.nupd2[0] = lv.upd2_off[1] - lv.upd2_off[0]; lv.nupd2[1] = (int)P.upd_tasks.size() - lv.upd2_off[1];
     std::vector<UpdItem>& items = P.upd_items;
     for (int pass = 0; pass < 3; ++pass) {
diff --git a/robust_cvd_b200/csrc/rcvd_ptx.cuh b/robust_cvd_b200/csrc/rcvd_ptx.cuh
--- a/robust_cvd_b200/csrc/rcvd_ptx.cuh
+++ b/robust_cvd_b200/csrc/rcvd_ptx.cuh
@@ -57,6 +57,7 @@
 __device__ __forceinline__ int ld_acquire_gpu(const int* p) { int v; asm volatile("ld.acquire.gpu.global.s32 %0, [%1];" : "=r"(v) : "l"(p) : "memory"); return v; }
 __device__ __forceinline__ void st_release_gpu(int* p, int v) { asm volatile("st.release.gpu.global.s32 [%0], %1;" ::"l"(p), "r"(v) : "memory"); }
 __device__ __forceinline__ void red_release_add(int* p, int v) { asm volatile("red.release.gpu.global.add.s32 [%0], %1;" ::"l"(p), "r"(v) : "memory"); }
+__device__ __forceinline__ void fence_proxy_async_global() { asm volatile("fence.proxy.async.global;" ::: "memory"); }
 __device__ __forceinline__ void griddep_wait() { asm volatile("griddepcontrol.wait;" ::: "memory"); }
 __device__ __forceinline__ void griddep_launch_dependents() { asm volatile("griddepcontrol.launch_dependents;" ::: "memory"); }
 template <int ID, int N> __device__ __forceinline__ void named_bar_sync() { asm volatile("bar.sync %0, %1;" ::"n"(ID), "n"(N) : "memory"); }
diff --git a/robust_cvd_b200/csrc/rcvd_update.cuh b/robust_cvd_b200/csrc/rcvd_update.cuh
--- a/robust_cvd_b200/csrc/rcvd_update.cuh
+++ b/robust_cvd_b200/csrc/rcvd_update.cuh
@@ -89,14 +89,25 @@
     for (int j = 0; j < NJ; ++j) *reinterpret_cast<double2*>(part + (size_t)(i * 5 + j) * 64) = make_double2(acc[i][j][0], acc[i][j][1]);
 }
 
+__device__ __forceinline__ int xprog_wait(const int* xprog, int strips, int b, int r0, int n, int need) {
+  int least = 1 << 30;
+  for (int s = r0 / kTrsmStrip; s <= (r0 + n - 1) / kTrsmStrip; ++s) {
+    int v;
+    while ((v = ld_acquire_gpu(xprog + (size_t)b * strips + s)) < need) __nanosleep(32);
+    least = min(least, v);
+  }
+  return least;
+}
+
 #define RCVD_UPD_CASES(M) \
   M(1, 1) M(1, 2) M(1, 3) M(1, 4) M(1, 5) M(2, 1) M(2, 2) M(2, 3) M(2, 4) M(2, 5) M(3, 1) M(3, 2) M(3, 3) M(3, 4) M(3, 5) \
   M(4, 1) M(4, 2) M(4, 3) M(4, 4) M(4, 5) M(5, 1) M(5, 2) M(5, 3) M(5, 4) M(5, 5)
 
-template <int TEAMS>
+template <int TEAMS, bool kStreamed = false>
 __global__ void __launch_bounds__(UpdShape<TEAMS>::threads, UpdShape<TEAMS>::ctas) k_update_tma(const __grid_constant__ CUtensorMap tmap, double* __restrict__ dst,
                                                                const UpdItem* __restrict__ items, int nitems, const int2* __restrict__ pairs,
-                                                               int npad, int neff, int rb, int dbg) {
+                                                               int npad, int neff, int rb, int dbg, const int* xprog, int strips) {
+  static_assert(!kStreamed || TEAMS == 2, "the host streams only the two-team launches");
   extern __shared__ __align__(1024) unsigned char ring[];
   griddep_launch_dependents();
   if (smem_u32(ring) & 1023u) __trap();
@@ -122,7 +133,14 @@
       for (int p = 0; p < it.count; ++p) {
         const int2 pr = pairs[it.first + p];
         const int rowA = pr.x * npad + it.m0, rowB = pr.y * npad + it.n0;
+        int ready = 0;
         for (int kk = 0; kk < nk; ++kk) {
+          if constexpr (kStreamed) {
+            if (kk >= ready) {
+              ready = min(xprog_wait(xprog, strips, pr.x, it.m0, it.mrows, kk + 1), xprog_wait(xprog, strips, pr.y, it.n0, it.ncols, kk + 1));
+              fence_proxy_async_global();
+            }
+          }
           mbar_wait(&empty[stage], phase ^ 1);
           unsigned char* sa = ring + (size_t)stage * stage_bytes;
           mbar_expect_tx(&full[stage], (uint32_t)stage_bytes);
@@ -140,6 +158,7 @@
         }
       }
     }
+    if constexpr (kStreamed) griddep_wait();
     return;
   }
   const int team = warp >> 2, tw = warp & 3;
diff --git a/robust_cvd_b200/solver.py b/robust_cvd_b200/solver.py
--- a/robust_cvd_b200/solver.py
+++ b/robust_cvd_b200/solver.py
@@ -171,7 +171,7 @@
         _check(self.L.rcvd_debug_factor_dense(self.h, _p(order, C.c_int32), _p(Lf, C.c_double), _p(Li, C.c_double)))
         return order, Lf, Li
 
-    LINEAR_PATHS = ("potrf_smem", "potrf_panel", "trsm_ll4", "trsm_ll2", "trsm_gemm", "update_tma1", "update_tma2", "substitution_levels", "substitution_fused", "trinv", "other", "update_tma1_multi_item", "trsm_ll_streamed")
+    LINEAR_PATHS = ("potrf_smem", "potrf_panel", "trsm_ll4", "trsm_ll2", "trsm_gemm", "update_tma1", "update_tma2", "substitution_levels", "substitution_fused", "trinv", "other", "update_tma1_multi_item", "trsm_ll_streamed", "update_tma_streamed")
 
     def linear_paths(self):
         out = (C.c_int64 * len(self.LINEAR_PATHS))()
@@ -239,6 +239,9 @@
 
     def set_overlap(self, on=True):
         _check(self.L.rcvd_debug_set_overlap(self.h, C.c_int32(1 if on else 0)))
+
+    def set_update_stream(self, on=True):
+        _check(self.L.rcvd_debug_set_update_stream(self.h, C.c_int32(1 if on else 0)))
 
     def launch_count(self):
         return int(self.L.rcvd_launch_count(self.h))
```

After: 86.71 million, median of 6. 1.9% higher.
